# senikm/trpx

Hardware: AMD Instinct MI355X
Metric: frames/s (Terse encode + Prolix decode round trip, 512x512 uint16 stack, bit-exact vs CPU ref) (higher is better)
Workload: dtype u16

## Files before the change

### include/trpx_hip.h

```cpp
#ifndef TRPX_HIP_H
#define TRPX_HIP_H

#include <stddef.h>
#include <stdint.h>

#ifdef __cplusplus
extern "C" {
#endif

#define TRPX_ABI_VERSION 3

typedef enum trpx_status {
    TRPX_OK = 0,
    TRPX_ERR_INVALID_ARG = 1,
    TRPX_ERR_UNSUPPORTED = 2,
    TRPX_ERR_CAPACITY = 3,
    TRPX_ERR_HIP = 4,
    TRPX_ERR_CORRUPT = 5,
    TRPX_ERR_NO_DEVICE = 6,
    TRPX_ERR_TIMEOUT = 7
} trpx_status;

typedef enum trpx_dtype {
    TRPX_U8 = 0, TRPX_I8 = 1, TRPX_U16 = 2, TRPX_I16 = 3, TRPX_U32 = 4, TRPX_I32 = 5,
    TRPX_F32 = 6, TRPX_F64 = 7,
    TRPX_U64 = 8, TRPX_I64 = 9
} trpx_dtype;

enum { TRPX_STATUS_WORDS = 8 };

int         trpx_abi_version(void);
const char* trpx_last_error_string(void);
size_t      trpx_dtype_size(int dtype);
int         trpx_dtype_is_signed(int dtype);
int         trpx_device_count(void);

size_t trpx_worst_case_bytes(int dtype, size_t n_values, unsigned block);

size_t trpx_encode_workspace_bytes(int dtype, size_t n_values, size_t n_frames, unsigned block);
size_t trpx_decode_workspace_bytes(int dtype, size_t n_values, size_t n_frames, unsigned block);
unsigned trpx_decode_parts_per_frame(int dtype, size_t n_values, size_t n_frames, unsigned block);

int trpx_encode(int dtype, const void* pixels, size_t n_values, size_t n_frames, unsigned block,
                uint8_t* out, size_t out_capacity, uint64_t* frame_offsets, uint32_t* status,
                void* workspace, size_t workspace_bytes, void* stream);

int trpx_decode(int stream_signed, int out_dtype, const uint8_t* terse, size_t terse_bytes,
                const uint64_t* frame_offsets, size_t n_values, size_t n_frames, unsigned block,
                void* pixels_out, uint32_t* status, void* workspace, size_t workspace_bytes,
                void* stream);

int trpx_decode_convert(int stream_signed, int out_dtype, const uint8_t* terse, size_t terse_bytes,
                        const uint64_t* frame_offsets, size_t n_values, size_t n_frames, unsigned block,
                        void* pixels_out, uint32_t* status, void* workspace, size_t workspace_bytes,
                        void* stream);

size_t trpx_index_bytes(int dtype, size_t n_values, size_t n_frames, unsigned block);
int trpx_encode_indexed(int dtype, const void* pixels, size_t n_values, size_t n_frames, unsigned block,
                        uint8_t* out, size_t out_capacity, uint64_t* frame_offsets, uint32_t* status,
                        void* index, void* workspace, size_t workspace_bytes, void* stream);
int trpx_build_index(int dtype, const uint8_t* terse, size_t terse_bytes, const uint64_t* frame_offsets,
                     size_t n_values, size_t n_frames, unsigned block, void* index, uint32_t* status,
                     void* stream);
int trpx_decode_indexed(int stream_signed, int out_dtype, const uint8_t* terse, size_t terse_bytes,
                        const uint64_t* frame_offsets, const void* index, size_t n_values, size_t n_frames,
                        unsigned block, void* pixels_out, uint32_t* status, void* stream);

int trpx_encode_host(int dtype, const void* pixels, size_t n_values, size_t n_frames,
                     unsigned block, uint8_t* out, size_t out_capacity, size_t* total_bytes,
                     uint64_t* frame_offsets, uint32_t* prolix_bits, int device);
int trpx_decode_host(int stream_signed, int out_dtype, const uint8_t* terse, size_t terse_bytes,
                     const uint64_t* frame_offsets, size_t n_values, size_t n_frames,
                     unsigned block, void* pixels_out, int device);

int trpx_frame_offsets_host(const uint8_t* terse, size_t terse_bytes, size_t n_values, size_t n_frames,
                            unsigned block, unsigned max_bits, uint64_t* frame_offsets, int device);

size_t trpx_locate_workspace_bytes(size_t terse_bytes, size_t n_values, size_t n_frames, unsigned block);
int trpx_locate_frames(const uint8_t* terse, size_t terse_bytes, size_t n_values, size_t n_frames, unsigned block,
                       unsigned max_bits, uint64_t* frame_offsets, uint32_t* status, void* workspace, size_t workspace_bytes,
                       void* stream);
int trpx_set_locate_path(int path);

size_t trpx_decode_sum_workspace_bytes(int dtype, size_t terse_bytes, size_t n_values, size_t n_frames,
                                       unsigned block, unsigned group);
int trpx_decode_sum(int dtype, int out_dtype, const uint8_t* terse, size_t terse_bytes,
                    const uint64_t* frame_offsets, const void* index, size_t n_values, size_t n_frames,
                    unsigned block, unsigned group, void* sums_out, uint32_t* status,
                    void* workspace, size_t workspace_bytes, void* stream);
int trpx_decode_sum_host(int dtype, int out_dtype, const uint8_t* terse, size_t terse_bytes,
                         const uint64_t* frame_offsets, size_t n_values, size_t n_frames, unsigned block,
                         unsigned group, void* sums_out, int device);

size_t trpx_decode_roi_workspace_bytes(int dtype, size_t terse_bytes, size_t n_values, size_t n_frames, unsigned block);
int trpx_decode_roi(int dtype, const uint8_t* terse, size_t terse_bytes, const uint64_t* frame_offsets, const void* index,
                    size_t n_values, size_t n_frames, unsigned block, size_t width, const uint32_t* boxes, size_t n_boxes,
                    unsigned box_h, unsigned box_w, void* pixels_out, uint32_t* status, void* workspace,
                    size_t workspace_bytes, void* stream);
int trpx_decode_roi_host(int dtype, const uint8_t* terse, size_t terse_bytes, const uint64_t* frame_offsets, size_t n_values,
                         size_t n_frames, unsigned block, size_t width, const uint32_t* boxes, size_t n_boxes,
                         unsigned box_h, unsigned box_w, void* pixels_out, int device);

int trpx_synth_fill(int dtype, uint64_t seed, uint64_t frame0, size_t n_frames, size_t n_values,
                    void* pixels_dev, void* stream);

int trpx_workspace_invalidate(const void* workspace, size_t workspace_bytes);

int trpx_bench_stream(int mode, const void* src, void* dst, size_t bytes, void* stream);

int trpx_set_encode_path(int path);

int trpx_set_decode_path(int path);

int trpx_encode_checked(int dtype, const void* pixels, size_t n_values, size_t n_frames, unsigned block, uint8_t* out,
                        size_t out_capacity, uint64_t* frame_offsets, uint32_t* status, void* index, void* workspace,
                        size_t workspace_bytes, void* stream, uint32_t* host_status);

int trpx_profile_enable(int on);
int trpx_profile_read(float* stage_ms, int capacity);

typedef struct trpx_header {
    unsigned prolix_bits;
    int      is_signed;
    unsigned block;
    uint64_t memory_size;
    uint64_t number_of_values;
    uint64_t number_of_frames;
    unsigned n_dims;
    uint64_t dims[8];
} trpx_header;

size_t trpx_header_format(const trpx_header* h, char* buf, size_t buf_cap);
int trpx_header_parse(const char* data, size_t len, trpx_header* h, size_t* payload_offset);

size_t trpx_header_format_indexed(const trpx_header* h, const uint64_t* frame_sizes, size_t n_sizes, char* buf, size_t buf_cap);
size_t trpx_header_frame_sizes(const char* data, size_t len, uint64_t* frame_sizes, size_t capacity);

size_t trpx_group_count(size_t n_values, unsigned block);
int trpx_index_group_states(const void* index, size_t n_values, size_t n_frames, unsigned block, uint64_t* group_states, void* stream);
int trpx_index_from_group_states(int dtype, const uint8_t* terse, size_t terse_bytes, const uint64_t* frame_offsets,
                                 const uint64_t* group_states, size_t n_values, size_t n_frames, unsigned block, void* index,
                                 uint32_t* status, void* stream);
int trpx_group_states_host(const uint8_t* terse, size_t terse_bytes, const uint64_t* frame_offsets, size_t n_values,
                           size_t n_frames, unsigned block, unsigned max_bits, uint64_t* group_states, int device);
int trpx_decode_host_grouped(int stream_signed, int out_dtype, const uint8_t* terse, size_t terse_bytes, const uint64_t* frame_offsets,
                             const uint64_t* group_states, size_t n_values, size_t n_frames, unsigned block, void* pixels_out,
                             int device);
size_t trpx_header_format_grouped(const trpx_header* h, const uint64_t* frame_sizes, size_t n_sizes, const uint64_t* group_states,
                                  size_t n_states, char* buf, size_t buf_cap);
size_t trpx_header_group_states(const char* data, size_t len, uint64_t* group_states, size_t capacity);

typedef struct trpx_stack trpx_stack;
int trpx_stack_open(trpx_stack** handle, int stream_signed, const uint8_t* terse, size_t terse_bytes, const uint64_t* frame_offsets,
                    const uint64_t* group_states , size_t n_values, size_t n_frames, unsigned block,
                    unsigned max_bits, int device);
int trpx_stack_read(trpx_stack* stack, size_t frame, int out_dtype, void* pixels_out);
void trpx_stack_close(trpx_stack* stack);
void trpx_host_release(void);

size_t trpx_gather_workspace_bytes(size_t n_slot, int world);
int trpx_gather_frame_offsets(void* comm, const uint64_t* local_offsets, size_t n_local, size_t n_slot,
                              const uint32_t* encode_status, uint64_t* global_offsets, uint32_t* prolix_bits,
                              uint64_t* rank_base, void* workspace, size_t workspace_bytes, void* stream);
int trpx_gather_pack(const uint64_t* local_offsets, size_t n_local, size_t n_slot, const uint32_t* encode_status, uint64_t* message,
                     void* stream);
int trpx_gather_scan(const uint64_t* all_messages, int world, size_t n_slot, uint64_t* global_offsets, uint32_t* prolix_bits,
                     uint64_t* rank_base, void* stream);
size_t trpx_encode_sharded_workspace_bytes(int dtype, size_t n_values, size_t n_local, size_t n_slot, unsigned block, int world);
int trpx_encode_sharded(void* comm, int dtype, const void* pixels, size_t n_values, size_t n_local, size_t n_slot, unsigned block,
                        uint8_t* out, size_t out_capacity, uint64_t* local_offsets, uint32_t* status, uint64_t* global_offsets,
                        uint32_t* prolix_bits, uint64_t* rank_base, void* workspace, size_t workspace_bytes, void* stream,
                        void* gather_stream);
size_t trpx_decode_sharded_workspace_bytes(int dtype, size_t n_values, size_t n_local, unsigned block);
int trpx_decode_sharded(int stream_signed, int out_dtype, const uint8_t* local_terse, size_t local_bytes, const uint64_t* global_offsets,
                        size_t first_frame, size_t n_values, size_t n_local, unsigned block, void* pixels_out, uint32_t* status,
                        void* workspace, size_t workspace_bytes, void* stream);
int trpx_comm_unique_id(void* id128);
int trpx_comm_init(void** comm, int world, int rank, const void* id128);
int trpx_comm_destroy(void* comm);
int trpx_comm_info(void* comm, int* world, int* rank);
const char* trpx_shard_last_error(void);

#ifdef __cplusplus
}
#endif
#endif
```

### trpx_amd/_lib.py

```python
from __future__ import annotations

import ctypes as C
import os

_HERE = os.path.dirname(os.path.abspath(__file__))
LIB_PATH = os.environ.get("TRPX_LIB") or os.path.join(_HERE, "libtrpx_hip.so")

OK, ERR_INVALID_ARG, ERR_UNSUPPORTED, ERR_CAPACITY, ERR_HIP, ERR_CORRUPT, ERR_NO_DEVICE, ERR_TIMEOUT = range(8)
U8, I8, U16, I16, U32, I32, F32, F64, U64, I64 = range(10)
STATUS_WORDS = 8
ABI_VERSION = 3


class TrpxError(RuntimeError):
    def __init__(self, code: int, text: str):
        super().__init__(f"trpx error {code}: {text}")
        self.code = code


class trpx_header(C.Structure):
    _fields_ = [("prolix_bits", C.c_uint), ("is_signed", C.c_int), ("block", C.c_uint),
                ("memory_size", C.c_uint64), ("number_of_values", C.c_uint64),
                ("number_of_frames", C.c_uint64), ("n_dims", C.c_uint), ("dims", C.c_uint64 * 8)]


_P, _SZ, _U, _I, _U64 = C.c_void_p, C.c_size_t, C.c_uint, C.c_int, C.c_uint64
SYMBOLS = {
    "trpx_abi_version": (_I, []),
    "trpx_last_error_string": (C.c_char_p, []),
    "trpx_dtype_size": (_SZ, [_I]),
    "trpx_dtype_is_signed": (_I, [_I]),
    "trpx_device_count": (_I, []),
    "trpx_worst_case_bytes": (_SZ, [_I, _SZ, _U]),
    "trpx_encode_workspace_bytes": (_SZ, [_I, _SZ, _SZ, _U]),
    "trpx_decode_workspace_bytes": (_SZ, [_I, _SZ, _SZ, _U]),
    "trpx_decode_parts_per_frame": (_U, [_I, _SZ, _SZ, _U]),
    "trpx_encode": (_I, [_I, _P, _SZ, _SZ, _U, _P, _SZ, _P, _P, _P, _SZ, _P]),
    "trpx_decode": (_I, [_I, _I, _P, _SZ, _P, _SZ, _SZ, _U, _P, _P, _P, _SZ, _P]),
    "trpx_index_bytes": (_SZ, [_I, _SZ, _SZ, _U]),
    "trpx_encode_indexed": (_I, [_I, _P, _SZ, _SZ, _U, _P, _SZ, _P, _P, _P, _P, _SZ, _P]),
    "trpx_encode_checked": (_I, [_I, _P, _SZ, _SZ, _U, _P, _SZ, _P, _P, _P, _P, _SZ, _P, _P]),
    "trpx_build_index": (_I, [_I, _P, _SZ, _P, _SZ, _SZ, _U, _P, _P, _P]),
    "trpx_decode_indexed": (_I, [_I, _I, _P, _SZ, _P, _P, _SZ, _SZ, _U, _P, _P, _P]),
    "trpx_decode_convert": (_I, [_I, _I, _P, _SZ, _P, _SZ, _SZ, _U, _P, _P, _P, _SZ, _P]),
    "trpx_encode_host": (_I, [_I, _P, _SZ, _SZ, _U, _P, _SZ, C.POINTER(_SZ), _P, C.POINTER(_U), _I]),
    "trpx_decode_host": (_I, [_I, _I, _P, _SZ, _P, _SZ, _SZ, _U, _P, _I]),
    "trpx_frame_offsets_host": (_I, [_P, _SZ, _SZ, _SZ, _U, _U, _P, _I]),
    "trpx_locate_workspace_bytes": (_SZ, [_SZ, _SZ, _SZ, _U]),
    "trpx_locate_frames": (_I, [_P, _SZ, _SZ, _SZ, _U, _U, _P, _P, _P, _SZ, _P]),
    "trpx_decode_sum_workspace_bytes": (_SZ, [_I, _SZ, _SZ, _SZ, _U, _U]),
    "trpx_decode_sum": (_I, [_I, _I, _P, _SZ, _P, _P, _SZ, _SZ, _U, _U, _P, _P, _P, _SZ, _P]),
    "trpx_decode_sum_host": (_I, [_I, _I, _P, _SZ, _P, _SZ, _SZ, _U, _U, _P, _I]),
    "trpx_decode_roi_workspace_bytes": (_SZ, [_I, _SZ, _SZ, _SZ, _U]),
    "trpx_decode_roi": (_I, [_I, _P, _SZ, _P, _P, _SZ, _SZ, _U, _SZ, _P, _SZ, _U, _U, _P, _P, _P, _SZ, _P]),
    "trpx_decode_roi_host": (_I, [_I, _P, _SZ, _P, _SZ, _SZ, _U, _SZ, _P, _SZ, _U, _U, _P, _I]),
    "trpx_gather_workspace_bytes": (_SZ, [_SZ, _I]),
    "trpx_gather_frame_offsets": (_I, [_P, _P, _SZ, _SZ, _P, _P, _P, _P, _P, _SZ, _P]),
    "trpx_encode_sharded_workspace_bytes": (_SZ, [_I, _SZ, _SZ, _SZ, _U, _I]),
    "trpx_encode_sharded": (_I, [_P, _I, _P, _SZ, _SZ, _SZ, _U, _P, _SZ, _P, _P, _P, _P, _P, _P, _SZ, _P, _P]),
    "trpx_decode_sharded_workspace_bytes": (_SZ, [_I, _SZ, _SZ, _U]),
    "trpx_decode_sharded": (_I, [_I, _I, _P, _SZ, _P, _SZ, _SZ, _SZ, _U, _P, _P, _P, _SZ, _P]),
    "trpx_gather_pack": (_I, [_P, _SZ, _SZ, _P, _P, _P]),
    "trpx_gather_scan": (_I, [_P, _I, _SZ, _P, _P, _P, _P]),
    "trpx_comm_unique_id": (_I, [_P]),
    "trpx_comm_init": (_I, [C.POINTER(_P), _I, _I, _P]),
    "trpx_comm_destroy": (_I, [_P]),
    "trpx_comm_info": (_I, [_P, C.POINTER(C.c_int), C.POINTER(C.c_int)]),
    "trpx_shard_last_error": (C.c_char_p, []),
    "trpx_stack_open": (_I, [C.POINTER(_P), _I, _P, _SZ, _P, _P, _SZ, _SZ, _U, _U, _I]),
    "trpx_group_count": (_SZ, [_SZ, _U]),
    "trpx_index_group_states": (_I, [_P, _SZ, _SZ, _U, _P, _P]),
    "trpx_index_from_group_states": (_I, [_I, _P, _SZ, _P, _P, _SZ, _SZ, _U, _P, _P, _P]),
    "trpx_group_states_host": (_I, [_P, _SZ, _P, _SZ, _SZ, _U, _U, _P, _I]),
    "trpx_decode_host_grouped": (_I, [_I, _I, _P, _SZ, _P, _P, _SZ, _SZ, _U, _P, _I]),
    "trpx_header_format_grouped": (_SZ, [C.POINTER(trpx_header), C.c_void_p, _SZ, C.c_void_p, _SZ, C.c_char_p, _SZ]),
    "trpx_header_group_states": (_SZ, [C.c_char_p, _SZ, C.c_void_p, _SZ]),
    "trpx_stack_read": (_I, [_P, _SZ, _I, _P]),
    "trpx_stack_close": (None, [_P]),
    "trpx_host_release": (None, []),
    "trpx_set_encode_path": (_I, [_I]),
    "trpx_set_decode_path": (_I, [_I]),
    "trpx_set_locate_path": (_I, [_I]),
    "trpx_profile_enable": (_I, [_I]),
    "trpx_profile_read": (_I, [C.POINTER(C.c_float), _I]),
    "trpx_bench_stream": (_I, [_I, _P, _P, _SZ, _P]),
    "trpx_workspace_invalidate": (_I, [_P, _SZ]),
    "trpx_synth_fill": (_I, [_I, _U64, _U64, _SZ, _SZ, _P, _P]),
    "trpx_header_format": (_SZ, [C.POINTER(trpx_header), C.c_char_p, _SZ]),
    "trpx_header_parse": (_I, [C.c_char_p, _SZ, C.POINTER(trpx_header), C.POINTER(_SZ)]),
    "trpx_header_format_indexed": (_SZ, [C.POINTER(trpx_header), C.c_void_p, _SZ, C.c_char_p, _SZ]),
    "trpx_header_frame_sizes": (_SZ, [C.c_char_p, _SZ, C.c_void_p, _SZ]),
}

_lib = None


def lib() -> C.CDLL:
    global _lib
    if _lib is None:
        if not os.path.exists(LIB_PATH):
            raise ImportError(f"{LIB_PATH} is missing: the HIP extension has not been built "
                              "(run __graft_entry__.build()); trpx_amd has no CPU fallback")
        L = C.CDLL(LIB_PATH)
        for name, (res, args) in SYMBOLS.items():
            fn = getattr(L, name)
            fn.restype = res
            fn.argtypes = args
        if L.trpx_abi_version() != ABI_VERSION:
            raise ImportError(f"libtrpx_hip.so ABI version {L.trpx_abi_version()} != {ABI_VERSION} (include/trpx_hip.h: TRPX_ABI_VERSION)")
        _lib = L
    return _lib


def check(rc: int) -> None:
    if rc != OK:
        raise TrpxError(rc, lib().trpx_last_error_string().decode(errors="replace"))
```

### trpx_amd/codec.py

```python
from __future__ import annotations

from dataclasses import dataclass

import numpy as np
import torch

from . import _lib
from ._lib import check, lib

_TORCH2DT = {torch.uint8: _lib.U8, torch.int8: _lib.I8, torch.uint16: _lib.U16, torch.int16: _lib.I16,
             torch.uint32: _lib.U32, torch.int32: _lib.I32, torch.uint64: _lib.U64, torch.int64: _lib.I64}
_NP2TORCH = {np.dtype(np.uint8): torch.uint8, np.dtype(np.int8): torch.int8, np.dtype(np.uint16): torch.uint16,
             np.dtype(np.int16): torch.int16, np.dtype(np.uint32): torch.uint32, np.dtype(np.int32): torch.int32,
             np.dtype(np.uint64): torch.uint64, np.dtype(np.int64): torch.int64}
BLOCK = 12


def dtype_code(dt) -> int:
    if isinstance(dt, torch.dtype):
        return _TORCH2DT[dt]
    return _TORCH2DT[_NP2TORCH[np.dtype(dt)]]


def torch_dtype(dt) -> torch.dtype:
    return dt if isinstance(dt, torch.dtype) else _NP2TORCH[np.dtype(dt)]


def _stream_ptr(t: torch.Tensor) -> int:
    return torch.cuda.current_stream(t.device).cuda_stream


def worst_case_bytes(dtype, n_values: int, block: int = BLOCK) -> int:
    return lib().trpx_worst_case_bytes(dtype_code(dtype), n_values, block)


@dataclass
class Encoded:
    data: torch.Tensor
    frame_offsets: torch.Tensor
    status: torch.Tensor
    n_values: int
    n_frames: int
    dtype: torch.dtype
    index: torch.Tensor | None = None
    _retry: tuple | None = None

    def total_bytes(self) -> int:
        return int(self.frame_offsets[-1].item())

    def prolix_bits(self) -> int:
        return int(self.status[1].item())

    def check(self) -> None:
        code = int(self.status[0].item())
        if code == _lib.ERR_TIMEOUT and self._retry is not None:
            px, ws, block = self._retry
            with torch.cuda.device(px.device):
                check(lib().trpx_encode_checked(dtype_code(px.dtype), px.data_ptr(), self.n_values, self.n_frames, block,
                                                self.data.data_ptr(), self.data.numel(), self.frame_offsets.data_ptr(),
                                                self.status.data_ptr(), self.index.data_ptr() if self.index is not None else None,
                                                ws.data_ptr(), ws.numel(), _stream_ptr(px), None))
            code = int(self.status[0].item())
        if code:
            raise _lib.TrpxError(code, "device status after encode")

    def stack(self) -> torch.Tensor:
        return self.data[: self.total_bytes()]


class Workspace:

    def __init__(self, device):
        self.device = torch.device(device)
        self.buf = None

    def get(self, nbytes: int) -> torch.Tensor:
        if self.buf is None or self.buf.numel() < nbytes:
            self.release()
            self.buf = torch.empty(max(nbytes, 256), dtype=torch.uint8, device=self.device)
        return self.buf

    def release(self) -> None:
        if self.buf is not None:
            try:
                lib().trpx_workspace_invalidate(self.buf.data_ptr(), self.buf.numel())
            except Exception:
                pass
            self.buf = None

    def __del__(self):
        self.release()


def index_bytes(dtype, n_values: int, n_frames: int, block: int = BLOCK) -> int:
    return lib().trpx_index_bytes(dtype_code(dtype), n_values, n_frames, block)


def encode(pixels: torch.Tensor, out: torch.Tensor | None = None, workspace: Workspace | None = None,
           frame_offsets: torch.Tensor | None = None, status: torch.Tensor | None = None,
           block: int = BLOCK, index: torch.Tensor | bool | None = None) -> Encoded:
    if not pixels.is_cuda:
        raise ValueError("pixels must live on the GPU (use trpx_amd.Terse for host data)")
    px = pixels.contiguous()
    n_frames = px.shape[0]
    n_values = px[0].numel()
    code = dtype_code(px.dtype)
    dev = px.device
    if out is None:
        cap = (n_frames * worst_case_bytes(px.dtype, n_values, block) + 15) // 16 * 16
        out = torch.empty(cap, dtype=torch.uint8, device=dev)
    if frame_offsets is None:
        frame_offsets = torch.empty(n_frames + 1, dtype=torch.int64, device=dev)
    if status is None:
        status = torch.empty(_lib.STATUS_WORDS, dtype=torch.int32, device=dev)
    ws_bytes = lib().trpx_encode_workspace_bytes(code, n_values, n_frames, block)
    ws = workspace.get(ws_bytes) if workspace is not None else torch.empty(max(ws_bytes, 256), dtype=torch.uint8, device=dev)
    if index is True:
        index = torch.empty(index_bytes(px.dtype, n_values, n_frames, block), dtype=torch.uint8, device=dev)
    with torch.cuda.device(dev):
        check(lib().trpx_encode_indexed(code, px.data_ptr(), n_values, n_frames, block, out.data_ptr(), out.numel(),
                                        frame_offsets.data_ptr(), status.data_ptr(),
                                        index.data_ptr() if index is not None else None, ws.data_ptr(), ws.numel(),
                                        _stream_ptr(px)))
        if workspace is None:
            check(lib().trpx_workspace_invalidate(ws.data_ptr(), ws.numel()))
    return Encoded(out, frame_offsets, status, n_values, n_frames, px.dtype, index if index is not None else None, (px, ws, block))


def decode(terse: torch.Tensor, frame_offsets: torch.Tensor | None, n_values: int, n_frames: int, dtype,
           out: torch.Tensor | None = None, workspace: Workspace | None = None,
           status: torch.Tensor | None = None, stream_signed: bool | None = None,
           block: int = BLOCK, index: torch.Tensor | None = None):
    tdt = torch_dtype(dtype)
    code = dtype_code(tdt)
    dev = terse.device
    if stream_signed is None:
        stream_signed = bool(lib().trpx_dtype_is_signed(code))
    if out is None:
        out = torch.empty((n_frames, n_values), dtype=tdt, device=dev)
    if status is None:
        status = torch.empty(_lib.STATUS_WORDS, dtype=torch.int32, device=dev)
    if index is not None:
        with torch.cuda.device(dev):
            check(lib().trpx_decode_indexed(int(stream_signed), code, terse.data_ptr(), terse.numel(),
                                            frame_offsets.data_ptr(), index.data_ptr(), n_values, n_frames, block,
                                            out.data_ptr(), status.data_ptr(), _stream_ptr(terse)))
        return out, status
    ws_bytes = lib().trpx_decode_workspace_bytes(code, n_values, n_frames, block)
    ws = (workspace or Workspace(dev)).get(ws_bytes)
    with torch.cuda.device(dev):
        check(lib().trpx_decode(int(stream_signed), code, terse.data_ptr(), terse.numel(),
                                frame_offsets.data_ptr() if frame_offsets is not None else None,
                                n_values, n_frames, block, out.data_ptr(), status.data_ptr(), ws.data_ptr(),
                                ws.numel(), _stream_ptr(terse)))
    return out, status


def locate_workspace_bytes(terse_bytes: int, n_values: int, n_frames: int, block: int = BLOCK) -> int:
    return lib().trpx_locate_workspace_bytes(terse_bytes, n_values, n_frames, block)


def _max_bits(dtype) -> int:
    return 8 * lib().trpx_dtype_size(dtype_code(torch_dtype(dtype)))


def locate_frames(terse: torch.Tensor, n_values: int, n_frames: int, dtype, block: int = BLOCK,
                  workspace: Workspace | None = None, status: torch.Tensor | None = None,
                  out: torch.Tensor | None = None):
    dev = terse.device
    if out is None:
        out = torch.empty(n_frames + 1, dtype=torch.int64, device=dev)
    if status is None:
        status = torch.empty(_lib.STATUS_WORDS, dtype=torch.int32, device=dev)
    ws = (workspace or Workspace(dev)).get(locate_workspace_bytes(terse.numel(), n_values, n_frames, block))
    with torch.cuda.device(dev):
        check(lib().trpx_locate_frames(terse.data_ptr(), terse.numel(), n_values, n_frames, block, _max_bits(dtype),
                                       out.data_ptr(), status.data_ptr(), ws.data_ptr(), ws.numel(), _stream_ptr(terse)))
    return out, status


def build_index(terse: torch.Tensor, frame_offsets: torch.Tensor, n_values: int, n_frames: int, dtype,
                block: int = BLOCK) -> torch.Tensor:
    code = dtype_code(torch_dtype(dtype))
    dev = terse.device
    index = torch.empty(index_bytes(dtype, n_values, n_frames, block), dtype=torch.uint8, device=dev)
    status = torch.empty(_lib.STATUS_WORDS, dtype=torch.int32, device=dev)
    with torch.cuda.device(dev):
        check(lib().trpx_build_index(code, terse.data_ptr(), terse.numel(), frame_offsets.data_ptr(), n_values,
                                     n_frames, block, index.data_ptr(), status.data_ptr(), _stream_ptr(terse)))
    return index


def synth(dtype, frame0: int, n_frames: int, n_values: int, device="cuda", seed: int = 20240807) -> torch.Tensor:
    tdt = torch_dtype(dtype)
    out = torch.empty((n_frames, n_values), dtype=tdt, device=device)
    with torch.cuda.device(out.device):
        check(lib().trpx_synth_fill(dtype_code(tdt), seed, frame0, n_frames, n_values, out.data_ptr(),
                                    _stream_ptr(out)))
    return out


_SUM_OUT = {torch.int32: _lib.I32, torch.uint32: _lib.U32, torch.int64: _lib.I64, torch.uint64: _lib.U64,
            torch.float32: _lib.F32, torch.float64: _lib.F64}


def decode_sum_workspace_bytes(terse_bytes: int, n_values: int, n_frames: int, dtype, group: int, block: int = BLOCK) -> int:
    return lib().trpx_decode_sum_workspace_bytes(dtype_code(torch_dtype(dtype)), terse_bytes, n_values, n_frames, block, group)


def decode_sum(terse: torch.Tensor, frame_offsets: torch.Tensor | None, n_values: int, n_frames: int, dtype, group: int,
               out_dtype=torch.int32, index: torch.Tensor | None = None, out: torch.Tensor | None = None,
               workspace: Workspace | None = None, status: torch.Tensor | None = None, block: int = BLOCK):
    odt = torch_dtype(out_dtype)
    if odt not in _SUM_OUT:
        raise TypeError(f"decode_sum: out_dtype {odt} (int32, uint32, int64, uint64, float32, float64)")
    code = dtype_code(torch_dtype(dtype))
    dev = terse.device
    n_out = -(-n_frames // group) if group > 0 else 0
    if out is None:
        out = torch.empty((n_out, n_values), dtype=odt, device=dev)
    if status is None:
        status = torch.empty(_lib.STATUS_WORDS, dtype=torch.int32, device=dev)
    ws_bytes = lib().trpx_decode_sum_workspace_bytes(code, terse.numel(), n_values, n_frames, block, group)
    ws = (workspace or Workspace(dev)).get(ws_bytes)
    with torch.cuda.device(dev):
        check(lib().trpx_decode_sum(code, _SUM_OUT[odt], terse.data_ptr(), terse.numel(),
                                    frame_offsets.data_ptr() if frame_offsets is not None else None,
                                    index.data_ptr() if index is not None else None, n_values, n_frames, block, group,
                                    out.data_ptr(), status.data_ptr(), ws.data_ptr(), ws.numel(), _stream_ptr(terse)))
    return out, status


def decode_roi_workspace_bytes(terse_bytes: int, n_values: int, n_frames: int, dtype, block: int = BLOCK) -> int:
    return lib().trpx_decode_roi_workspace_bytes(dtype_code(torch_dtype(dtype)), terse_bytes, n_values, n_frames, block)


def decode_roi(terse: torch.Tensor, frame_offsets: torch.Tensor | None, n_values: int, n_frames: int, dtype, width: int,
               boxes: torch.Tensor, box_shape, index: torch.Tensor | None = None, out: torch.Tensor | None = None,
               workspace: Workspace | None = None, status: torch.Tensor | None = None, block: int = BLOCK):
    tdt = torch_dtype(dtype)
    code = dtype_code(tdt)
    dev = terse.device
    if boxes.dtype not in (torch.int32, torch.uint32) or boxes.dim() != 2 or boxes.shape[1] != 3 or not boxes.is_contiguous():
        raise TypeError("decode_roi: boxes must be a contiguous [n, 3] tensor of int32 / uint32")
    if boxes.device != dev:
        raise ValueError("decode_roi: boxes must live on the stack's device")
    box_h, box_w = (int(x) for x in box_shape)
    n_boxes = boxes.shape[0]
    if out is None:
        out = torch.empty((n_boxes, box_h, box_w), dtype=tdt, device=dev)
    elif out.dtype != tdt or out.numel() != n_boxes * box_h * box_w or not out.is_contiguous() or out.device != dev:
        raise ValueError(f"decode_roi: out must be a contiguous {tdt} tensor of {n_boxes} x {box_h} x {box_w} elements on {dev}")
    if status is None:
        status = torch.empty(_lib.STATUS_WORDS, dtype=torch.int32, device=dev)
    ws_ptr, ws_bytes = None, 0
    if index is None or frame_offsets is None:
        ws = (workspace or Workspace(dev)).get(lib().trpx_decode_roi_workspace_bytes(code, terse.numel(), n_values, n_frames, block))
        ws_ptr, ws_bytes = ws.data_ptr(), ws.numel()
    with torch.cuda.device(dev):
        check(lib().trpx_decode_roi(code, terse.data_ptr(), terse.numel(),
                                    frame_offsets.data_ptr() if frame_offsets is not None else None,
                                    index.data_ptr() if index is not None else None, n_values, n_frames, block, width,
                                    boxes.data_ptr(), n_boxes, box_h, box_w, out.data_ptr(), status.data_ptr(), ws_ptr, ws_bytes,
                                    _stream_ptr(terse)))
    return out, status
```

### trpx_amd/csrc/api.hip

```cpp
#include <hip/hip_runtime.h>
#include <stdarg.h>
#include <stdio.h>
#include <stdlib.h>
#include <string.h>
#include <algorithm>
#include <initializer_list>
#include <vector>

#include "../../include/trpx_hip.h"
#include "decode_roi.hpp"
#include "decode_sum.hpp"
#include "launchers.hpp"
#include "profile.hpp"

namespace trpx {
Profiler& profiler() {
    static thread_local Profiler p;
    return p;
}
}

namespace {

thread_local char g_err[512] = "";

int fail(int code, const char* fmt, ...) {
    va_list ap;
    va_start(ap, fmt);
    vsnprintf(g_err, sizeof g_err, fmt, ap);
    va_end(ap);
    return code;
}
#define HIP_TRY(expr)                                                                         \
    do {                                                                                      \
        hipError_t e_ = (expr);                                                               \
        if (e_ != hipSuccess) return fail(TRPX_ERR_HIP, "%s: %s", #expr, hipGetErrorString(e_)); \
    } while (0)

constexpr unsigned kMaxBlock = 4096;
constexpr unsigned kBlock = trpx::kBlock;

bool is64(int dtype) { return dtype == TRPX_U64 || dtype == TRPX_I64; }
size_t convert_elem_size(int out_dtype) { return out_dtype == TRPX_F32 ? 4 : out_dtype == TRPX_F64 ? 8 : trpx_dtype_size(out_dtype); }
bool tuned_type(int stream_signed, int out_dtype) {
    return trpx_dtype_size(out_dtype) && out_dtype <= TRPX_I32 && (stream_signed != 0) == (trpx_dtype_is_signed(out_dtype) != 0);
}
uint64_t worst_frame_bits(int dtype, size_t n_values, unsigned block) { return 8 * (uint64_t)trpx_worst_case_bytes(dtype, n_values, block); }
bool frame_bits_fit_32(int dtype, size_t n_values, unsigned block) { return worst_frame_bits(dtype, n_values, block) < 0xF0000000ull; }
bool fits_per_frame_decoder(int dtype, size_t n_values, unsigned block) { return worst_frame_bits(dtype, n_values, block) + (1u << 17) < (1ull << 26); }

bool geom_of(size_t n_values, unsigned block, trpx::FrameGeom* g) {
    if (n_values == 0 || block == 0 || block > kMaxBlock) return false;
    const uint64_t nb = (n_values + block - 1) / block;
    if (nb > 0xFFFFFFFFull) return false;
    g->n_values = n_values;
    g->n_blocks = (uint32_t)nb;
    g->n_tiles = (uint32_t)((nb + trpx::kTileBlocks - 1) / trpx::kTileBlocks);
    g->block = block;
    return true;
}

bool sizes_ok(const trpx::FrameGeom& g, size_t n_frames) {
    if (n_frames == 0 || n_frames > 0x7FFFFFFFull / g.n_tiles) return false;
    const unsigned __int128 bytes = (unsigned __int128)g.n_values * n_frames * 8;
    return bytes < ((unsigned __int128)1 << 62);
}
int bad_geom(const char* fn, unsigned block) {
    return fail(block != kBlock ? TRPX_ERR_UNSUPPORTED : TRPX_ERR_INVALID_ARG, "%s: unsupported sizes/block (block=%u)", fn, block);
}

struct PtrReq { const void* p; size_t align; bool required = true; };
enum : unsigned {
    kDtypeFirst = 1,
    kIndexOnly = 2,
    kSameSign = 4,
    kHasStream = 8,
};
int check_args(const char* fn, unsigned rules, int dtype, size_t elem, int stream_signed, size_t terse_bytes, size_t n_values,
               size_t n_frames, unsigned block, std::initializer_list<PtrReq> ptrs, trpx::FrameGeom* g) {
    if ((rules & kDtypeFirst) && !elem) return fail(TRPX_ERR_INVALID_ARG, "%s: unknown dtype %d", fn, dtype);
    if (rules & kIndexOnly ? block != kBlock : block == 0 || block > kMaxBlock)
        return fail(TRPX_ERR_UNSUPPORTED, rules & kIndexOnly ? "%s: block=%u (the decode index needs %u)" : "%s: block=%u (supported: 1..%u; 12 is the tuned default, Terse.hpp:264)",
                    fn, block, rules & kIndexOnly ? kBlock : kMaxBlock);
    if ((rules & kIndexOnly) && is64(dtype)) return fail(TRPX_ERR_UNSUPPORTED, "%s: no decode index for 64-bit containers (generic kernels)", fn);
    if ((rules & kSameSign) && (stream_signed != 0) != (trpx_dtype_is_signed(dtype) != 0))
        return fail(TRPX_ERR_UNSUPPORTED, "%s: stream signed=%d into dtype %d: only same-signedness decode is defined by the reference (Terse.hpp:356-357)",
                    fn, stream_signed, dtype);
    if (!elem) return fail(TRPX_ERR_INVALID_ARG, "%s: unknown dtype %d", fn, dtype);
    if (!geom_of(n_values, block, g) || !sizes_ok(*g, n_frames) || ((rules & kHasStream) && !terse_bytes))
        return fail(TRPX_ERR_INVALID_ARG, "%s: bad sizes n_values=%zu n_frames=%zu", fn, n_values, n_frames);
    for (const PtrReq& q : ptrs)
        if (q.required && !q.p) return fail(TRPX_ERR_INVALID_ARG, "%s: null pointer", fn);
    for (const PtrReq& q : ptrs)
        if ((uintptr_t)q.p % q.align) return fail(TRPX_ERR_INVALID_ARG, "%s: misaligned pointer (%p needs %zu B)", fn, q.p, q.align);
    return TRPX_OK;
}

struct EncWs { size_t frame_size, tile_off, tile_bits, fused, total; };
EncWs enc_ws(const trpx::FrameGeom& g, size_t n_frames) {
    EncWs w;
    const size_t tiles = n_frames * (size_t)g.n_tiles;
    w.frame_size = 0;
    w.tile_off = trpx::align_up(w.frame_size + 8 * n_frames, 16);
    w.tile_bits = trpx::align_up(w.tile_off + 8 * tiles, 16);
    w.fused = trpx::align_up(w.tile_bits + 4 * tiles, 256);
    w.total = w.fused + trpx::fused_workspace_bytes(g, n_frames);
    return w;
}

struct DecLayout { size_t tile_off, widths, seg, defer, parts, part_ws, total; };
DecLayout dec_layout(const trpx::FrameGeom& g, size_t n_frames, size_t pixel_bytes, size_t front, bool parts_route) {
    DecLayout l;
    l.tile_off = trpx::align_up(front, 16);
    l.widths = trpx::align_up(l.tile_off + 8 * n_frames * (size_t)g.n_tiles, 16);
    l.seg = trpx::align_up(l.widths + n_frames * (size_t)g.n_blocks, 256);
    l.defer = l.seg + trpx::seg_workspace_bytes(g, n_frames);
    l.parts = l.defer + trpx::defer_bytes(n_frames);
    size_t P = trpx::chain_parts_per_frame(g, n_frames, pixel_bytes), scratch = trpx::chain_workspace_bytes(g, n_frames, pixel_bytes);
    if (parts_route) {
        P = std::max<size_t>(P, trpx::parts_per_frame(g, n_frames));
        scratch = std::max(scratch, trpx::part_workspace_bytes(g, n_frames));
    }
    l.part_ws = l.parts + (P > 1 ? trpx::align_up(sizeof(trpx::PartDesc) * n_frames * P, 256) : 0);
    l.total = l.part_ws + scratch;
    return l;
}
DecLayout idx_layout(const trpx::FrameGeom& g, size_t n_frames, size_t pixel_bytes = 4) { return dec_layout(g, n_frames, pixel_bytes, 0, false); }
DecLayout dec_ws(const trpx::FrameGeom& g, size_t n_frames, size_t pixel_bytes) { return dec_layout(g, n_frames, pixel_bytes, 8 * (n_frames + 1), true); }

trpx::DecodeArgs decode_args(const uint8_t* terse, size_t terse_bytes, const uint64_t* frame_offsets, const trpx::FrameGeom& g,
                             size_t n_frames, void* pixels_out, uint32_t* status) {
    trpx::DecodeArgs a{};
    a.terse = terse;
    a.terse_bytes = terse_bytes;
    a.frame_offsets = frame_offsets;
    a.geom = g;
    a.n_frames = (uint32_t)n_frames;
    a.pixels_out = pixels_out;
    a.status = status;
    return a;
}
enum : unsigned { kSeg = 1, kDefer = 2, kParts = 4 };
void point_into(trpx::DecodeArgs& a, const void* block, const DecLayout& l, unsigned scratch = 0) {
    char* b = const_cast<char*>(static_cast<const char*>(block));
    a.tile_off = reinterpret_cast<uint64_t*>(b + l.tile_off);
    a.widths = reinterpret_cast<uint8_t*>(b + l.widths);
    if (scratch & kSeg) a.seg_ws = b + l.seg;
    if (scratch & kDefer) a.defer = reinterpret_cast<uint32_t*>(b + l.defer + trpx::kDeferFront);
    if (scratch & kParts) {
        a.parts = reinterpret_cast<trpx::PartDesc*>(b + l.parts);
        a.part_ws = b + l.part_ws;
    }
}

int g_encode_path = [] {
    const char* e = getenv("TRPX_ENCODE_PATH");
    return e && strcmp(e, "twopass") == 0 ? 1 : 0;
}();
enum DecodeRoute {
    kRouteAuto = 0,
    kRouteBasic = 1,
    kRouteTiled = 2,
    kRouteFrames = 3,
    kRouteParts = 4,
};
constexpr int kSelectDense = 5;
DecodeRoute g_decode_path = [] {
    const char* e = getenv("TRPX_DECODE_PATH");
    if (!e) return kRouteAuto;
    if (strcmp(e, "dense") == 0) trpx::set_dense_route(true);
    return strcmp(e, "basic") == 0 ? kRouteBasic : (strcmp(e, "tiles") == 0 || strcmp(e, "seg") == 0) ? kRouteTiled
           : strcmp(e, "frames") == 0 ? kRouteFrames : strcmp(e, "parts") == 0 ? kRouteParts : kRouteAuto;
}();
bool large_frames_by_index() { return g_decode_path != kRouteTiled && g_decode_path != kRouteParts; }
[[maybe_unused]] const int g_single_part_env = [] {
    const char* e = getenv("TRPX_SINGLE_PART");
    unsigned f = 0, b = 0;
    if (e && sscanf(e, "%u,%u", &f, &b) == 2) trpx::set_single_part_rule(f, b);
    return 0;
}();

struct IdxScratch {
    struct Slot { int dev; hipStream_t st; void* p; size_t bytes; };
    std::vector<Slot> slots;
    ~IdxScratch() { for (auto& s : slots) if (s.p) (void)hipFree(s.p); }
};
void* indexed_scratch(size_t bytes, hipStream_t st) {
    static thread_local IdxScratch t;
    int dev = 0;
    if (hipGetDevice(&dev) != hipSuccess) return nullptr;
    hipStreamCaptureStatus cs = hipStreamCaptureStatusNone;
    if (hipStreamIsCapturing(st, &cs) != hipSuccess) { (void)hipGetLastError(); return nullptr; }
    if (cs != hipStreamCaptureStatusNone) return nullptr;
    for (auto& s : t.slots)
        if (s.dev == dev && s.st == st) {
            if (s.bytes >= bytes) return s.p;
            if (hipStreamSynchronize(st) != hipSuccess) return nullptr;
            (void)hipFree(s.p);
            s.p = nullptr; s.bytes = 0;
            if (hipMalloc(&s.p, bytes) != hipSuccess) { s.p = nullptr; (void)hipGetLastError(); return nullptr; }
            s.bytes = bytes;
            return s.p;
        }
    void* p = nullptr;
    if (hipMalloc(&p, bytes) != hipSuccess) { (void)hipGetLastError(); return nullptr; }
    t.slots.push_back({dev, st, p, bytes});
    return p;
}

int build_index_impl(int dtype, const uint8_t* terse, size_t terse_bytes, const uint64_t* frame_offsets, size_t n_values,
                     size_t n_frames, unsigned block, void* index, uint32_t* status, bool clear_status, void* stream) {
    trpx::FrameGeom g;
    if (const int rc = check_args("trpx_build_index", kIndexOnly | kHasStream, dtype, trpx_dtype_size(dtype), 0, terse_bytes, n_values, n_frames, block,
                                  {{terse, 4}, {frame_offsets, 8}, {index, 16}, {status, 8}}, &g))
        return rc;
    if (!frame_bits_fit_32(dtype, n_values, block)) return fail(TRPX_ERR_UNSUPPORTED, "trpx_build_index: frames of >= 2^32 bits");
    trpx::DecodeArgs a = decode_args(terse, terse_bytes, frame_offsets, g, n_frames, nullptr, status);
    const DecLayout il = idx_layout(g, n_frames, trpx_dtype_size(dtype));
    point_into(a, index, il, kSeg | kDefer);
    a.index_per_frame = fits_per_frame_decoder(dtype, n_values, block) && g_decode_path != kRouteTiled;
    a.parts_per_frame = trpx::chain_parts_per_frame(g, n_frames, trpx_dtype_size(dtype));
    a.chain = a.parts_per_frame > 1u && n_frames * (uint64_t)a.parts_per_frame < 0x7FFFFFFFull && large_frames_by_index();
    if (a.chain) point_into(a, index, il, kParts);
    else a.parts_per_frame = 1;
    HIP_TRY(trpx::launch_walk_only(a, (uint32_t)(8 * trpx_dtype_size(dtype)), clear_status, static_cast<hipStream_t>(stream)));
    return TRPX_OK;
}

int encode_impl(int dtype, const void* pixels, size_t n_values, size_t n_frames, unsigned block, uint8_t* out, size_t out_capacity,
                uint64_t* frame_offsets, uint32_t* status, void* index, void* workspace, size_t workspace_bytes, void* stream,
                bool two_pass) {
    trpx::FrameGeom g;
    if (const int rc = check_args("trpx_encode", kDtypeFirst, dtype, trpx_dtype_size(dtype), 0, 0, n_values, n_frames, block,
                                  {{pixels, trpx_dtype_size(dtype)}, {frame_offsets, 8}, {status, 8}, {workspace, 8},
                                   {out, 16, out_capacity != 0}}, &g))
        return rc;
    const EncWs w = enc_ws(g, n_frames);
    if (workspace_bytes < w.total)
        return fail(TRPX_ERR_CAPACITY, "trpx_encode: workspace %zu < %zu", workspace_bytes, w.total);

    trpx::EncodeArgs a;
    a.pixels = pixels;
    a.geom = g;
    a.n_frames = (uint32_t)n_frames;
    a.out = out;
    a.out_capacity = out_capacity;
    a.frame_offsets = frame_offsets;
    a.status = status;
    char* ws = static_cast<char*>(workspace);
    a.frame_size = reinterpret_cast<uint64_t*>(ws + w.frame_size);
    a.tile_off = reinterpret_cast<uint64_t*>(ws + w.tile_off);
    a.tile_bits = reinterpret_cast<uint32_t*>(ws + w.tile_bits);
    if ((uintptr_t)index % 16) return fail(TRPX_ERR_INVALID_ARG, "trpx_encode_indexed: index must be 16-byte aligned");
    const DecLayout il = idx_layout(g, n_frames, trpx_dtype_size(dtype));
    a.idx_group_off = index ? reinterpret_cast<uint64_t*>(static_cast<char*>(index) + il.tile_off) : nullptr;
    a.idx_widths = index ? reinterpret_cast<uint8_t*>(static_cast<char*>(index) + il.widths) : nullptr;
    if (block != kBlock || is64(dtype)) {
        if (index) return fail(TRPX_ERR_UNSUPPORTED, "trpx_encode_indexed: the decode index needs block=12 and pixels of <= 32 bits");
        trpx::fused_ws_forget(workspace, workspace_bytes);
        HIP_TRY(trpx::launch_encode_generic(dtype, a, static_cast<hipStream_t>(stream)));
        return TRPX_OK;
    }
    const bool vec_ok = (uint64_t)g.n_blocks * 396 < (1ull << 40);
    if (g_encode_path == 0 && !two_pass && vec_ok) {
        trpx::fused_ws_forget(workspace, workspace_bytes, ws + w.fused);
        HIP_TRY(trpx::launch_encode_fused(dtype, a, ws + w.fused, static_cast<hipStream_t>(stream)));
    } else {
        trpx::fused_ws_forget(workspace, workspace_bytes);
        HIP_TRY(trpx::launch_encode(dtype, a, static_cast<hipStream_t>(stream)));
        if (index && out)
            return build_index_impl(dtype, out, out_capacity, frame_offsets, n_values, n_frames, block, index, status, false, stream);
    }
    return TRPX_OK;
}

hipError_t copy_sync(hipStream_t hs, void* dst, const void* src, size_t n, hipMemcpyKind kind) {
    const hipError_t e = hipMemcpyAsync(dst, src, n, kind, hs);
    return e != hipSuccess ? e : hipStreamSynchronize(hs);
}
int read_status(hipStream_t hs, const uint32_t* d_status, uint32_t st[TRPX_STATUS_WORDS]) {
    HIP_TRY(copy_sync(hs, st, d_status, 4 * TRPX_STATUS_WORDS, hipMemcpyDeviceToHost));
    return TRPX_OK;
}
int status_result(const char* fn, const uint32_t* st) {
    return st[0] ? fail((int)st[0], "%s: device status %u (5: corrupt or truncated stream)", fn, st[0]) : TRPX_OK;
}

int encode_retrying(int dtype, const void* pixels, size_t n_values, size_t n_frames, unsigned block, uint8_t* out, size_t out_capacity,
                    uint64_t* frame_offsets, uint32_t* status, void* index, void* workspace, size_t workspace_bytes, void* stream,
                    uint32_t st[TRPX_STATUS_WORDS]) {
    for (int attempt = 0; attempt < 2; ++attempt) {
        int rc = encode_impl(dtype, pixels, n_values, n_frames, block, out, out_capacity, frame_offsets, status, index, workspace,
                             workspace_bytes, stream, attempt == 1);
        if (rc || (rc = read_status(static_cast<hipStream_t>(stream), status, st))) return rc;
        if (st[0] != TRPX_ERR_TIMEOUT) break;
    }
    return TRPX_OK;
}

}

extern "C" {

int trpx_abi_version(void) { return TRPX_ABI_VERSION; }
const char* trpx_last_error_string(void) { return g_err; }

size_t trpx_dtype_size(int dtype) {
    switch (dtype) {
    case TRPX_U8: case TRPX_I8: return 1;
    case TRPX_U16: case TRPX_I16: return 2;
    case TRPX_U32: case TRPX_I32: return 4;
    case TRPX_U64: case TRPX_I64: return 8;
    }
    return 0;
}
int trpx_dtype_is_signed(int dtype) { return dtype >= 0 && dtype <= TRPX_I32 ? (dtype & 1) : (dtype == TRPX_I64 ? 1 : 0); }

int trpx_device_count(void) {
    int n = 0;
    if (hipGetDeviceCount(&n) != hipSuccess) return 0;
    return n;
}

size_t trpx_worst_case_bytes(int dtype, size_t n_values, unsigned block) {
    const size_t es = trpx_dtype_size(dtype);
    if (!es || !block) return 0;
    const size_t nblocks = (n_values + block - 1) / block;
    return n_values * es + (12 * nblocks + 7) / 8 + 1;
}

size_t trpx_encode_workspace_bytes(int dtype, size_t n_values, size_t n_frames, unsigned block) {
    trpx::FrameGeom g;
    if (!trpx_dtype_size(dtype) || !geom_of(n_values, block, &g)) return 0;
    return enc_ws(g, n_frames).total;
}
size_t trpx_decode_workspace_bytes(int dtype, size_t n_values, size_t n_frames, unsigned block) {
    trpx::FrameGeom g;
    if (!trpx_dtype_size(dtype) || !geom_of(n_values, block, &g)) return 0;
    return dec_ws(g, n_frames, trpx_dtype_size(dtype)).total;
}
size_t trpx_index_bytes(int dtype, size_t n_values, size_t n_frames, unsigned block) {
    trpx::FrameGeom g;
    if (!trpx_dtype_size(dtype) || !geom_of(n_values, block, &g)) return 0;
    return idx_layout(g, n_frames, trpx_dtype_size(dtype)).total;
}

unsigned trpx_decode_parts_per_frame(int dtype, size_t n_values, size_t n_frames, unsigned block) {
    trpx::FrameGeom g;
    if (!trpx_dtype_size(dtype) || is64(dtype) || block != kBlock || !geom_of(n_values, block, &g)) return 1;
    return g_decode_path != kRouteParts && frame_bits_fit_32(dtype, n_values, block) ? trpx::chain_parts_per_frame(g, n_frames, trpx_dtype_size(dtype))
                                                                                   : trpx::parts_per_frame(g, n_frames);
}

int trpx_encode(int dtype, const void* pixels, size_t n_values, size_t n_frames, unsigned block, uint8_t* out,
                size_t out_capacity, uint64_t* frame_offsets, uint32_t* status, void* workspace,
                size_t workspace_bytes, void* stream) {
    return encode_impl(dtype, pixels, n_values, n_frames, block, out, out_capacity, frame_offsets, status, nullptr, workspace,
                       workspace_bytes, stream, false);
}

int trpx_encode_indexed(int dtype, const void* pixels, size_t n_values, size_t n_frames, unsigned block, uint8_t* out,
                        size_t out_capacity, uint64_t* frame_offsets, uint32_t* status, void* index,
                        void* workspace, size_t workspace_bytes, void* stream) {
    return encode_impl(dtype, pixels, n_values, n_frames, block, out, out_capacity, frame_offsets, status, index, workspace,
                       workspace_bytes, stream, false);
}

int trpx_encode_checked(int dtype, const void* pixels, size_t n_values, size_t n_frames, unsigned block, uint8_t* out,
                        size_t out_capacity, uint64_t* frame_offsets, uint32_t* status, void* index, void* workspace,
                        size_t workspace_bytes, void* stream, uint32_t* host_status) {
    uint32_t st[TRPX_STATUS_WORDS] = {0};
    if (const int rc = encode_retrying(dtype, pixels, n_values, n_frames, block, out, out_capacity, frame_offsets, status, index,
                                       workspace, workspace_bytes, stream, st))
        return rc;
    if (host_status) memcpy(host_status, st, sizeof st);
    return status_result("trpx_encode_checked", st);
}

int trpx_decode(int stream_signed, int out_dtype, const uint8_t* terse, size_t terse_bytes,
                const uint64_t* frame_offsets, size_t n_values, size_t n_frames, unsigned block, void* pixels_out,
                uint32_t* status, void* workspace, size_t workspace_bytes, void* stream) {
    trpx::FrameGeom g;
    const size_t es = trpx_dtype_size(out_dtype);
    if (!es) return fail(TRPX_ERR_INVALID_ARG, "trpx_decode: unknown dtype %d", out_dtype);
    if (is64(out_dtype))
        return trpx_decode_convert(stream_signed, out_dtype, terse, terse_bytes, frame_offsets, n_values, n_frames, block, pixels_out,
                                   status, workspace, workspace_bytes, stream);
    if (const int rc = check_args("trpx_decode", kDtypeFirst | kSameSign | kHasStream, out_dtype, es, stream_signed, terse_bytes, n_values, n_frames,
                                  block, {{terse, 4}, {pixels_out, es}, {status, 8}, {workspace, 8}, {frame_offsets, 8, false}}, &g))
        return rc;
    const DecLayout w = dec_ws(g, n_frames, es);
    if (workspace_bytes < w.total)
        return fail(TRPX_ERR_CAPACITY, "trpx_decode: workspace %zu < %zu", workspace_bytes, w.total);

    hipStream_t hs = static_cast<hipStream_t>(stream);
    trpx::fused_ws_forget(workspace, workspace_bytes);
    trpx::DecodeArgs a = decode_args(terse, terse_bytes, frame_offsets, g, n_frames, pixels_out, status);
    char* ws = static_cast<char*>(workspace);
    a.walk_offsets = reinterpret_cast<uint64_t*>(ws);
#ifdef TRPX_DIAGNOSTICS
    static const bool no_defer = getenv("TRPX_NO_DEFER") != nullptr;
#else
    constexpr bool no_defer = false;
#endif
    point_into(a, ws, w, no_defer ? kSeg : kSeg | kDefer);
    const bool basic = g_decode_path == kRouteBasic, force_tiles = g_decode_path == kRouteTiled;
    const bool bits32 = frame_bits_fit_32(out_dtype, n_values, block);
    const uint32_t max_w = 8u * (uint32_t)es;
    const bool located = !frame_offsets && !basic && bits32 && block == kBlock && trpx::locate_parallel(g, terse_bytes, n_frames, max_w) &&
                         w.total - w.tile_off >= trpx::locate_workspace_bytes(g, terse_bytes, n_frames);
    if (located) {
        HIP_TRY(trpx::launch_locate(terse, terse_bytes, g, (uint32_t)n_frames, max_w, a.walk_offsets, status, ws + w.tile_off, hs));
        a.frame_offsets = frame_offsets = a.walk_offsets;
    }
    const bool fast_ok = frame_offsets && !basic && bits32 && block == kBlock;
    const bool frame26 = fits_per_frame_decoder(out_dtype, n_values, block);
    a.chain = large_frames_by_index() && bits32;
    a.parts_per_frame = a.chain ? trpx::chain_parts_per_frame(g, n_frames, es) : trpx::parts_per_frame(g, n_frames);
    const bool parts_ok = a.parts_per_frame > 1u && n_frames * (uint64_t)a.parts_per_frame < 0x7FFFFFFFull && a.defer;
    if (parts_ok) point_into(a, ws, w, kParts);
    else a.parts_per_frame = 1;
    if (fast_ok && (parts_ok || (frame26 && trpx::parts_per_frame(g, n_frames) == 1u)) && !force_tiles)
        HIP_TRY(trpx::launch_decode_frames(out_dtype, a, hs));
    else if (fast_ok)
        HIP_TRY(trpx::launch_decode_fast(out_dtype, a, false, hs));
    else
        HIP_TRY(trpx::launch_decode(out_dtype, a, frame_offsets != nullptr, hs));
    if (located)
        HIP_TRY(trpx::launch_locate_status(a.walk_offsets, (uint32_t)n_frames, status, hs));
    return TRPX_OK;
}

int trpx_build_index(int dtype, const uint8_t* terse, size_t terse_bytes, const uint64_t* frame_offsets,
                     size_t n_values, size_t n_frames, unsigned block, void* index, uint32_t* status, void* stream) {
    return build_index_impl(dtype, terse, terse_bytes, frame_offsets, n_values, n_frames, block, index, status, true, stream);
}

int trpx_decode_indexed(int stream_signed, int out_dtype, const uint8_t* terse, size_t terse_bytes,
                        const uint64_t* frame_offsets, const void* index, size_t n_values, size_t n_frames,
                        unsigned block, void* pixels_out, uint32_t* status, void* stream) {
    trpx::FrameGeom g;
    const size_t es = trpx_dtype_size(out_dtype);
    if (const int rc = check_args("trpx_decode_indexed", kDtypeFirst | kIndexOnly | kSameSign | kHasStream, out_dtype, es, stream_signed, terse_bytes,
                                  n_values, n_frames, block, {{terse, 4}, {index, 16}, {frame_offsets, 8}, {pixels_out, es}, {status, 8}}, &g))
        return rc;
    hipStream_t hs = static_cast<hipStream_t>(stream);
    trpx::DecodeArgs a = decode_args(terse, terse_bytes, frame_offsets, g, n_frames, pixels_out, status);
    point_into(a, index, idx_layout(g, n_frames, es));
    const bool per_frame = fits_per_frame_decoder(out_dtype, n_values, block) && g_decode_path != kRouteTiled &&
                           (g_decode_path == kRouteFrames || n_frames >= 1024);
    const bool misaligned = (g.n_values * es) % 128u != 0u || (uintptr_t)pixels_out % 128u != 0u;
    if (per_frame && misaligned && g_decode_path == kRouteAuto && trpx::parts_per_frame(g, n_frames) == 1u) {
        void* scratch = indexed_scratch(trpx::defer_bytes(n_frames), hs);
        if (scratch) {
            a.defer = reinterpret_cast<uint32_t*>(static_cast<char*>(scratch) + trpx::kDeferFront);
            a.seg_ws = scratch;
            a.index_given = true;
            HIP_TRY(trpx::launch_decode_frames(out_dtype, a, hs));
            return TRPX_OK;
        }
    }
    HIP_TRY(trpx::launch_decode_fast(out_dtype, a, true, hs, per_frame));
    return TRPX_OK;
}

size_t trpx_group_count(size_t n_values, unsigned block) {
    trpx::FrameGeom g;
    if (block != kBlock || !geom_of(n_values, block, &g)) return 0;
    return g.n_tiles;
}

int trpx_index_group_states(const void* index, size_t n_values, size_t n_frames, unsigned block, uint64_t* states, void* stream) {
    trpx::FrameGeom g;
    if (const int rc = check_args("trpx_index_group_states", kIndexOnly, TRPX_U8, 1, 0, 0, n_values, n_frames, block, {{index, 16}, {states, 8}}, &g))
        return rc;
    trpx::DecodeArgs a = decode_args(nullptr, 0, nullptr, g, n_frames, nullptr, nullptr);
    point_into(a, index, idx_layout(g, n_frames));
    HIP_TRY(trpx::launch_index_group_states(a, states, static_cast<hipStream_t>(stream)));
    return TRPX_OK;
}

int trpx_index_from_group_states(int dtype, const uint8_t* terse, size_t terse_bytes, const uint64_t* frame_offsets,
                                 const uint64_t* states, size_t n_values, size_t n_frames, unsigned block, void* index,
                                 uint32_t* status, void* stream) {
    trpx::FrameGeom g;
    if (const int rc = check_args("trpx_index_from_group_states", kIndexOnly | kHasStream, dtype, trpx_dtype_size(dtype), 0, terse_bytes, n_values,
                                  n_frames, block, {{terse, 4}, {frame_offsets, 8}, {states, 8}, {index, 16}, {status, 8}}, &g))
        return rc;
    if (worst_frame_bits(dtype, n_values, block) >= (1ull << 40))
        return fail(TRPX_ERR_UNSUPPORTED, "trpx_index_from_group_states: frames of >= 2^40 bits");
    trpx::DecodeArgs a = decode_args(terse, terse_bytes, frame_offsets, g, n_frames, nullptr, status);
    point_into(a, index, idx_layout(g, n_frames));
    HIP_TRY(trpx::launch_walk_groups(a, (uint32_t)(8 * trpx_dtype_size(dtype)), states, true, static_cast<hipStream_t>(stream)));
    return TRPX_OK;
}

int trpx_decode_convert(int stream_signed, int out_dtype, const uint8_t* terse, size_t terse_bytes,
                        const uint64_t* frame_offsets, size_t n_values, size_t n_frames, unsigned block, void* pixels_out,
                        uint32_t* status, void* workspace, size_t workspace_bytes, void* stream) {
    trpx::FrameGeom g;
    const size_t es = convert_elem_size(out_dtype);
    if (const int rc = check_args("trpx_decode_convert", kDtypeFirst | kHasStream, out_dtype, es, stream_signed, terse_bytes, n_values, n_frames, block,
                                  {{terse, 4}, {pixels_out, es}, {status, 8}, {workspace, 8}, {frame_offsets, 8, false}}, &g))
        return rc;
    const DecLayout w = dec_ws(g, n_frames, es);
    if (workspace_bytes < w.total) return fail(TRPX_ERR_CAPACITY, "trpx_decode_convert: workspace %zu < %zu", workspace_bytes, w.total);
    trpx::fused_ws_forget(workspace, workspace_bytes);
    trpx::DecodeArgs a = decode_args(terse, terse_bytes, frame_offsets, g, n_frames, pixels_out, status);
    a.walk_offsets = static_cast<uint64_t*>(workspace);
    point_into(a, workspace, w, kSeg);
    HIP_TRY(trpx::launch_decode_convert(out_dtype, a, stream_signed != 0, frame_offsets != nullptr, static_cast<hipStream_t>(stream)));
    return TRPX_OK;
}

int trpx_workspace_invalidate(const void* workspace, size_t workspace_bytes) {
    trpx::fused_ws_forget(workspace, workspace_bytes);
    return TRPX_OK;
}

int trpx_set_encode_path(int path) {
    if (path != 0 && path != 1) return fail(TRPX_ERR_INVALID_ARG, "trpx_set_encode_path: 0 = auto, 1 = two-pass");
    g_encode_path = path;
    return TRPX_OK;
}

int trpx_set_decode_path(int path) {
    if (path < kRouteAuto || path > kSelectDense) return fail(TRPX_ERR_INVALID_ARG, "trpx_set_decode_path: 0 = auto, 1 = basic, 2 = tiled, 3 = per-frame, 4 = parts route for large frames, 5 = auto with the dense walk for listed frames");
    trpx::set_dense_route(path == kSelectDense);
    g_decode_path = path == kSelectDense ? kRouteAuto : static_cast<DecodeRoute>(path);
    return TRPX_OK;
}

int trpx_set_locate_path(int path) {
    if (path != 0 && path != 1) return fail(TRPX_ERR_INVALID_ARG, "trpx_set_locate_path: 0 = auto, 1 = serial");
    trpx::g_locate_path = path;
    return TRPX_OK;
}

int trpx_profile_enable(int on) {
    trpx::profiler().enabled = on != 0;
    return TRPX_OK;
}
int trpx_profile_read(float* stage_ms, int capacity) {
    if (!stage_ms || capacity <= 0) return 0;
    return trpx::profiler().read(stage_ms, capacity);
}

int trpx_synth_fill(int dtype, uint64_t seed, uint64_t frame0, size_t n_frames, size_t n_values, void* pixels_dev,
                    void* stream) {
    if (dtype != TRPX_U16 && dtype != TRPX_I32)
        return fail(TRPX_ERR_UNSUPPORTED, "trpx_synth_fill: synth-v1 is defined for U16 and I32");
    if (!pixels_dev) return fail(TRPX_ERR_INVALID_ARG, "trpx_synth_fill: null pointer");
    HIP_TRY(trpx::launch_synth(dtype, seed, frame0, n_frames, n_values, pixels_dev, static_cast<hipStream_t>(stream)));
    return TRPX_OK;
}

size_t trpx_locate_workspace_bytes(size_t terse_bytes, size_t n_values, size_t n_frames, unsigned block) {
    trpx::FrameGeom g;
    if (!terse_bytes || !geom_of(n_values, block, &g) || !sizes_ok(g, n_frames)) return 0;
    return trpx::locate_workspace_bytes(g, terse_bytes, n_frames);
}

int trpx_locate_frames(const uint8_t* terse, size_t terse_bytes, size_t n_values, size_t n_frames, unsigned block, unsigned max_bits,
                       uint64_t* frame_offsets, uint32_t* status, void* workspace, size_t workspace_bytes, void* stream) {
    trpx::FrameGeom g;
    if (!terse || !terse_bytes || !frame_offsets || !status || !workspace || max_bits == 0 || max_bits > 64)
        return fail(TRPX_ERR_INVALID_ARG, "trpx_locate_frames: bad argument");
    if (!geom_of(n_values, block, &g)) return bad_geom("trpx_locate_frames", block);
    if (!sizes_ok(g, n_frames) || n_frames > terse_bytes)
        return fail(TRPX_ERR_INVALID_ARG, "trpx_locate_frames: bad sizes n_values=%zu n_frames=%zu", n_values, n_frames);
    if ((uintptr_t)terse % 4 || (uintptr_t)workspace % 8 || (uintptr_t)frame_offsets % 8 || (uintptr_t)status % 8)
        return fail(TRPX_ERR_INVALID_ARG, "trpx_locate_frames: misaligned pointer (terse needs 4 B, workspace 8 B)");
    const size_t need = trpx::locate_workspace_bytes(g, terse_bytes, n_frames);
    if (workspace_bytes < need) return fail(TRPX_ERR_CAPACITY, "trpx_locate_frames: workspace %zu < %zu", workspace_bytes, need);
    trpx::fused_ws_forget(workspace, workspace_bytes);
    HIP_TRY(trpx::launch_locate(terse, terse_bytes, g, (uint32_t)n_frames, max_bits, frame_offsets, status, workspace,
                                static_cast<hipStream_t>(stream)));
    return TRPX_OK;
}

}
namespace {
bool sum_out_ok(int out_dtype) {
    return out_dtype == TRPX_I32 || out_dtype == TRPX_U32 || out_dtype == TRPX_I64 || out_dtype == TRPX_U64 ||
           out_dtype == TRPX_F32 || out_dtype == TRPX_F64;
}
size_t sum_out_size(int out_dtype) { return out_dtype == TRPX_I32 || out_dtype == TRPX_U32 || out_dtype == TRPX_F32 ? 4 : 8; }
struct IndexWs { size_t offsets, region, total; };
IndexWs index_ws(int dtype, const trpx::FrameGeom& g, size_t terse_bytes, size_t n_frames, bool have_offsets, bool have_index) {
    IndexWs w;
    w.offsets = 0;
    w.region = have_offsets ? 0 : trpx::align_up(8 * (n_frames + 1), 256);
    const size_t idx = have_index ? 0 : idx_layout(g, n_frames, trpx_dtype_size(dtype)).total;
    const size_t loc = have_offsets ? 0 : trpx::locate_workspace_bytes(g, terse_bytes, n_frames);
    w.total = w.region + trpx::align_up(std::max(idx, loc), 256);
    return w;
}
int index_in_workspace(int dtype, const uint8_t* terse, size_t terse_bytes, const uint64_t** frame_offsets, const void** index,
                       size_t n_values, size_t n_frames, unsigned block, const trpx::FrameGeom& g, uint32_t* status, char* ws,
                       const IndexWs& w, void* stream, bool* clear) {
    *clear = true;
    if (!*frame_offsets) {
        uint64_t* offs = reinterpret_cast<uint64_t*>(ws + w.offsets);
        HIP_TRY(trpx::launch_locate(terse, terse_bytes, g, (uint32_t)n_frames, 8u * (uint32_t)trpx_dtype_size(dtype), offs, status,
                                    ws + w.region, static_cast<hipStream_t>(stream)));
        *frame_offsets = offs;
        *clear = false;
    }
    if (!*index) {
        const int rc = build_index_impl(dtype, terse, terse_bytes, *frame_offsets, n_values, n_frames, block, ws + w.region, status,
                                        *clear, stream);
        if (rc) return rc;
        *index = ws + w.region;
        *clear = false;
    }
    return TRPX_OK;
}
struct SumWs { IndexWs front; size_t partial, total; };
SumWs sum_ws(int dtype, const trpx::FrameGeom& g, size_t terse_bytes, size_t n_frames, size_t group, bool have_offsets, bool have_index) {
    SumWs w;
    w.front = index_ws(dtype, g, terse_bytes, n_frames, have_offsets, have_index);
    w.partial = w.front.total;
    w.total = w.partial + trpx::sum_plan(dtype, g, n_frames, group).partial_bytes;
    return w;
}
}

extern "C" {

size_t trpx_decode_sum_workspace_bytes(int dtype, size_t terse_bytes, size_t n_values, size_t n_frames, unsigned block,
                                       unsigned group) {
    trpx::FrameGeom g;
    if (dtype < TRPX_U8 || dtype > TRPX_I32 || block != kBlock || !group || !terse_bytes ||
        !geom_of(n_values, block, &g) || !sizes_ok(g, n_frames))
        return 0;
    return sum_ws(dtype, g, terse_bytes, n_frames, group, false, false).total;
}

int trpx_decode_sum(int dtype, int out_dtype, const uint8_t* terse, size_t terse_bytes, const uint64_t* frame_offsets,
                    const void* index, size_t n_values, size_t n_frames, unsigned block, unsigned group, void* sums_out,
                    uint32_t* status, void* workspace, size_t workspace_bytes, void* stream) {
    trpx::FrameGeom g;
    if (is64(dtype)) return fail(TRPX_ERR_UNSUPPORTED, "trpx_decode_sum: no decode index for 64-bit containers");
    if (dtype < TRPX_U8 || dtype > TRPX_I32) return fail(TRPX_ERR_INVALID_ARG, "trpx_decode_sum: unknown stream dtype %d", dtype);
    if (!sum_out_ok(out_dtype)) return fail(TRPX_ERR_INVALID_ARG, "trpx_decode_sum: out_dtype %d (I32, U32, I64, U64, F32, F64)", out_dtype);
    if (block != kBlock) return fail(TRPX_ERR_UNSUPPORTED, "trpx_decode_sum: block=%u (the decode index needs 12)", block);
    if (trpx_dtype_is_signed(dtype) && (out_dtype == TRPX_U32 || out_dtype == TRPX_U64))
        return fail(TRPX_ERR_UNSUPPORTED, "trpx_decode_sum: signed stream into an unsigned output (Terse.hpp:356-357)");
    if (group == 0) return fail(TRPX_ERR_INVALID_ARG, "trpx_decode_sum: group = 0");
    if (!geom_of(n_values, block, &g) || !sizes_ok(g, n_frames) || terse_bytes == 0 || n_frames > terse_bytes)
        return fail(TRPX_ERR_INVALID_ARG, "trpx_decode_sum: bad sizes n_values=%zu n_frames=%zu", n_values, n_frames);
    if (!terse || !sums_out || !status) return fail(TRPX_ERR_INVALID_ARG, "trpx_decode_sum: null pointer");
    if (index && !frame_offsets) return fail(TRPX_ERR_INVALID_ARG, "trpx_decode_sum: an index needs its frame offsets");
    if ((uintptr_t)terse % 4 || (uintptr_t)frame_offsets % 8 || (uintptr_t)index % 16 || (uintptr_t)status % 8 ||
        (uintptr_t)workspace % 8 || (uintptr_t)sums_out % sum_out_size(out_dtype))
        return fail(TRPX_ERR_INVALID_ARG, "trpx_decode_sum: misaligned pointer (terse 4 B, offsets / workspace 8 B, index 16 B, sums their type)");
    if (!frame_bits_fit_32(dtype, n_values, block)) return fail(TRPX_ERR_UNSUPPORTED, "trpx_decode_sum: frames of >= 2^32 bits");
    const SumWs w = sum_ws(dtype, g, terse_bytes, n_frames, group, frame_offsets != nullptr, index != nullptr);
    if (workspace_bytes < w.total) return fail(TRPX_ERR_CAPACITY, "trpx_decode_sum: workspace %zu < %zu", workspace_bytes, w.total);
    if (w.total && !workspace) return fail(TRPX_ERR_INVALID_ARG, "trpx_decode_sum: null workspace");
    const trpx::SumPlan p = trpx::sum_plan(dtype, g, n_frames, group);
    if (p.n_out * p.chunks * (uint64_t)p.tpf >= (1ull << 40)) return fail(TRPX_ERR_INVALID_ARG, "trpx_decode_sum: bad sizes");

    hipStream_t st = static_cast<hipStream_t>(stream);
    char* ws = static_cast<char*>(workspace);
    if (workspace) trpx::fused_ws_forget(workspace, workspace_bytes);
    bool clear = true;
    if (const int rc = index_in_workspace(dtype, terse, terse_bytes, &frame_offsets, &index, n_values, n_frames, block, g, status, ws,
                                          w.front, stream, &clear))
        return rc;
    const DecLayout il = idx_layout(g, n_frames, trpx_dtype_size(dtype));
    trpx::SumArgs a{};
    a.terse = terse;
    a.terse_bytes = terse_bytes;
    a.frame_offsets = frame_offsets;
    a.geom = g;
    a.n_frames = n_frames;
    a.group = group;
    a.n_out = p.n_out;
    a.tpf = p.tpf;
    a.chunks = p.chunks;
    a.fpc = p.fpc;
    a.tile_off = reinterpret_cast<const uint64_t*>(static_cast<const char*>(index) + il.tile_off);
    a.widths = reinterpret_cast<const uint8_t*>(static_cast<const char*>(index) + il.widths);
    a.out = sums_out;
    a.out_code = out_dtype;
    a.partial = p.chunks > 1 ? ws + w.partial : nullptr;
    a.status = status;
    HIP_TRY(trpx::launch_decode_sum(dtype, a, clear, st));
    return TRPX_OK;
}

}
namespace {
int roi_geometry(const char* fn, size_t n_values, size_t width, size_t n_boxes, unsigned box_h, unsigned box_w) {
    if (width == 0 || n_values % width) return fail(TRPX_ERR_INVALID_ARG, "%s: width %zu does not divide n_values %zu", fn, width, n_values);
    if (box_h == 0 || box_w == 0 || box_h > n_values / width || box_w > width)
        return fail(TRPX_ERR_INVALID_ARG, "%s: box %u x %u in frames of %zu x %zu", fn, box_h, box_w, n_values / width, width);
    if (n_boxes == 0) return fail(TRPX_ERR_INVALID_ARG, "%s: no boxes", fn);
    return TRPX_OK;
}
}
extern "C" {

size_t trpx_decode_roi_workspace_bytes(int dtype, size_t terse_bytes, size_t n_values, size_t n_frames, unsigned block) {
    trpx::FrameGeom g;
    if (dtype < TRPX_U8 || dtype > TRPX_I32 || block != kBlock || !terse_bytes || !geom_of(n_values, block, &g) || !sizes_ok(g, n_frames))
        return 0;
    return index_ws(dtype, g, terse_bytes, n_frames, false, false).total;
}

int trpx_decode_roi(int dtype, const uint8_t* terse, size_t terse_bytes, const uint64_t* frame_offsets, const void* index,
                    size_t n_values, size_t n_frames, unsigned block, size_t width, const uint32_t* boxes, size_t n_boxes,
                    unsigned box_h, unsigned box_w, void* pixels_out, uint32_t* status, void* workspace, size_t workspace_bytes,
                    void* stream) {
    trpx::FrameGeom g;
    const size_t es = trpx_dtype_size(dtype);
    if (const int rc = check_args("trpx_decode_roi", kDtypeFirst | kIndexOnly | kHasStream, dtype, es, 0, terse_bytes, n_values, n_frames, block,
                                  {{terse, 4}, {boxes, 4}, {pixels_out, es}, {status, 8}, {frame_offsets, 8, false}, {index, 16, false},
                                   {workspace, 8, false}}, &g))
        return rc;
    if (!frame_bits_fit_32(dtype, n_values, block)) return fail(TRPX_ERR_UNSUPPORTED, "trpx_decode_roi: frames of >= 2^32 bits");
    if (n_frames > terse_bytes) return fail(TRPX_ERR_INVALID_ARG, "trpx_decode_roi: bad sizes n_values=%zu n_frames=%zu", n_values, n_frames);
    if (const int rc = roi_geometry("trpx_decode_roi", n_values, width, n_boxes, box_h, box_w)) return rc;
    if (index && !frame_offsets) return fail(TRPX_ERR_INVALID_ARG, "trpx_decode_roi: an index needs its frame offsets");
    const uint32_t units = trpx::roi_units_per_box(g, (uint32_t)width, box_h, box_w);
    if ((unsigned __int128)n_boxes * units >= ((unsigned __int128)1 << 40) || (unsigned __int128)n_boxes * box_h * box_w * es >= ((unsigned __int128)1 << 62))
        return fail(TRPX_ERR_INVALID_ARG, "trpx_decode_roi: bad sizes n_boxes=%zu", n_boxes);
    const IndexWs w = index_ws(dtype, g, terse_bytes, n_frames, frame_offsets != nullptr, index != nullptr);
    if (workspace_bytes < w.total) return fail(TRPX_ERR_CAPACITY, "trpx_decode_roi: workspace %zu < %zu", workspace_bytes, w.total);
    if (w.total && !workspace) return fail(TRPX_ERR_INVALID_ARG, "trpx_decode_roi: null workspace");

    if (w.total) trpx::fused_ws_forget(workspace, workspace_bytes);
    bool clear = true;
    if (const int rc = index_in_workspace(dtype, terse, terse_bytes, &frame_offsets, &index, n_values, n_frames, block, g, status,
                                          static_cast<char*>(workspace), w, stream, &clear))
        return rc;
    const DecLayout il = idx_layout(g, n_frames, es);
    trpx::RoiArgs a{};
    a.terse = terse;
    a.terse_bytes = terse_bytes;
    a.frame_offsets = frame_offsets;
    a.geom = g;
    a.n_frames = n_frames;
    a.width = (uint32_t)width;
    a.height = (uint32_t)(n_values / width);
    a.boxes = boxes;
    a.n_boxes = n_boxes;
    a.box_h = box_h;
    a.box_w = box_w;
    a.units_per_box = units;
    a.tile_off = reinterpret_cast<const uint64_t*>(static_cast<const char*>(index) + il.tile_off);
    a.widths = reinterpret_cast<const uint8_t*>(static_cast<const char*>(index) + il.widths);
    a.out = pixels_out;
    a.status = status;
    HIP_TRY(trpx::launch_decode_roi(dtype, a, clear, static_cast<hipStream_t>(stream)));
    return TRPX_OK;
}

}
namespace {
struct Arena {
    enum { kPixels, kStream, kOffsets, kStatus, kWorkspace, kSlots };
    void* p[kSlots] = {};
    size_t cap[kSlots] = {};
    int device = -1;
    hipStream_t stream = nullptr;
    hipError_t on_device() {
        int dev = 0;
        const hipError_t e = hipGetDevice(&dev);
        if (e != hipSuccess) return e;
        if (dev != device) { release(); device = dev; }
        return hipSuccess;
    }
    hipError_t get(int slot, size_t n, void** out, bool encoder = false) {
        hipError_t e = on_device();
        if (e != hipSuccess) return e;
        if (slot == kWorkspace && !encoder && p[slot]) trpx::fused_ws_forget(p[slot], cap[slot]);
        if (cap[slot] < n) {
            if (p[slot] && slot == kWorkspace) trpx::fused_ws_forget(p[slot], cap[slot]);
            if (p[slot]) (void)hipFree(p[slot]);
            p[slot] = nullptr; cap[slot] = 0;
            const size_t want = n + n / 8 + 256;
            e = hipMalloc(&p[slot], want);
            if (e != hipSuccess) return e;
            cap[slot] = want;
        }
        *out = p[slot];
        return hipSuccess;
    }
    hipError_t get_stream(hipStream_t* out) {
        hipError_t e = on_device();
        if (e != hipSuccess) return e;
        if (!stream && (e = hipStreamCreateWithFlags(&stream, hipStreamNonBlocking)) != hipSuccess) return e;
        *out = stream;
        return hipSuccess;
    }
    void release() {
        if (p[kWorkspace]) trpx::fused_ws_forget(p[kWorkspace], cap[kWorkspace]);
        for (int i = 0; i < kSlots; ++i) { if (p[i]) (void)hipFree(p[i]); p[i] = nullptr; cap[i] = 0; }
        if (stream) (void)hipStreamDestroy(stream);
        stream = nullptr;
    }
    ~Arena() { release(); }
};
Arena& arena() {
    static thread_local Arena a;
    return a;
}

int enter(const char* fn, int device, hipStream_t* hs) {
    if (trpx_device_count() == 0) return fail(TRPX_ERR_NO_DEVICE, "%s: no HIP device", fn);
    if (device >= 0) HIP_TRY(hipSetDevice(device));
    HIP_TRY(arena().get_stream(hs));
    return TRPX_OK;
}
size_t padded_stream_bytes(size_t terse_bytes) { return trpx::align_up(terse_bytes, 4) + 8; }
hipError_t copy_stream_zero_tail(hipStream_t hs, void* d_terse, const uint8_t* terse, size_t terse_bytes) {
    const size_t whole = terse_bytes & ~size_t(3);
    const hipError_t e = hipMemsetAsync(static_cast<char*>(d_terse) + whole, 0, padded_stream_bytes(terse_bytes) - whole, hs);
    return e != hipSuccess ? e : copy_sync(hs, d_terse, terse, terse_bytes, hipMemcpyHostToDevice);
}
int upload_stream(hipStream_t hs, const uint8_t* terse, size_t terse_bytes, const uint8_t** d_terse) {
    void* p = nullptr;
    HIP_TRY(arena().get(Arena::kStream, padded_stream_bytes(terse_bytes), &p));
    HIP_TRY(copy_stream_zero_tail(hs, p, terse, terse_bytes));
    *d_terse = static_cast<const uint8_t*>(p);
    return TRPX_OK;
}
int upload_offsets(hipStream_t hs, const uint64_t* frame_offsets, size_t n_frames, size_t extra, uint64_t** d_offs) {
    void* p = nullptr;
    HIP_TRY(arena().get(Arena::kOffsets, 8 * (n_frames + 1) + extra, &p));
    if (frame_offsets) HIP_TRY(copy_sync(hs, p, frame_offsets, 8 * (n_frames + 1), hipMemcpyHostToDevice));
    *d_offs = static_cast<uint64_t*>(p);
    return TRPX_OK;
}
int status_slot(uint32_t** d_st) {
    void* p = nullptr;
    HIP_TRY(arena().get(Arena::kStatus, 4 * TRPX_STATUS_WORDS, &p));
    *d_st = static_cast<uint32_t*>(p);
    return TRPX_OK;
}

int decode_any(int stream_signed, int out_dtype, const uint8_t* d_terse, size_t terse_bytes, const uint64_t* d_offs, size_t n_values,
               size_t n_frames, unsigned block, void* d_out, uint32_t* d_st, void* d_ws, size_t ws_bytes, hipStream_t hs,
               uint32_t st[TRPX_STATUS_WORDS]) {
    for (bool convert = !tuned_type(stream_signed, out_dtype);; convert = true) {
        int rc = convert ? trpx_decode_convert(stream_signed, out_dtype, d_terse, terse_bytes, d_offs, n_values, n_frames, block, d_out, d_st, d_ws, ws_bytes, hs)
                         : trpx_decode(stream_signed, out_dtype, d_terse, terse_bytes, d_offs, n_values, n_frames, block, d_out, d_st, d_ws, ws_bytes, hs);
        if (rc || (rc = read_status(hs, d_st, st))) return rc;
        if (st[0] != TRPX_ERR_CORRUPT || convert) return TRPX_OK;
    }
}
int decode_walk_free(int stream_signed, int out_dtype, const uint8_t* d_terse, size_t terse_bytes, const uint64_t* d_offs,
                     const uint64_t* d_states, size_t n_values, size_t n_frames, unsigned block, void* d_index, void* d_out,
                     uint32_t* d_st, hipStream_t hs, bool stop_on_any, uint32_t st[TRPX_STATUS_WORDS], bool* decoded) {
    *decoded = false;
    int rc = trpx_index_from_group_states(out_dtype, d_terse, terse_bytes, d_offs, d_states, n_values, n_frames, block, d_index, d_st, hs);
    if (rc || (rc = read_status(hs, d_st, st))) return rc;
    if (st[0] == TRPX_ERR_CORRUPT || (stop_on_any && st[0])) return TRPX_OK;
    rc = trpx_decode_indexed(stream_signed, out_dtype, d_terse, terse_bytes, d_offs, d_index, n_values, n_frames, block, d_out, d_st, hs);
    if (rc || (rc = read_status(hs, d_st, st))) return rc;
    *decoded = true;
    return TRPX_OK;
}
}
extern "C" {

void trpx_host_release(void) { arena().release(); }

int trpx_encode_host(int dtype, const void* pixels, size_t n_values, size_t n_frames, unsigned block, uint8_t* out,
                     size_t out_capacity, size_t* total_bytes, uint64_t* frame_offsets, uint32_t* prolix_bits,
                     int device) {
    hipStream_t hs = nullptr;
    if (const int rc = enter("trpx_encode_host", device, &hs)) return rc;
    const size_t es = trpx_dtype_size(dtype);
    if (!es || !pixels || !out || !total_bytes) return fail(TRPX_ERR_INVALID_ARG, "trpx_encode_host: bad argument");
    trpx::FrameGeom g;
    if (!geom_of(n_values, block, &g)) return fail(block == 0 || block > kMaxBlock ? TRPX_ERR_UNSUPPORTED : TRPX_ERR_INVALID_ARG, "trpx_encode_host: unsupported sizes/block (block=%u)", block);
    if (!sizes_ok(g, n_frames)) return fail(TRPX_ERR_INVALID_ARG, "trpx_encode_host: bad sizes n_values=%zu n_frames=%zu", n_values, n_frames);
    const size_t in_bytes = n_values * n_frames * es;
    const size_t cap = trpx::align_up(n_frames * trpx_worst_case_bytes(dtype, n_values, block), 16);
    const size_t ws_bytes = enc_ws(g, n_frames).total;
    void *d_px = nullptr, *d_out = nullptr, *d_ws = nullptr;
    uint64_t* d_off = nullptr;
    uint32_t* d_st = nullptr;
    Arena& A = arena();
    HIP_TRY(A.get(Arena::kPixels, in_bytes, &d_px));
    HIP_TRY(A.get(Arena::kStream, cap, &d_out));
    HIP_TRY(A.get(Arena::kWorkspace, ws_bytes, &d_ws, true));
    int rc = upload_offsets(hs, nullptr, n_frames, 0, &d_off);
    if (rc || (rc = status_slot(&d_st))) return rc;
    HIP_TRY(copy_sync(hs, d_px, pixels, in_bytes, hipMemcpyHostToDevice));
    uint32_t st[TRPX_STATUS_WORDS];
    rc = encode_retrying(dtype, d_px, n_values, n_frames, block, static_cast<uint8_t*>(d_out), cap, d_off, d_st, nullptr, d_ws, ws_bytes, hs, st);
    if (rc || (rc = status_result("trpx_encode_host", st))) return rc;
    std::vector<uint64_t> offs(n_frames + 1);
    HIP_TRY(copy_sync(hs, offs.data(), d_off, 8 * (n_frames + 1), hipMemcpyDeviceToHost));
    const size_t total = (size_t)offs[n_frames];
    if (total > out_capacity) return fail(TRPX_ERR_CAPACITY, "trpx_encode_host: need %zu bytes, have %zu", total, out_capacity);
    HIP_TRY(copy_sync(hs, out, d_out, total, hipMemcpyDeviceToHost));
    *total_bytes = total;
    if (frame_offsets) memcpy(frame_offsets, offs.data(), 8 * (n_frames + 1));
    if (prolix_bits) *prolix_bits = st[1];
    return TRPX_OK;
}

int trpx_decode_host(int stream_signed, int out_dtype, const uint8_t* terse, size_t terse_bytes,
                     const uint64_t* frame_offsets, size_t n_values, size_t n_frames, unsigned block,
                     void* pixels_out, int device) {
    hipStream_t hs = nullptr;
    if (const int rc = enter("trpx_decode_host", device, &hs)) return rc;
    const size_t es = convert_elem_size(out_dtype);
    if (!es || !terse || !pixels_out || !terse_bytes) return fail(TRPX_ERR_INVALID_ARG, "trpx_decode_host: bad argument");
    trpx::FrameGeom g;
    if (!geom_of(n_values, block, &g)) return bad_geom("trpx_decode_host", block);
    if (!sizes_ok(g, n_frames)) return fail(TRPX_ERR_INVALID_ARG, "trpx_decode_host: bad sizes");
    const size_t out_bytes = n_values * n_frames * es;
    const size_t ws_bytes = trpx_decode_workspace_bytes(TRPX_U8, n_values, n_frames, block);
    const uint8_t* d_in = nullptr;
    uint64_t* d_off = nullptr;
    uint32_t* d_st = nullptr;
    void *d_out = nullptr, *d_ws = nullptr;
    int rc = upload_stream(hs, terse, terse_bytes, &d_in);
    if (rc || (rc = status_slot(&d_st)) || (frame_offsets && (rc = upload_offsets(hs, frame_offsets, n_frames, 0, &d_off)))) return rc;
    HIP_TRY(arena().get(Arena::kPixels, out_bytes, &d_out));
    HIP_TRY(arena().get(Arena::kWorkspace, ws_bytes, &d_ws));
    uint32_t st[TRPX_STATUS_WORDS];
    rc = decode_any(stream_signed, out_dtype, d_in, terse_bytes, d_off, n_values, n_frames, block, d_out, d_st, d_ws, ws_bytes, hs, st);
    if (rc || (rc = status_result("trpx_decode_host", st))) return rc;
    HIP_TRY(copy_sync(hs, pixels_out, d_out, out_bytes, hipMemcpyDeviceToHost));
    return TRPX_OK;
}

int trpx_frame_offsets_host(const uint8_t* terse, size_t terse_bytes, size_t n_values, size_t n_frames,
                            unsigned block, unsigned max_bits, uint64_t* frame_offsets, int device) {
    hipStream_t hs = nullptr;
    if (const int rc = enter("trpx_frame_offsets_host", device, &hs)) return rc;
    trpx::FrameGeom g;
    if (!terse || !terse_bytes || !frame_offsets || !n_frames || max_bits == 0 || max_bits > 64)
        return fail(TRPX_ERR_INVALID_ARG, "trpx_frame_offsets_host: bad argument");
    if (!geom_of(n_values, block, &g)) return bad_geom("trpx_frame_offsets_host", block);
    if (!sizes_ok(g, n_frames) || n_frames > terse_bytes)
        return fail(TRPX_ERR_INVALID_ARG, "trpx_frame_offsets_host: bad sizes n_values=%zu n_frames=%zu", n_values, n_frames);
    const size_t ws_bytes = trpx::locate_workspace_bytes(g, terse_bytes, n_frames);
    const uint8_t* d_in = nullptr;
    uint64_t* d_off = nullptr;
    uint32_t* d_st = nullptr;
    void* d_ws = nullptr;
    int rc = upload_stream(hs, terse, terse_bytes, &d_in);
    if (rc || (rc = upload_offsets(hs, nullptr, n_frames, 0, &d_off)) || (rc = status_slot(&d_st))) return rc;
    HIP_TRY(arena().get(Arena::kWorkspace, ws_bytes, &d_ws));
    uint32_t st[TRPX_STATUS_WORDS];
    rc = trpx_locate_frames(d_in, terse_bytes, n_values, n_frames, block, max_bits, d_off, d_st, d_ws, ws_bytes, hs);
    if (rc || (rc = read_status(hs, d_st, st)) || (rc = status_result("trpx_frame_offsets_host", st))) return rc;
    HIP_TRY(copy_sync(hs, frame_offsets, d_off, 8 * (n_frames + 1), hipMemcpyDeviceToHost));
    return TRPX_OK;
}

int trpx_decode_sum_host(int dtype, int out_dtype, const uint8_t* terse, size_t terse_bytes, const uint64_t* frame_offsets,
                         size_t n_values, size_t n_frames, unsigned block, unsigned group, void* sums_out, int device) {
    hipStream_t hs = nullptr;
    if (const int rc = enter("trpx_decode_sum_host", device, &hs)) return rc;
    trpx::FrameGeom g;
    if (!terse || !sums_out || !terse_bytes || !sum_out_ok(out_dtype) || !group)
        return fail(TRPX_ERR_INVALID_ARG, "trpx_decode_sum_host: bad argument");
    if (block != kBlock || is64(dtype)) return fail(TRPX_ERR_UNSUPPORTED, "trpx_decode_sum_host: block=%u dtype=%d", block, dtype);
    if (!geom_of(n_values, block, &g) || !sizes_ok(g, n_frames)) return fail(TRPX_ERR_INVALID_ARG, "trpx_decode_sum_host: bad sizes");
    const size_t ws_bytes = trpx_decode_sum_workspace_bytes(dtype, terse_bytes, n_values, n_frames, block, group);
    if (!ws_bytes) return fail(TRPX_ERR_INVALID_ARG, "trpx_decode_sum_host: bad dtype/sizes");
    const size_t out_bytes = (n_frames + group - 1) / group * n_values * sum_out_size(out_dtype);
    const uint8_t* d_in = nullptr;
    uint64_t* d_off = nullptr;
    uint32_t* d_st = nullptr;
    void *d_out = nullptr, *d_ws = nullptr;
    int rc = upload_stream(hs, terse, terse_bytes, &d_in);
    if (rc || (rc = status_slot(&d_st)) || (frame_offsets && (rc = upload_offsets(hs, frame_offsets, n_frames, 0, &d_off)))) return rc;
    HIP_TRY(arena().get(Arena::kPixels, out_bytes, &d_out));
    HIP_TRY(arena().get(Arena::kWorkspace, ws_bytes, &d_ws));
    uint32_t st[TRPX_STATUS_WORDS];
    rc = trpx_decode_sum(dtype, out_dtype, d_in, terse_bytes, d_off, nullptr, n_values, n_frames, block, group, d_out, d_st, d_ws, ws_bytes, hs);
    if (rc || (rc = read_status(hs, d_st, st)) || (rc = status_result("trpx_decode_sum_host", st))) return rc;
    HIP_TRY(copy_sync(hs, sums_out, d_out, out_bytes, hipMemcpyDeviceToHost));
    return TRPX_OK;
}

int trpx_decode_roi_host(int dtype, const uint8_t* terse, size_t terse_bytes, const uint64_t* frame_offsets, size_t n_values,
                         size_t n_frames, unsigned block, size_t width, const uint32_t* boxes, size_t n_boxes, unsigned box_h,
                         unsigned box_w, void* pixels_out, int device) {
    trpx::FrameGeom g;
    if (!terse || !boxes || !pixels_out || !terse_bytes) return fail(TRPX_ERR_INVALID_ARG, "trpx_decode_roi_host: bad argument");
    if (block != kBlock || is64(dtype)) return fail(TRPX_ERR_UNSUPPORTED, "trpx_decode_roi_host: block=%u dtype=%d", block, dtype);
    if (!geom_of(n_values, block, &g) || !sizes_ok(g, n_frames)) return fail(TRPX_ERR_INVALID_ARG, "trpx_decode_roi_host: bad sizes");
    if (const int rc = roi_geometry("trpx_decode_roi_host", n_values, width, n_boxes, box_h, box_w)) return rc;
    const size_t ws_bytes = trpx_decode_roi_workspace_bytes(dtype, terse_bytes, n_values, n_frames, block);
    if (!ws_bytes) return fail(TRPX_ERR_INVALID_ARG, "trpx_decode_roi_host: bad dtype/sizes");
    if ((unsigned __int128)n_boxes * box_h * box_w * trpx_dtype_size(dtype) >= ((unsigned __int128)1 << 62) || n_boxes >= ((size_t)1 << 40))
        return fail(TRPX_ERR_INVALID_ARG, "trpx_decode_roi_host: bad sizes n_boxes=%zu", n_boxes);
    for (size_t i = 0; i < n_boxes; ++i)
        if (boxes[3 * i] >= n_frames || (uint64_t)boxes[3 * i + 1] + box_h > n_values / width || (uint64_t)boxes[3 * i + 2] + box_w > width)
            return fail(TRPX_ERR_INVALID_ARG, "trpx_decode_roi_host: box %zu (frame %u, y0 %u, x0 %u) leaves the stack", i, boxes[3 * i],
                        boxes[3 * i + 1], boxes[3 * i + 2]);
    hipStream_t hs = nullptr;
    if (const int rc = enter("trpx_decode_roi_host", device, &hs)) return rc;
    const size_t out_bytes = n_boxes * box_h * box_w * trpx_dtype_size(dtype);
    const uint8_t* d_in = nullptr;
    uint64_t* d_off = nullptr;
    uint32_t* d_st = nullptr;
    void *d_out = nullptr, *d_ws = nullptr;
    int rc = upload_stream(hs, terse, terse_bytes, &d_in);
    if (rc || (rc = status_slot(&d_st)) || (rc = upload_offsets(hs, frame_offsets, n_frames, 12 * n_boxes, &d_off))) return rc;
    uint32_t* d_boxes = reinterpret_cast<uint32_t*>(d_off + (n_frames + 1));
    HIP_TRY(copy_sync(hs, d_boxes, boxes, 12 * n_boxes, hipMemcpyHostToDevice));
    HIP_TRY(arena().get(Arena::kPixels, out_bytes, &d_out));
    HIP_TRY(arena().get(Arena::kWorkspace, ws_bytes, &d_ws));
    uint32_t st[TRPX_STATUS_WORDS];
    rc = trpx_decode_roi(dtype, d_in, terse_bytes, frame_offsets ? d_off : nullptr, nullptr, n_values, n_frames, block, width, d_boxes,
                         n_boxes, box_h, box_w, d_out, d_st, d_ws, ws_bytes, hs);
    if (rc || (rc = read_status(hs, d_st, st)) || (rc = status_result("trpx_decode_roi_host", st))) return rc;
    HIP_TRY(copy_sync(hs, pixels_out, d_out, out_bytes, hipMemcpyDeviceToHost));
    return TRPX_OK;
}

int trpx_group_states_host(const uint8_t* terse, size_t terse_bytes, const uint64_t* frame_offsets, size_t n_values,
                           size_t n_frames, unsigned block, unsigned max_bits, uint64_t* group_states, int device) {
    hipStream_t hs = nullptr;
    if (const int rc = enter("trpx_group_states_host", device, &hs)) return rc;
    trpx::FrameGeom g;
    if (!terse || !terse_bytes || !frame_offsets || !group_states || max_bits == 0 || max_bits > 32)
        return fail(TRPX_ERR_INVALID_ARG, "trpx_group_states_host: bad argument");
    if (block != kBlock) return fail(TRPX_ERR_UNSUPPORTED, "trpx_group_states_host: block=%u", block);
    if (!geom_of(n_values, block, &g) || !sizes_ok(g, n_frames) || n_frames > terse_bytes)
        return fail(TRPX_ERR_INVALID_ARG, "trpx_group_states_host: bad sizes");
    const int dtype = max_bits <= 8 ? TRPX_U8 : max_bits <= 16 ? TRPX_U16 : TRPX_U32;
    const size_t ib = trpx_index_bytes(dtype, n_values, n_frames, block), ng = n_frames * (size_t)g.n_tiles;
    const uint8_t* d_in = nullptr;
    uint64_t* d_off = nullptr;
    uint32_t* d_st = nullptr;
    void* d_idx = nullptr;
    int rc = upload_stream(hs, terse, terse_bytes, &d_in);
    if (rc || (rc = upload_offsets(hs, frame_offsets, n_frames, 8 * ng, &d_off)) || (rc = status_slot(&d_st))) return rc;
    HIP_TRY(arena().get(Arena::kWorkspace, ib, &d_idx));
    uint64_t* d_states = d_off + (n_frames + 1);
    uint32_t st[TRPX_STATUS_WORDS];
    rc = trpx_build_index(dtype, d_in, terse_bytes, d_off, n_values, n_frames, block, d_idx, d_st, hs);
    if (rc || (rc = trpx_index_group_states(d_idx, n_values, n_frames, block, d_states, hs)) || (rc = read_status(hs, d_st, st)) ||
        (rc = status_result("trpx_group_states_host", st)))
        return rc;
    HIP_TRY(copy_sync(hs, group_states, d_states, 8 * ng, hipMemcpyDeviceToHost));
    return TRPX_OK;
}

int trpx_decode_host_grouped(int stream_signed, int out_dtype, const uint8_t* terse, size_t terse_bytes, const uint64_t* frame_offsets,
                             const uint64_t* group_states, size_t n_values, size_t n_frames, unsigned block, void* pixels_out,
                             int device) {
    trpx::FrameGeom g;
    const bool tuned = group_states && frame_offsets && tuned_type(stream_signed, out_dtype) && block == kBlock &&
                       geom_of(n_values, block, &g) && sizes_ok(g, n_frames);
    if (!tuned) return trpx_decode_host(stream_signed, out_dtype, terse, terse_bytes, frame_offsets, n_values, n_frames, block, pixels_out, device);
    hipStream_t hs = nullptr;
    if (const int rc = enter("trpx_decode_host_grouped", device, &hs)) return rc;
    if (!terse || !terse_bytes || !pixels_out) return fail(TRPX_ERR_INVALID_ARG, "trpx_decode_host_grouped: bad argument");
    const size_t out_bytes = n_values * n_frames * trpx_dtype_size(out_dtype), ng = n_frames * (size_t)g.n_tiles;
    const size_t ib = trpx_index_bytes(out_dtype, n_values, n_frames, block);
    const uint8_t* d_in = nullptr;
    uint64_t* d_off = nullptr;
    uint32_t* d_st = nullptr;
    void *d_out = nullptr, *d_idx = nullptr;
    int rc = upload_stream(hs, terse, terse_bytes, &d_in);
    if (rc || (rc = upload_offsets(hs, frame_offsets, n_frames, 8 * ng, &d_off)) || (rc = status_slot(&d_st))) return rc;
    HIP_TRY(arena().get(Arena::kPixels, out_bytes, &d_out));
    HIP_TRY(arena().get(Arena::kWorkspace, ib, &d_idx));
    uint64_t* d_states = d_off + (n_frames + 1);
    HIP_TRY(copy_sync(hs, d_states, group_states, 8 * ng, hipMemcpyHostToDevice));
    uint32_t st[TRPX_STATUS_WORDS];
    bool decoded = false;
    rc = decode_walk_free(stream_signed, out_dtype, d_in, terse_bytes, d_off, d_states, n_values, n_frames, block, d_idx, d_out, d_st, hs,
                          false, st, &decoded);
    if (rc) return rc;
    if (!decoded)
        return trpx_decode_host(stream_signed, out_dtype, terse, terse_bytes, frame_offsets, n_values, n_frames, block, pixels_out, device);
    if ((rc = status_result("trpx_decode_host_grouped", st))) return rc;
    HIP_TRY(copy_sync(hs, pixels_out, d_out, out_bytes, hipMemcpyDeviceToHost));
    return TRPX_OK;
}

struct trpx_stack {
    int device = 0;
    int stream_signed = 0;
    size_t n_values = 0, n_frames = 0, terse_bytes = 0;
    unsigned block = kBlock;
    void* d_terse = nullptr;
    void* d_offs = nullptr;
    void* d_status = nullptr;
    void* d_ws = nullptr;
    size_t ws_bytes = 0;
    void* d_states = nullptr;
    void* d_index = nullptr;
    size_t groups = 0;
    void* d_window = nullptr;
    size_t window_cap = 0, win_first = 0, win_count = 0, window_frames = 0;
    int win_dtype = -1;
    std::vector<uint64_t> offs;
};

static void stack_free(trpx_stack* s) {
    if (!s) return;
    for (void* q : {s->d_terse, s->d_offs, s->d_status, s->d_ws, s->d_window, s->d_states, s->d_index}) if (q) (void)hipFree(q);
    delete s;
}

int trpx_stack_open(trpx_stack** handle, int stream_signed, const uint8_t* terse, size_t terse_bytes, const uint64_t* frame_offsets,
                    const uint64_t* group_states, size_t n_values, size_t n_frames, unsigned block, unsigned max_bits, int device) {
    if (!handle) return fail(TRPX_ERR_INVALID_ARG, "trpx_stack_open: null handle");
    *handle = nullptr;
    hipStream_t hs = nullptr;
    if (const int rc = enter("trpx_stack_open", device, &hs)) return rc;
    trpx::FrameGeom g;
    if (!terse || !terse_bytes || !geom_of(n_values, block, &g) || !sizes_ok(g, n_frames) || n_frames > terse_bytes)
        return fail(TRPX_ERR_INVALID_ARG, "trpx_stack_open: bad argument / sizes");
    std::vector<uint64_t> offs(n_frames + 1);
    if (frame_offsets) {
        memcpy(offs.data(), frame_offsets, 8 * (n_frames + 1));
        if (offs[0] != 0 || offs[n_frames] > terse_bytes) return fail(TRPX_ERR_CORRUPT, "trpx_stack_open: frame offsets do not fit the stack");
        for (size_t f = 0; f < n_frames; ++f)
            if (offs[f + 1] <= offs[f]) return fail(TRPX_ERR_CORRUPT, "trpx_stack_open: frame offsets are not increasing");
    } else if (max_bits > 64) {
        return fail(TRPX_ERR_INVALID_ARG, "trpx_stack_open: max_bits=%u", max_bits);
    }
    trpx_stack* s = new trpx_stack;
    auto bail = [&](hipError_t e, const char* what) { stack_free(s); return fail(TRPX_ERR_HIP, "trpx_stack_open: %s: %s", what, hipGetErrorString(e)); };
    hipError_t e;
    if ((e = hipGetDevice(&s->device)) != hipSuccess) return bail(e, "hipGetDevice");
    s->stream_signed = stream_signed != 0;
    s->n_values = n_values; s->n_frames = n_frames; s->terse_bytes = terse_bytes; s->block = block;
    s->offs.swap(offs);
    const size_t frame_bytes = n_values * 8;
    s->window_frames = std::max<size_t>(1, std::min<size_t>(n_frames, (size_t(64) << 20) / frame_bytes));
    s->ws_bytes = trpx_decode_workspace_bytes(TRPX_U8, n_values, s->window_frames, block);
    if ((e = hipMalloc(&s->d_terse, padded_stream_bytes(terse_bytes))) != hipSuccess) return bail(e, "hipMalloc(stack)");
    if ((e = hipMalloc(&s->d_offs, 8 * (n_frames + 1))) != hipSuccess) return bail(e, "hipMalloc(offsets)");
    if ((e = hipMalloc(&s->d_status, 4 * TRPX_STATUS_WORDS)) != hipSuccess) return bail(e, "hipMalloc(status)");
    if ((e = hipMalloc(&s->d_ws, s->ws_bytes ? s->ws_bytes : 256)) != hipSuccess) return bail(e, "hipMalloc(workspace)");
    if ((e = copy_stream_zero_tail(hs, s->d_terse, terse, terse_bytes)) != hipSuccess) return bail(e, "upload of the stack");
    if (frame_offsets) {
        if ((e = copy_sync(hs, s->d_offs, s->offs.data(), 8 * (n_frames + 1), hipMemcpyHostToDevice)) != hipSuccess) return bail(e, "hipMemcpy(offsets)");
    } else {
        const size_t lb = trpx::locate_workspace_bytes(g, terse_bytes, n_frames);
        void* d_lws = nullptr;
        if ((e = arena().get(Arena::kWorkspace, lb, &d_lws)) != hipSuccess) return bail(e, "locate workspace");
        uint32_t st[TRPX_STATUS_WORDS];
        int rc = trpx_locate_frames(static_cast<const uint8_t*>(s->d_terse), terse_bytes, n_values, n_frames, block,
                                    max_bits ? max_bits : 32, static_cast<uint64_t*>(s->d_offs),
                                    static_cast<uint32_t*>(s->d_status), d_lws, lb, hs);
        if (rc || (rc = read_status(hs, static_cast<uint32_t*>(s->d_status), st)) || (rc = status_result("trpx_stack_open", st))) { stack_free(s); return rc; }
        if ((e = copy_sync(hs, s->offs.data(), s->d_offs, 8 * (n_frames + 1), hipMemcpyDeviceToHost)) != hipSuccess) return bail(e, "hipMemcpy(offsets)");
    }
    if (group_states && block == kBlock) {
        s->groups = g.n_tiles;
        if ((e = hipMalloc(&s->d_states, 8 * n_frames * s->groups)) != hipSuccess) return bail(e, "hipMalloc(states)");
        if ((e = copy_sync(hs, s->d_states, group_states, 8 * n_frames * s->groups, hipMemcpyHostToDevice)) != hipSuccess) return bail(e, "hipMemcpy(states)");
        if ((e = hipMalloc(&s->d_index, trpx_index_bytes(TRPX_U8, n_values, s->window_frames, block))) != hipSuccess) return bail(e, "hipMalloc(index)");
    }
    *handle = s;
    return TRPX_OK;
}

int trpx_stack_read(trpx_stack* s, size_t frame, int out_dtype, void* pixels_out) {
    if (!s || !pixels_out || frame >= s->n_frames) return fail(TRPX_ERR_INVALID_ARG, "trpx_stack_read: bad argument");
    const size_t es = convert_elem_size(out_dtype);
    if (!es) return fail(TRPX_ERR_INVALID_ARG, "trpx_stack_read: unknown dtype %d", out_dtype);
    HIP_TRY(hipSetDevice(s->device));
    hipStream_t hs = nullptr;
    HIP_TRY(arena().get_stream(&hs));
    if (out_dtype != s->win_dtype || frame < s->win_first || frame >= s->win_first + s->win_count) {
        const size_t count = std::min(s->window_frames, s->n_frames - frame);
        const size_t need = count * s->n_values * es;
        if (s->window_cap < need) {
            if (s->d_window) (void)hipFree(s->d_window);
            s->d_window = nullptr; s->window_cap = 0;
            HIP_TRY(hipMalloc(&s->d_window, need));
            s->window_cap = need;
        }
        s->win_count = 0;
        const uint64_t first_byte = s->offs[frame] & ~uint64_t(3);
        const uint8_t* base = static_cast<const uint8_t*>(s->d_terse) + first_byte;
        uint64_t* d_offs = static_cast<uint64_t*>(s->d_offs);
        uint32_t* d_st = static_cast<uint32_t*>(s->d_status);
        std::vector<uint64_t> rel(count + 1);
        for (size_t i = 0; i <= count; ++i) rel[i] = s->offs[frame + i] - first_byte;
        HIP_TRY(copy_sync(hs, d_offs, rel.data(), 8 * (count + 1), hipMemcpyHostToDevice));
        const size_t bytes = (size_t)rel[count];
        uint32_t st[TRPX_STATUS_WORDS];
        bool done = false;
        if (s->d_states && tuned_type(s->stream_signed, out_dtype)) {
            if (const int rc = decode_walk_free(s->stream_signed, out_dtype, base, bytes, d_offs, static_cast<const uint64_t*>(s->d_states) + frame * s->groups,
                                                s->n_values, count, s->block, s->d_index, s->d_window, d_st, hs, true, st, &done))
                return rc;
            done = done && st[0] == 0;
        }
        if (!done)
            if (const int rc = decode_any(s->stream_signed, out_dtype, base, bytes, d_offs, s->n_values, count, s->block, s->d_window, d_st,
                                          s->d_ws, s->ws_bytes, hs, st))
                return rc;
        if (const int rc = status_result("trpx_stack_read", st)) return rc;
        s->win_first = frame; s->win_count = count; s->win_dtype = out_dtype;
    }
    const size_t fb = s->n_values * es;
    HIP_TRY(copy_sync(hs, pixels_out, static_cast<const char*>(s->d_window) + (frame - s->win_first) * fb, fb, hipMemcpyDeviceToHost));
    return TRPX_OK;
}

void trpx_stack_close(trpx_stack* s) {
    if (s) { (void)hipSetDevice(s->device); stack_free(s); }
}

}
```

### trpx_amd/csrc/codec_common.hpp

```cpp
#pragma once
#include <hip/hip_runtime.h>
#include <stdint.h>
#include "trpx_hip.h"

namespace trpx {

constexpr int kBlock = 12;
constexpr int kWave = 64;
constexpr int kThreads = 256;
constexpr int kTileBlocks = kThreads;
constexpr int kTileValues = kTileBlocks * kBlock;

struct FrameGeom {
    uint64_t n_values;
    uint32_t n_blocks;
    uint32_t n_tiles;
    uint32_t block;
};

template <typename T> struct PixelTraits;
template <> struct PixelTraits<uint8_t>  { using U = uint8_t;  static constexpr int bits = 8;  static constexpr bool is_signed = false; static constexpr int dtype = TRPX_U8; };
template <> struct PixelTraits<int8_t>   { using U = uint8_t;  static constexpr int bits = 8;  static constexpr bool is_signed = true;  static constexpr int dtype = TRPX_I8; };
template <> struct PixelTraits<uint16_t> { using U = uint16_t; static constexpr int bits = 16; static constexpr bool is_signed = false; static constexpr int dtype = TRPX_U16; };
template <> struct PixelTraits<int16_t>  { using U = uint16_t; static constexpr int bits = 16; static constexpr bool is_signed = true;  static constexpr int dtype = TRPX_I16; };
template <> struct PixelTraits<uint32_t> { using U = uint32_t; static constexpr int bits = 32; static constexpr bool is_signed = false; static constexpr int dtype = TRPX_U32; };
template <> struct PixelTraits<int32_t>  { using U = uint32_t; static constexpr int bits = 32; static constexpr bool is_signed = true;  static constexpr int dtype = TRPX_I32; };
template <> struct PixelTraits<uint64_t> { using U = uint64_t; static constexpr int bits = 64; static constexpr bool is_signed = false; static constexpr int dtype = TRPX_U64; };
template <> struct PixelTraits<int64_t>  { using U = uint64_t; static constexpr int bits = 64; static constexpr bool is_signed = true;  static constexpr int dtype = TRPX_I64; };

template <class F> inline hipError_t for_pixel_type(int dtype, F&& f) {
    switch (dtype) {
    case TRPX_U8:  return f.template operator()<uint8_t>();
    case TRPX_I8:  return f.template operator()<int8_t>();
    case TRPX_U16: return f.template operator()<uint16_t>();
    case TRPX_I16: return f.template operator()<int16_t>();
    case TRPX_U32: return f.template operator()<uint32_t>();
    case TRPX_I32: return f.template operator()<int32_t>();
    }
    return hipErrorInvalidValue;
}

template <typename T> constexpr int max_block_bits() { return 12 + kBlock * PixelTraits<T>::bits; }

__device__ __forceinline__ uint32_t header_len(uint32_t w, uint32_t w_prev) {
    return w == w_prev ? 1u : (w < 7u ? 4u : (w < 10u ? 6u : 12u));
}
__device__ __forceinline__ uint32_t header_val(uint32_t w, uint32_t w_prev) {
    if (w == w_prev) return 1u;
    if (w < 7u) return w << 1;
    if (w < 10u) return (7u + ((w - 7u) << 3)) << 1;
    return (31u + ((w - 10u) << 5)) << 1;
}
struct ExplicitHeader { uint32_t w, len; };
__device__ __forceinline__ ExplicitHeader parse_explicit_header(uint32_t bits) {
    uint32_t w = (bits >> 1) & 7u, len = 4;
    if (w == 7u) {
        w += (bits >> 4) & 3u; len = 6;
        if (w == 10u) { w += (bits >> 6) & 63u; len = 12; }
    }
    return {w, len};
}
__device__ __forceinline__ ExplicitHeader parse_explicit_header_select(uint32_t bits, uint32_t ext_mask = 63u) {
    const uint32_t w3 = (bits >> 1) & 7u, wa = 7u + ((bits >> 4) & 3u), wb = 10u + ((bits >> 6) & ext_mask);
    return {w3 != 7u ? w3 : (wa != 10u ? wa : wb), w3 != 7u ? 4u : (wa != 10u ? 6u : 12u)};
}

template <typename T>
__device__ __forceinline__ uint32_t width_from_or(uint32_t m) {
    uint32_t bl = 32u - (uint32_t)__builtin_clz(m | 0u) ;
    bl = m ? bl : 0u;
    if (PixelTraits<T>::is_signed) {
        uint32_t w = m ? bl + 1u : 0u;
        return w > (uint32_t)PixelTraits<T>::bits ? (uint32_t)PixelTraits<T>::bits : w;
    }
    return bl;
}

template <typename T>
__device__ __forceinline__ uint32_t width_from_or64(uint64_t m) {
    const uint32_t bl = m ? 64u - (uint32_t)__builtin_clzll(m) : 0u;
    if (PixelTraits<T>::is_signed) {
        const uint32_t w = m ? bl + 1u : 0u;
        return w > (uint32_t)PixelTraits<T>::bits ? (uint32_t)PixelTraits<T>::bits : w;
    }
    return bl;
}
template <typename T>
__device__ __forceinline__ uint64_t magnitude64(T v) {
    if (PixelTraits<T>::is_signed) {
        const int64_t s = (int64_t)v;
        return s < 0 ? (uint64_t)0 - (uint64_t)s : (uint64_t)s;
    }
    return (uint64_t)(typename PixelTraits<T>::U)v;
}

template <typename T>
__device__ __forceinline__ uint32_t magnitude(T v) {
    if (PixelTraits<T>::is_signed) {
        int32_t s = (int32_t)v;
        return s < 0 ? 0u - (uint32_t)s : (uint32_t)s;
    }
    return (uint32_t)(typename PixelTraits<T>::U)v;
}

__device__ __forceinline__ uint32_t wave_inclusive_scan(uint32_t v) {
    v += (uint32_t)__builtin_amdgcn_update_dpp(0, (int)v, 0x111, 0xf, 0xf, false);
    v += (uint32_t)__builtin_amdgcn_update_dpp(0, (int)v, 0x112, 0xf, 0xf, false);
    v += (uint32_t)__builtin_amdgcn_update_dpp(0, (int)v, 0x114, 0xf, 0xf, false);
    v += (uint32_t)__builtin_amdgcn_update_dpp(0, (int)v, 0x118, 0xf, 0xf, false);
    v += (uint32_t)__builtin_amdgcn_update_dpp(0, (int)v, 0x142, 0xa, 0xf, false);
    v += (uint32_t)__builtin_amdgcn_update_dpp(0, (int)v, 0x143, 0xc, 0xf, false);
    return v;
}

__device__ __forceinline__ uint32_t wave_max(uint32_t v) {
    auto step = [](uint32_t x, uint32_t y) { return x > y ? x : y; };
    v = step(v, (uint32_t)__builtin_amdgcn_update_dpp(0, (int)v, 0x111, 0xf, 0xf, false));
    v = step(v, (uint32_t)__builtin_amdgcn_update_dpp(0, (int)v, 0x112, 0xf, 0xf, false));
    v = step(v, (uint32_t)__builtin_amdgcn_update_dpp(0, (int)v, 0x114, 0xf, 0xf, false));
    v = step(v, (uint32_t)__builtin_amdgcn_update_dpp(0, (int)v, 0x118, 0xf, 0xf, false));
    v = step(v, (uint32_t)__builtin_amdgcn_update_dpp(0, (int)v, 0x142, 0xa, 0xf, false));
    v = step(v, (uint32_t)__builtin_amdgcn_update_dpp(0, (int)v, 0x143, 0xc, 0xf, false));
    return (uint32_t)__builtin_amdgcn_readlane((int)v, 63);
}

__device__ __forceinline__ int lane_id() { return (int)(threadIdx.x & 63u); }
__device__ __forceinline__ int wave_id() { return __builtin_amdgcn_readfirstlane((int)(threadIdx.x >> 6)); }

__device__ __forceinline__ uint32_t block_exclusive_scan(uint32_t v, uint32_t* wave_tot, uint32_t* total) {
    uint32_t inc = wave_inclusive_scan(v);
    if (lane_id() == 63) wave_tot[wave_id()] = inc;
    __syncthreads();
    uint32_t t0 = wave_tot[0], t1 = wave_tot[1], t2 = wave_tot[2], t3 = wave_tot[3];
    int w = wave_id();
    uint32_t base = (w > 0 ? t0 : 0u) + (w > 1 ? t1 : 0u) + (w > 2 ? t2 : 0u);
    *total = t0 + t1 + t2 + t3;
    return base + inc - v;
}

template <int kUnused = 0>
__global__ __launch_bounds__(kThreads) void k_zero_words(uint64_t* __restrict__ p, uint64_t n, uint64_t* __restrict__ q,
                                                         uint64_t m) {
    for (uint64_t i = (uint64_t)blockIdx.x * kThreads + threadIdx.x; i < n; i += (uint64_t)gridDim.x * kThreads) p[i] = 0ull;
    if (blockIdx.x == 0 && threadIdx.x < m) q[threadIdx.x] = 0ull;
}
inline void zero_status(uint32_t* status, hipStream_t st) {
    hipLaunchKernelGGL(k_zero_words<0>, dim3(1), dim3(kThreads), 0, st, static_cast<uint64_t*>(nullptr), (uint64_t)0,
                       reinterpret_cast<uint64_t*>(status), (uint64_t)4);
}

__host__ __device__ inline uint64_t align_up(uint64_t x, uint64_t a) { return (x + a - 1) / a * a; }
constexpr uint32_t kDeferSlots = 64, kDeferSlotWords = 16;
constexpr size_t kDeferFront = 8u * kDeferSlots * kDeferSlotWords;
inline size_t defer_bytes(size_t n_frames) { return kDeferFront + align_up(4 * (n_frames + 2), 256); }

}
```

### trpx_amd/csrc/decode_frame.hip

```cpp
#include "codec_common.hpp"
#include "launchers.hpp"
#include "profile.hpp"
#include "unpack_common.hpp"

namespace trpx {

#ifndef TRPX_FRAME_WAVES
#define TRPX_FRAME_WAVES 4
#endif
constexpr int kFrameWaves = TRPX_FRAME_WAVES;
constexpr int kFrameThreads = kFrameWaves * kWave;

#ifndef TRPX_FRAME_CHUNK_DW
#define TRPX_FRAME_CHUNK_DW 2048
#endif
#ifndef TRPX_IDX_TOUCH
#define TRPX_IDX_TOUCH 1
#endif
template <typename T>
struct FrameCfg {
#ifdef TRPX_FRAME_GPW
    static constexpr int kGpw = TRPX_FRAME_GPW;
#else
    static constexpr int kGpw = 4;
#endif
    static constexpr int kStepGroups = (kFrameWaves - 1) * kGpw;
    static constexpr int kStepBlocks = kStepGroups * kWave;
    static constexpr int kChunkDw = TRPX_FRAME_CHUNK_DW;
#ifdef TRPX_DEC_DIRECT_STORES
    static constexpr bool kOutStaged = sizeof(T) == 4;
#else
    static constexpr bool kOutStaged = true;
#endif
    static constexpr int kRawDw = 4 * RawQuads<T>::n;
    static constexpr int kOutDw = kWave * kBlock * (int)sizeof(T) / 4;
    static_assert(kChunkDw % (kWave * 4) == 0, "window = whole 1 KB pieces");
};

__device__ __forceinline__ void lds_dma16(const uint32_t* src_uniform, uint32_t lane_byte_offset, uint32_t lds_base) {
    uint32_t keep;
    asm volatile("s_mov_b32 %0, m0\n\ts_mov_b32 m0, %3\n\ts_nop 0\n\tglobal_load_lds_dwordx4 %1, %2\n\ts_mov_b32 m0, %0"
                 : "=&s"(keep) : "v"(lane_byte_offset), "s"(src_uniform), "s"(lds_base) : "memory");
}

template <typename T, int MODE, bool PARTS = false, bool LINES = false>
__device__ __forceinline__ void decode_frame_body(const uint8_t* __restrict__ terse, uint64_t terse_bytes,
                                                  const uint64_t* __restrict__ frame_offsets, const FrameGeom& g,
                                                  T* __restrict__ pixels_out, uint32_t* __restrict__ defer,
                                                  uint32_t* __restrict__ status, const uint64_t item,
                                                  const uint8_t* __restrict__ idx_widths, const uint64_t* __restrict__ idx_group_off,
                                                  const PartDesc* __restrict__ parts = nullptr) {
    using Cfg = FrameCfg<T>;
    constexpr bool IDX = MODE == 1;
    constexpr int kStepBlocks = Cfg::kStepBlocks, kChunkDw = Cfg::kChunkDw;
    constexpr uint32_t kMaxW = PixelTraits<T>::bits;
    __shared__ __attribute__((aligned(16))) uint32_t s_chunk[kChunkDw + 4];
    constexpr int kPosEntries = kStepBlocks + 64 + 68;
    __shared__ uint32_t s_pos[2][kPosEntries];
    uint32_t* const s_posx = &s_pos[0][0];
    constexpr uint32_t kPosBits = 26, kPosMask = (1u << kPosBits) - 1u;
    __shared__ __attribute__((aligned(16))) uint32_t s_out[kFrameWaves - 1][Cfg::kOutStaged ? Cfg::kOutDw + kStageCarryDw : 4];
    __shared__ uint32_t s_err;
#ifdef TRPX_DEC_LDS_PAD
    __shared__ uint32_t s_pad[TRPX_DEC_LDS_PAD / 4];
    if (terse_bytes == 1) s_pad[threadIdx.x] = 0;
#endif
    __shared__ uint32_t s_role[kFrameWaves];
    __shared__ uint64_t s_keep[3];

    const uint32_t lane = (uint32_t)lane_id();
    const int hw_wave = wave_id();
    uint64_t frame = item;
    uint32_t pb0 = 0, pb1 = g.n_blocks, ppos0 = 0, pw0 = 0, ppos1 = 0, pw1 = 0;
    if constexpr (PARTS && MODE == 1) {
        const uint32_t unit_blocks = (uint32_t)(uintptr_t)parts;
        const uint32_t upf = (g.n_blocks + unit_blocks - 1u) / unit_blocks;
        frame = item / upf;
        pb0 = (uint32_t)(item % upf) * unit_blocks;
        pb1 = pb0 + unit_blocks < g.n_blocks ? pb0 + unit_blocks : g.n_blocks;
        ppos0 = (uint32_t)idx_group_off[frame * g.n_tiles + pb0 / (uint32_t)kTileBlocks];
        pw0 = pb0 ? (uint32_t)idx_widths[frame * g.n_blocks + pb0 - 1u] : 0u;
        if (pb1 < g.n_blocks) {
            ppos1 = (uint32_t)idx_group_off[frame * g.n_tiles + pb1 / (uint32_t)kTileBlocks];
            pw1 = (uint32_t)idx_widths[frame * g.n_blocks + pb1 - 1u];
        }
    } else if constexpr (PARTS) {
        const PartDesc d = parts[item];
        frame = d.frame; pb0 = d.b0; pb1 = d.b1; ppos0 = d.pos0; pw0 = d.w0; ppos1 = d.pos1; pw1 = d.w1;
        if (pb1 <= pb0) return;
    }
    const uint64_t fo = frame_offsets[frame], fe = frame_offsets[frame + 1];
    if (threadIdx.x == 0) {
        s_err = (fe > fo && fe <= terse_bytes && (uint64_t)ppos0 < 8 * (fe - fo) && pb1 <= g.n_blocks) ? 0u : 1u;
        s_keep[0] = (uint64_t)(uintptr_t)status; s_keep[1] = (uint64_t)(uintptr_t)defer; s_keep[2] = item;
    }
    uint32_t hw_slot = 0;
    {
        uint32_t hwid;
        asm volatile("s_getreg_b32 %0, hwreg(HW_REG_HW_ID)" : "=s"(hwid));
        if (lane == 0) s_role[hw_wave] = ((hwid >> 4) & 3u) == (hwid & 3u) ? 1u : 0u;
        hw_slot = hwid & 7u;
    }
    __syncthreads();
    int walker_wave = 0;
#pragma unroll
    for (int i = kFrameWaves - 1; i >= 0; --i) walker_wave = s_role[i] ? i : walker_wave;
    walker_wave = __builtin_amdgcn_readfirstlane(walker_wave);
    const int wave = (hw_wave - walker_wave + kFrameWaves) % kFrameWaves;
    if (s_err) {
        if (threadIdx.x == 0) atomicMax(&status[0], 5u);
        return;
    }
    const uint32_t* __restrict__ s32 = reinterpret_cast<const uint32_t*>(terse);
    const uint64_t n_dw = (terse_bytes + 3) / 4;
    const bool base16 = ((uintptr_t)terse & 15) == 0;
    const uint64_t frame_abit = 8 * fo + ppos0;
    const uint32_t limit = (uint32_t)(8 * (fe - fo) - ppos0);
    const uint64_t frame_dw = frame_abit >> 5;
    const uint32_t frame_sh = (uint32_t)(frame_abit & 31);
    const uint32_t n_blocks = pb1 - pb0;
    const bool at_end = pb1 == g.n_blocks;
    const uint32_t nb_last = at_end ? (uint32_t)(g.n_values - (uint64_t)(g.n_blocks - 1) * kBlock) : (uint32_t)kBlock;
    const uint32_t sb0 = defer ? (uint32_t)((kFrameWaves - 1) * kWave) : (uint32_t)kStepBlocks;
    const uint32_t n_steps = n_blocks <= sb0 ? 1u : 1u + (n_blocks - sb0 + kStepBlocks - 1) / kStepBlocks;
    auto step_begin = [&](uint32_t t) -> uint32_t { return t == 0u ? 0u : sb0 + (t - 1u) * kStepBlocks; };
    T* __restrict__ fout = pixels_out + frame * g.n_values + (uint64_t)pb0 * kBlock;
    const uint32_t out_c = LINES ? (uint32_t)((uintptr_t)fout & 127u) : 0u;

#ifdef TRPX_DEC_NO_STORE
    uint32_t diag_acc = 0;
#endif
    int32_t c_lo = 0, c_hi = 0;
    uint32_t b = 0, w_prev = pw0, pos = 0;
#ifndef TRPX_DEC_WALK_PRIO
#define TRPX_DEC_WALK_PRIO 3
#endif
#ifndef TRPX_DEFER_NUM
#define TRPX_DEFER_NUM 2
#define TRPX_DEFER_DEN 9
#endif
    if (wave == 0) __builtin_amdgcn_s_setprio(TRPX_DEC_WALK_PRIO);
    constexpr int kIdxChunks = IDX ? kStepBlocks / kWave : 1;
    constexpr int kIdxQuads = IDX ? kStepBlocks / (4 * kWave) : 1;
    static_assert(!IDX || kStepBlocks % (4 * kWave) == 0, "the width prefetch covers a super-step in whole quads of 64 lanes (TRPX_FRAME_GPW: a multiple of 4 per three extraction waves)");
    __shared__ __attribute__((aligned(4))) uint8_t s_wnext[IDX ? kStepBlocks : 4];
    [[maybe_unused]] auto idx_load = [&](uint32_t ss, uint32_t (&dst)[kIdxQuads]) {
        const uint8_t* __restrict__ wfl = idx_widths + frame * g.n_blocks + pb0;
        const uint32_t bb = step_begin(ss), be = step_begin(ss + 1u) < n_blocks ? step_begin(ss + 1u) : n_blocks;
#pragma unroll
        for (int j = 0; j < kIdxQuads; ++j) {
            const uint32_t bi = bb + 4u * ((uint32_t)j * kWave + lane);
            uint32_t v = 0u;
            if (bi + 4u <= be) __builtin_memcpy(&v, wfl + bi, 4);
            else {
#pragma unroll
                for (uint32_t k = 0; k < 4u; ++k) v |= bi + k < be ? (uint32_t)wfl[bi + k] << (8u * k) : 0u;
            }
            dst[j] = v;
        }
    };
    [[maybe_unused]] auto idx_park = [&](const uint32_t (&src)[kIdxQuads]) {
#pragma unroll
        for (int j = 0; j < kIdxQuads; ++j) reinterpret_cast<uint32_t*>(s_wnext)[j * kWave + lane] = src[j];
    };
    if constexpr (IDX) {
        if (wave == 0) {
            uint32_t w0[kIdxQuads];
            idx_load(0u, w0);
            idx_park(w0);
        }
    }

#ifdef TRPX_DEC_STAMPS
    uint64_t st_work = 0, st_wait = 0, st_t0 = __builtin_readcyclecounter(), st_start = st_t0;
#endif
    [[maybe_unused]] uint32_t idx_touch = 0;
    for (uint32_t s = 0; s <= n_steps; ++s) {
        if (wave == 0) {
            if (IDX && s < n_steps) {
#if TRPX_IDX_TOUCH
                asm volatile("s_waitcnt vmcnt(0)" : "+v"(idx_touch) : : "memory");
#endif
                const uint32_t beg_b = step_begin(s);
                const uint32_t end_nom = step_begin(s + 1u) < n_blocks ? step_begin(s + 1u) : n_blocks;
                uint32_t* const ent = s_posx + (s & 1u) * kPosEntries;
                uint32_t wq[kIdxChunks], wn[kIdxQuads];
#pragma unroll
                for (int i = 0; i < kIdxChunks; ++i) wq[i] = s_wnext[i * kWave + lane];
                if (s + 1u < n_steps) idx_load(s + 1u, wn);
                bool bad = false;
                [[maybe_unused]] const uint32_t pos_begin = pos;
#pragma unroll
                for (int i = 0; i < kIdxChunks; ++i) {
                    const uint32_t b0 = beg_b + (uint32_t)i * kWave;
                    if (b0 >= end_nom) continue;
                    const uint32_t bi = b0 + lane, wi = wq[i];
                    uint32_t wp = (uint32_t)__shfl_up((int)wi, 1, 64);
                    if (lane == 0) wp = w_prev;
                    const uint32_t hl = wi == wp ? 1u : (wi < 7u ? 4u : (wi < 10u ? 6u : 12u));
                    const uint32_t nv = bi + 1u == n_blocks ? nb_last : (uint32_t)kBlock;
                    const uint32_t len = bi < end_nom ? hl + nv * wi : 0u;
                    const uint32_t incl = wave_inclusive_scan(len);
                    const uint32_t p = pos + incl - len;
                    bad = bad || wi > kMaxW;
                    if (bi < end_nom) {
                        ent[bi - beg_b] = (frame_sh + p) | (wp << kPosBits);
                        if (((pb0 + bi) & (uint32_t)(kTileBlocks - 1)) == 0u && idx_group_off &&
                            idx_group_off[frame * g.n_tiles + (pb0 + bi) / (uint32_t)kTileBlocks] != (uint64_t)ppos0 + p) bad = true;
                    }
                    pos += (uint32_t)__builtin_amdgcn_readlane((int)incl, 63);
                    const uint32_t lastl = end_nom - b0 < (uint32_t)kWave ? end_nom - b0 - 1u : (uint32_t)kWave - 1u;
                    w_prev = (uint32_t)__builtin_amdgcn_readlane((int)wi, (int)lastl);
                    if (pos > limit) bad = true;
                }
                b = end_nom;
                if (!__ballot(bad) && b == n_blocks)
                    bad = at_end ? !(pos <= limit && 1 + ((uint64_t)ppos0 + pos) / 8 == fe - fo) : !(ppos0 + pos == ppos1 && w_prev == pw1);
                if (__ballot(bad) && lane == 0) s_err = 1u;
                if (lane == 0) ent[b - beg_b] = (frame_sh + (pos <= limit ? pos : limit)) | (w_prev << kPosBits);
#if TRPX_IDX_TOUCH
                {
                    const uint64_t a0 = (4u * frame_dw + ((frame_sh + pos_begin) >> 3)) & ~127ull;
                    const uint64_t a1 = 4u * frame_dw + ((frame_sh + (pos <= limit ? pos : limit)) >> 3);
                    for (uint64_t my = a0 + 128u * lane; my <= a1 && my + 4u <= terse_bytes; my += 128u * kWave)
                        asm volatile("global_load_dword %0, %1, off" : "=v"(idx_touch) : "v"(terse + my) : "memory");
                }
#endif
                if (s + 1u < n_steps) idx_park(wn);
            } else if (s < n_steps) {
                const uint32_t buf = s & 1u;
                const uint32_t beg_b = step_begin(s);
                const uint32_t end_nom = step_begin(s + 1u) < n_blocks ? step_begin(s + 1u) : n_blocks;
                const int32_t fast_lim = (int32_t)end_nom < (int32_t)n_blocks - 64 ? (int32_t)end_nom : (int32_t)n_blocks - 64;
                uint32_t* const ent = s_posx + buf * kPosEntries;
                bool bad = false;
                if (s > 0u && lane <= b - beg_b)
                    ent[lane] = s_posx[(buf ^ 1u) * kPosEntries + (beg_b - step_begin(s - 1u)) + lane];
                while (true) {
                    {
                        const uint32_t base8 = 8u * (uint32_t)(uintptr_t)&s_chunk[0];
                        uint32_t pw = frame_sh + pos - 32u * (uint32_t)c_lo + base8;
                        uint32_t stride = 1u + kBlock * w_prev;
                        const uint32_t pw_end = 32u * (uint32_t)(c_hi - c_lo - 1) + base8;
                        uint32_t pw_max = pw_end - 63u * stride;
                        uint32_t v_ls = __umul24(lane, stride);
                        const uint32_t e_base = 32u * (uint32_t)c_lo - base8;
                        uint32_t s_e = e_base + (w_prev << kPosBits);
                        const uint32_t v_entl = (uint32_t)(uintptr_t)ent - 4u * beg_b + 4u * lane;
                        uint32_t s_bad = 0, t_first, t_h, t_t, t_p, t_a, t_bits;
                        asm volatile(
                            "s_cmp_lt_i32 %[b], %[lim]\n\t"
                            "s_cbranch_scc0 9f\n\t"
                            "s_cmp_lt_i32 %[pw], %[pwmax]\n\t"
                            "s_cbranch_scc0 9f\n"
                            "1:\n\t"
                            "v_add_u32 %[p], %[pw], %[ls]\n\t"
                            "v_lshrrev_b32 %[a], 3, %[p]\n\t"
                            "v_and_b32 %[a], 0x1ffffffc, %[a]\n\t"
                            "ds_read2_b32 v[62:63], %[a] offset1:1\n\t"
                            "v_add_u32 %[bits], %[se], %[p]\n\t"
                            "v_lshl_add_u32 %[a], %[b], 2, %[entl]\n\t"
                            "ds_write_b32 %[a], %[bits]\n\t"
                            "s_waitcnt lgkmcnt(1)\n\t"
                            "v_alignbit_b32 %[bits], v63, v62, %[p]\n\t"
                            "v_and_b32 %[a], 1, %[bits]\n\t"
                            "v_cmp_eq_u32 vcc, 0, %[a]\n\t"
                            "s_cbranch_vccz 5f\n\t"
                            "s_ff1_i32_b64 %[first], vcc\n\t"
                            "v_readlane_b32 %[h], %[bits], %[first]\n\t"
                            "s_bfe_u32 %[w], %[h], 0x30001\n\t"
                            "s_cmp_lg_u32 %[w], 7\n\t"
                            "s_cbranch_scc0 6f\n\t"
                            "s_addc_u32 %[b], %[b], %[first]\n\t"
                            "s_mul_i32 %[t], %[first], %[stride]\n\t"
                            "s_mul_i32 %[stride], %[w], 12\n\t"
                            "s_add_i32 %[pw], %[pw], %[t]\n\t"
                            "s_add_i32 %[stride], %[stride], 1\n\t"
                            "s_add_i32 %[pw], %[pw], %[stride]\n\t"
                            "s_add_i32 %[pw], %[pw], 3\n"
                            "3:\n\t"
                            "v_mul_u32_u24 %[ls], %[stride], %[lane]\n\t"
                            "s_lshl_b32 %[t], %[w], 26\n\t"
                            "s_add_i32 %[se], %[ebase], %[t]\n\t"
                            "s_mul_i32 %[t], %[stride], 63\n\t"
                            "s_sub_i32 %[pwmax], %[pwend], %[t]\n"
                            "4:\n\t"
                            "s_cmp_lt_i32 %[b], %[lim]\n\t"
                            "s_cbranch_scc0 9f\n\t"
                            "s_cmp_lt_i32 %[pw], %[pwmax]\n\t"
                            "s_cbranch_scc1 1b\n\t"
                            "s_branch 9f\n"
                            "5:\n\t"
                            "s_lshl_b32 %[t], %[stride], 6\n\t"
                            "s_add_i32 %[pw], %[pw], %[t]\n\t"
                            "s_add_i32 %[b], %[b], 64\n\t"
                            "s_branch 4b\n"
                            "6:\n\t"
                            "s_bfe_u32 %[t], %[h], 0x20004\n\t"
                            "s_add_i32 %[w], %[t], 7\n\t"
                            "s_mul_i32 %[t], %[first], %[stride]\n\t"
                            "s_add_i32 %[pw], %[pw], %[t]\n\t"
                            "s_add_i32 %[pw], %[pw], 6\n\t"
                            "s_cmp_lg_u32 %[w], 10\n\t"
                            "s_cbranch_scc1 7f\n\t"
                            "s_bfe_u32 %[t], %[h], 0x60006\n\t"
                            "s_add_i32 %[w], %[t], 10\n\t"
                            "s_add_i32 %[pw], %[pw], 6\n"
                            "7:\n\t"
                            "s_cmp_gt_u32 %[w], %[maxw]\n\t"
                            "s_cbranch_scc1 8f\n\t"
                            "s_add_i32 %[b], %[b], %[first]\n\t"
                            "s_add_i32 %[b], %[b], 1\n\t"
                            "s_mul_i32 %[stride], %[w], 12\n\t"
                            "s_add_i32 %[pw], %[pw], %[stride]\n\t"
                            "s_add_i32 %[stride], %[stride], 1\n\t"
                            "s_branch 3b\n"
                            "8:\n\t"
                            "s_mov_b32 %[bad], 1\n"
                            "9:\n"
                            : [pw] "+s"(pw), [b] "+s"(b), [w] "+s"(w_prev), [stride] "+s"(stride), [se] "+s"(s_e), [pwmax] "+s"(pw_max),
                              [ls] "+v"(v_ls), [bad] "+s"(s_bad), [first] "=&s"(t_first), [h] "=&s"(t_h), [t] "=&s"(t_t), [p] "=&v"(t_p),
                              [a] "=&v"(t_a), [bits] "=&v"(t_bits)
                            : [lim] "s"(fast_lim), [lane] "v"(lane), [entl] "v"(v_entl), [ebase] "s"(e_base), [pwend] "s"(pw_end),
                              [maxw] "n"(kMaxW)
                            : "vcc", "scc", "memory", "v62", "v63");
                        pos = pw - base8 + 32u * (uint32_t)c_lo - frame_sh;
                        bad = s_bad != 0u;
                    }
                    if (bad || b >= end_nom || b == n_blocks) break;
                    const uint32_t stride = 1u + kBlock * w_prev;
                    const uint32_t need_lo = (frame_sh + pos) >> 5;
                    const uint32_t need_hi = ((frame_sh + pos + 63u * stride) >> 5) + 2;
                    if ((int32_t)need_lo < c_lo || (int32_t)need_hi > c_hi) {
                        c_lo = (int32_t)(((frame_dw + need_lo) & ~3ull) - frame_dw);
                        c_hi = c_lo + kChunkDw;
                        const uint64_t d0 = (uint64_t)((int64_t)frame_dw + c_lo);
                        if (base16 && (d0 & 3) == 0 && d0 + kChunkDw <= n_dw) {
#pragma unroll
                            for (int it = 0; it < kChunkDw / (kWave * 4); ++it)
                                lds_dma16(s32 + d0 + it * kWave * 4, lane * 16u, (uint32_t)(uintptr_t)&s_chunk[it * kWave * 4]);
                            asm volatile("s_waitcnt vmcnt(0)" ::: "memory");
                        } else {
                            for (uint32_t i = lane * 4; i < (uint32_t)kChunkDw; i += kWave * 4) {
                                const uint64_t d = d0 + i;
                                uint4 x;
                                x.x = d < n_dw ? s32[d] : 0u; x.y = d + 1 < n_dw ? s32[d + 1] : 0u;
                                x.z = d + 2 < n_dw ? s32[d + 2] : 0u; x.w = d + 3 < n_dw ? s32[d + 3] : 0u;
                                *reinterpret_cast<uint4*>(&s_chunk[i]) = x;
                            }
                        }
                        if ((int32_t)b < fast_lim) continue;
                    }
                    const uint32_t lpos = pos + lane * stride;
                    const uint32_t fbit = frame_sh + lpos - 32u * (uint32_t)c_lo;
                    const uint32_t bits = __builtin_amdgcn_alignbit(s_chunk[(fbit >> 5) + 1], s_chunk[fbit >> 5], fbit);
                    const uint32_t left = n_blocks - b;
                    const uint64_t valid = left >= 64u ? ~0ull : ((1ull << left) - 1ull);
                    const uint64_t same = __ballot((bits & 1u) != 0u) & valid;
                    const uint64_t stop = ~same;
                    const uint32_t first = stop ? (uint32_t)__builtin_ctzll(stop) : 64u;
                    uint32_t e_w = w_prev, new_pos, new_b;
                    if (first < left && first < 64u) {
                        const auto [w, hl] = parse_explicit_header((uint32_t)__builtin_amdgcn_readlane((int)bits, first));
                        if (w > kMaxW) { bad = true; break; }
                        e_w = w;
                        const uint32_t nbv = b + first + 1 == n_blocks ? nb_last : (uint32_t)kBlock;
                        new_pos = pos + first * stride + hl + nbv * w;
                        new_b = b + first + 1;
                    } else {
                        const uint32_t cnt = left < 64u ? left : 64u;
                        new_pos = pos + cnt * stride;
                        if (b + cnt == n_blocks) new_pos = pos + (cnt - 1) * stride + 1u + nb_last * w_prev;
                        new_b = b + cnt;
                    }
                    if (lane < new_b - b) ent[b - beg_b + lane] = frame_sh + lpos + (w_prev << kPosBits);
                    pos = new_pos;
                    w_prev = e_w;
                    b = new_b;
                    if (pos > limit + 64u * 400u) { bad = true; break; }
                    if (b == n_blocks) break;
                }
                if (!bad && b == n_blocks)
                    bad = at_end ? !(pos <= limit && 1 + ((uint64_t)ppos0 + pos) / 8 == fe - fo) : !(ppos0 + pos == ppos1 && w_prev == pw1);
                if (bad && lane == 0) s_err = 1u;
                if (lane == 0) ent[b - beg_b] = (frame_sh + pos) | (w_prev << kPosBits);
                if (defer && !bad && (s <= 1u || s == 3u || s == 11u) && end_nom == step_begin(s + 1u) && end_nom < n_blocks) {
                    const uint32_t per = (end_nom - beg_b) / kWave;
                    uint32_t changes = 0;
#pragma unroll
                    for (int i = 0; i < kStepBlocks / kWave; ++i) {
                        const uint32_t at = lane * per + i;
                        if ((uint32_t)i < per) changes += (ent[at] >> kPosBits) != (ent[at + 1] >> kPosBits) ? 1u : 0u;
                    }
                    const uint32_t inc = wave_inclusive_scan(changes);
                    const uint32_t chg = (uint32_t)__builtin_amdgcn_readlane((int)inc, 63);
                    const uint32_t blk = per * kWave;
                    uint64_t* const slots = reinterpret_cast<uint64_t*>(defer) - kDeferSlots * kDeferSlotWords;
                    if (s == 0u && lane == 0)
                        __hip_atomic_fetch_add(slots + (blockIdx.x % kDeferSlots) * kDeferSlotWords, ((uint64_t)chg << 32) | blk, __ATOMIC_RELAXED,
                                               __HIP_MEMORY_SCOPE_AGENT);
                    uint64_t d_chg = chg, d_blk = blk;
                    if (chg * 100u > 14u * blk && chg * 100u < 30u * blk) {
                        const uint32_t enough = (gridDim.x < 64u ? gridDim.x : 64u) * blk;
                        uint32_t c = 0, n = 0;
                        for (int poll = 0; poll < 24; ++poll) {
                            const uint64_t v = __hip_atomic_load(slots + lane * kDeferSlotWords, __ATOMIC_RELAXED, __HIP_MEMORY_SCOPE_AGENT);
                            c = (uint32_t)(v >> 32); n = (uint32_t)v;
                            c = (uint32_t)__builtin_amdgcn_readlane((int)wave_inclusive_scan(c), 63);
                            n = (uint32_t)__builtin_amdgcn_readlane((int)wave_inclusive_scan(n), 63);
                            if (s != 0u || n >= enough) break;
                            __builtin_amdgcn_s_sleep(16);
                        }
                        if (s == 0u) { d_chg += c; d_blk += n; }
                        else if (n) { d_chg = c; d_blk = n; }
                    }
                    if (d_chg * (uint64_t)TRPX_DEFER_DEN > (uint64_t)TRPX_DEFER_NUM * d_blk && lane == 0) s_err = 3u;
#ifdef TRPX_DEFER_STATS
                    if (lane == 0) {
                        if (d_chg * (uint64_t)TRPX_DEFER_DEN > (uint64_t)TRPX_DEFER_NUM * d_blk) atomicAdd(status + (s == 0u ? 2 : s == 3u ? 3 : 4), 1u);
                        if (d_blk != blk) atomicAdd(status + 5, 1u);
                        if (s == 0u) atomicAdd(status + 6, chg * 1000u / blk);
                    }
#endif
                }
            }
        } else if (s >= 1) {
#ifndef TRPX_DEC_PRIO_FLAT
            if (((hw_slot + s) & 1u) != 0u) __builtin_amdgcn_s_setprio(1); else __builtin_amdgcn_s_setprio(0);
#endif
            const uint32_t pbuf = (s - 1) & 1u;
            constexpr int kRawDw = Cfg::kRawDw;
            const uint32_t* __restrict__ fbase = s32 + frame_dw;
            const uint32_t step0 = step_begin(s - 1u);
            const uint32_t step1 = step_begin(s) < n_blocks ? step_begin(s) : n_blocks;
            const uint32_t* const ent = s_posx + pbuf * kPosEntries;
#ifdef TRPX_DEC_WALK_ONLY
            const uint32_t gpw = 0;
#else
            const uint32_t gpw = (step_begin(s) - step0) / (uint32_t)((kFrameWaves - 1) * kWave);
#endif
            [[maybe_unused]] const uint32_t n_whole = nb_last == (uint32_t)kBlock || step1 < n_blocks ? step1 : step1 - 1u;
            [[maybe_unused]] bool carry_live = false;
#pragma unroll 1
            for (uint32_t gq = 0; gq < gpw; ++gq) {
                const uint32_t g0 = step0 + ((uint32_t)(wave - 1) * gpw + gq) * kWave;
                if (g0 >= step1) break;
                const uint32_t blk = g0 + lane;
                uint32_t w = 0, q = frame_sh + limit;
                if (blk < step1) {
                    const uint32_t pw = ent[blk - step0 + 1u];
                    w = pw >> kPosBits;
                    q = (pw & kPosMask) - (blk + 1u == n_blocks ? nb_last : (uint32_t)kBlock) * w;
                }
                if constexpr (MODE == 2) {
                    if (blk < step1) {
                        const_cast<uint8_t*>(idx_widths)[frame * g.n_blocks + pb0 + blk] = (uint8_t)w;
                        if (((pb0 + blk) & (uint32_t)(kTileBlocks - 1)) == 0u)
                            const_cast<uint64_t*>(idx_group_off)[frame * g.n_tiles + (pb0 + blk) / (uint32_t)kTileBlocks] =
                                (uint64_t)ppos0 + ((ent[blk - step0] & kPosMask) - frame_sh);
                    }
                    continue;
                }
                const uint32_t dq = q >> 5, sq = q & 31u;
                const uint32_t last_dw = (uint32_t)__builtin_amdgcn_readlane((int)dq, 63) + (uint32_t)kRawDw;
                uint32_t raw[kRawDw];
                if (frame_dw + last_dw <= n_dw) {
#pragma unroll
                    for (int i = 0; i < kRawDw / 4; ++i) {
                        typedef uint32_t u4 __attribute__((ext_vector_type(4)));
                        u4 x4;
                        __builtin_memcpy(&x4, fbase + dq + 4 * i, 16);
                        raw[4 * i] = x4.x; raw[4 * i + 1] = x4.y; raw[4 * i + 2] = x4.z; raw[4 * i + 3] = x4.w;
                    }
                } else {
#pragma unroll
                    for (int i = 0; i < kRawDw; ++i) {
                        const uint64_t d = frame_dw + dq + i;
                        raw[i] = d < n_dw ? s32[d] : 0u;
                    }
                }
#ifdef TRPX_DEC_NO_EXTRACT
                if (q == 0xFFFFFFFFu) fout[0] = (T)(w + raw[0]);
                continue;
#endif
                const bool full = blk < step1 && (blk + 1 < n_blocks || nb_last == (uint32_t)kBlock);
                T* __restrict__ dst = fout + (uint64_t)blk * kBlock;
                uint64_t todo = __ballot(full);
                if (Cfg::kOutStaged && todo == ~0ull) {
                    uint32_t* const stage = s_out[wave - 1] + kStageCarryDw;
                    uint32_t* const row = stage + lane * (kBlock * (uint32_t)sizeof(T) / 4u);
                    [[maybe_unused]] const bool cont = LINES && gq + 1u < gpw && g0 + 2u * (uint32_t)kWave <= n_whole;
                    while (todo) {
                        const int l0 = __builtin_ctzll(todo);
                        const uint32_t w0 = (uint32_t)__builtin_amdgcn_readlane((int)w, l0);
                        uint32_t wd = w0;
                        asm volatile("" : "+s"(wd));
                        const uint64_t mine = __ballot(w == w0);
                        uint32_t ss = sq;
                        asm volatile("" : "+v"(ss));
                        uint32_t o[PackedDwords<T>::n];
                        UnpackRegsDispatch<T, 0, PixelTraits<T>::bits>::run(raw, ss, wd, o);
                        stage_packed_masked<T>(row, o, mine);
                        todo &= ~mine;
                    }
                    __builtin_amdgcn_fence(__ATOMIC_RELEASE, "wavefront");
                    __builtin_amdgcn_wave_barrier();
                    __builtin_amdgcn_fence(__ATOMIC_ACQUIRE, "wavefront");
                    if constexpr (!LINES) store_group<T, false>(stage, fout + (uint64_t)g0 * kBlock);
                    else {
                        store_group_lines<T>(stage, fout + (uint64_t)g0 * kBlock, out_c, carry_live, cont);
                        carry_live = cont;
                    }
                    __builtin_amdgcn_wave_barrier();
                } else if constexpr (sizeof(T) == 4) {
                    while (todo) {
                        const int l0 = __builtin_ctzll(todo);
                        const uint32_t w0 = (uint32_t)__builtin_amdgcn_readlane((int)w, l0);
                        uint32_t wd = w0;
                        asm volatile("" : "+s"(wd));
                        const bool mine = full && w == w0;
                        uint32_t ss = sq;
                        asm volatile("" : "+v"(ss));
                        if (mine) UnpackStoreDispatch<T, 0, PixelTraits<T>::bits>::run(raw, ss, wd, dst);
                        todo &= ~__ballot(mine);
                    }
                } else {
                    uint32_t o[PackedDwords<T>::n];
                    while (todo) {
                        const int l0 = __builtin_ctzll(todo);
                        const uint32_t w0 = (uint32_t)__builtin_amdgcn_readlane((int)w, l0);
                        uint32_t wd = w0;
                        asm volatile("" : "+s"(wd));
                        const bool mine = full && w == w0;
                        uint32_t ss = sq;
                        asm volatile("" : "+v"(ss));
                        if (mine) UnpackRegsDispatch<T, 0, PixelTraits<T>::bits>::run(raw, ss, wd, o);
                        todo &= ~__ballot(mine);
                    }
#ifdef TRPX_DEC_NO_STORE
                    if (full) diag_acc ^= o[0];
#else
                    if (full) store_packed<T>(dst, o);
#endif
                }
                if (blk + 1 == n_blocks && blk < step1 && !full) {
                    const uint32_t mask = w >= 32u ? 0xFFFFFFFFu : ((1u << w) - 1u);
                    uint32_t p = q;
                    for (uint32_t k = 0; k < nb_last; ++k) {
                        uint32_t f = 0;
                        if (w) {
                            const uint64_t d = frame_dw + (p >> 5);
                            const uint64_t two = (uint64_t)(d < n_dw ? s32[d] : 0u) | ((uint64_t)(d + 1 < n_dw ? s32[d + 1] : 0u) << 32);
                            f = (uint32_t)(two >> (p & 31u)) & mask;
                            if (PixelTraits<T>::is_signed) f = (uint32_t)((int32_t)(f << (32u - w)) >> (32u - w));
                        }
                        dst[k] = (T)f;
                        p += w;
                    }
                }
            }
        }
#ifdef TRPX_DEC_STAMPS
        { const uint64_t t1 = __builtin_readcyclecounter(); st_work += t1 - st_t0; st_t0 = t1; }
#endif
        __syncthreads();
#ifdef TRPX_DEC_STAMPS
        { const uint64_t t1 = __builtin_readcyclecounter(); st_wait += t1 - st_t0; st_t0 = t1; }
#endif
        if (s_err) break;
    }
#ifdef TRPX_DEC_STAMPS
    if (lane == 0) {
        uint32_t hwid;
        asm volatile("s_getreg_b32 %0, hwreg(HW_REG_HW_ID)" : "=s"(hwid));
        uint32_t* dbg = reinterpret_cast<uint32_t*>(fout) + 8 * wave;
        dbg[0] = (uint32_t)st_work; dbg[1] = (uint32_t)st_wait; dbg[2] = hwid; dbg[3] = (uint32_t)(st_t0 - st_start);
        dbg[4] = (uint32_t)(st_start & 0xFFFFFFFFu);
        uint32_t xcc;
        asm volatile("s_getreg_b32 %0, hwreg(HW_REG_XCC_ID)" : "=s"(xcc));
        dbg[5] = xcc;
        dbg[6] = dbg[7] = 0;
    }
#endif
#ifdef TRPX_DEC_NO_STORE
    if (diag_acc == 0x12345678u) fout[threadIdx.x] = (T)diag_acc;
#endif
    if (threadIdx.x == 0 && s_err != 0u) {
        asm volatile("" ::: "memory");
        uint32_t* const status_l = reinterpret_cast<uint32_t*>((uintptr_t)s_keep[0]);
        uint32_t* const defer_l = reinterpret_cast<uint32_t*>((uintptr_t)s_keep[1]);
        if (s_err == 1u) atomicMax(&status_l[0], 5u);
        if (s_err >= 2u) {
            defer_l[1u + atomicAdd(&defer_l[0], 1u)] = (uint32_t)s_keep[2] | (s_err == 3u ? 0x80000000u : 0u);
            if (s_err == 3u) atomicAdd(reinterpret_cast<unsigned long long*>(defer_l) - 2, 1ull);
        }
    }
}

template <typename T, bool LINES>
__global__ __launch_bounds__(kFrameThreads, sizeof(T) == 4 ? 6 : 8) void k_decode_frames(const uint8_t* __restrict__ terse, uint64_t terse_bytes,
                                                               const uint64_t* __restrict__ frame_offsets, FrameGeom g,
                                                               T* __restrict__ pixels_out, uint32_t* __restrict__ defer,
                                                               uint32_t* __restrict__ status) {
    decode_frame_body<T, 0, false, LINES>(terse, terse_bytes, frame_offsets, g, pixels_out, defer, status, blockIdx.x, nullptr, nullptr);
}

template <typename T>
__global__ __launch_bounds__(kFrameThreads, sizeof(T) == 4 ? 6 : 8) void k_decode_parts(const uint8_t* __restrict__ terse, uint64_t terse_bytes,
                                                               const uint64_t* __restrict__ frame_offsets, FrameGeom g,
                                                               T* __restrict__ pixels_out, uint32_t* __restrict__ status,
                                                               const PartDesc* __restrict__ parts, const uint32_t* __restrict__ frame_mode) {
    if (status[0] != 0u) return;
    if (frame_mode && frame_mode[parts[blockIdx.x].frame] != 0u) return;
    decode_frame_body<T, 0, true, true>(terse, terse_bytes, frame_offsets, g, pixels_out, nullptr, status, blockIdx.x, nullptr, nullptr, parts);
}

template <typename T>
__global__ __launch_bounds__(kFrameThreads, sizeof(T) == 4 ? 6 : 8) void k_decode_frames_indexed(const uint8_t* __restrict__ terse, uint64_t terse_bytes,
                                                               const uint64_t* __restrict__ frame_offsets, FrameGeom g,
                                                               const uint8_t* __restrict__ widths, const uint64_t* __restrict__ group_off,
                                                               const uint32_t* __restrict__ list, T* __restrict__ pixels_out,
                                                               uint32_t* __restrict__ status) {
    uint64_t frame = blockIdx.x;
    if (list) {
        if (blockIdx.x >= list[0] || status[0] != 0u) return;
        frame = list[1u + blockIdx.x] & 0x7FFFFFFFu;
    }
#ifdef TRPX_IDX_LINES
    decode_frame_body<T, 1, false, true>(terse, terse_bytes, frame_offsets, g, pixels_out, nullptr, status, frame, widths, group_off);
#else
    decode_frame_body<T, 1>(terse, terse_bytes, frame_offsets, g, pixels_out, nullptr, status, frame, widths, group_off);
#endif
}

template <typename T>
__global__ __launch_bounds__(kFrameThreads, sizeof(T) == 4 ? 6 : 8) void k_decode_units_indexed(const uint8_t* __restrict__ terse, uint64_t terse_bytes,
                                                               const uint64_t* __restrict__ frame_offsets, FrameGeom g,
                                                               const uint8_t* __restrict__ widths, const uint64_t* __restrict__ group_off,
                                                               uint32_t unit_blocks, T* __restrict__ pixels_out, uint32_t* __restrict__ status,
                                                               const uint32_t* __restrict__ frame_mode) {
    if (status[0] != 0u) return;
    if (frame_mode && frame_mode[blockIdx.x / ((g.n_blocks + unit_blocks - 1u) / unit_blocks)] == 0u) return;
    decode_frame_body<T, 1, true>(terse, terse_bytes, frame_offsets, g, pixels_out, nullptr, status, blockIdx.x, widths, group_off,
                                  reinterpret_cast<const PartDesc*>((uintptr_t)unit_blocks));
}
template <typename T>
static uint32_t units_choose(const DecodeArgs& a, uint64_t* cost_out);
template <typename T>
static hipError_t launch_decode_units_indexed_t(const DecodeArgs& a, hipStream_t st, const uint32_t* frame_mode) {
    const uint32_t unit_blocks = units_choose<T>(a, nullptr);
    const uint32_t upf = (a.geom.n_blocks + unit_blocks - 1u) / unit_blocks;
    hipLaunchKernelGGL((k_decode_units_indexed<T>), dim3(a.n_frames * upf), dim3(kFrameThreads), 0, st, a.terse, (uint64_t)a.terse_bytes,
                       a.frame_offsets, a.geom, static_cast<const uint8_t*>(a.widths), static_cast<const uint64_t*>(a.tile_off), unit_blocks,
                       static_cast<T*>(a.pixels_out), a.status, frame_mode);
    return hipGetLastError();
}
constexpr uint64_t units_resident(size_t pixel_bytes) { return (uint64_t)(pixel_bytes == 4 ? 6 : 8) * 256u; }
template <typename T>
static uint32_t units_choose(const DecodeArgs& a, uint64_t* cost_out) {
    constexpr uint32_t step = FrameCfg<T>::kStepBlocks;
    static_assert(step % kTileBlocks == 0, "units start on index groups");
    const uint64_t resident = units_resident(sizeof(T)) * 15u / 16u;
    uint32_t unit_blocks = 8u * step;
    uint64_t best = ~0ull;
    for (uint32_t k = 8; k <= 32; ++k) {
        const uint64_t u = (uint64_t)k * step, units = (uint64_t)a.n_frames * ((a.geom.n_blocks + u - 1) / u);
        const uint64_t cost = ((units + resident - 1) / resident) * (u + step);
        if (cost < best) { best = cost; unit_blocks = (uint32_t)u; }
    }
    if (cost_out) *cost_out = best;
    return unit_blocks;
}
hipError_t launch_decode_units_indexed(int dtype, const DecodeArgs& a, hipStream_t st, const uint32_t* frame_mode) {
    return for_pixel_type(dtype, [&]<class T>() { return launch_decode_units_indexed_t<T>(a, st, frame_mode); });
}

template <typename T>
__global__ __launch_bounds__(kFrameThreads, sizeof(T) == 4 ? 6 : 8) void k_index_frames(const uint8_t* __restrict__ terse, uint64_t terse_bytes,
                                                               const uint64_t* __restrict__ frame_offsets, FrameGeom g,
                                                               uint8_t* __restrict__ widths, uint64_t* __restrict__ group_off,
                                                               uint32_t* __restrict__ defer, uint32_t* __restrict__ status) {
    decode_frame_body<T, 2>(terse, terse_bytes, frame_offsets, g, static_cast<T*>(nullptr), defer, status, blockIdx.x, widths, group_off);
}

hipError_t launch_index_frames(uint32_t max_w, const DecodeArgs& a, bool clear_status, hipStream_t st) {
    hipLaunchKernelGGL(k_zero_words<0>, dim3(1), dim3(kThreads), 0, st, reinterpret_cast<uint64_t*>(a.defer) - kDeferSlots * kDeferSlotWords,
                       (uint64_t)(kDeferSlots * kDeferSlotWords + 1), reinterpret_cast<uint64_t*>(a.status), (uint64_t)(clear_status ? 4 : 0));
    if (max_w <= 8u)
        hipLaunchKernelGGL((k_index_frames<uint8_t>), dim3(a.n_frames), dim3(kFrameThreads), 0, st, a.terse, (uint64_t)a.terse_bytes,
                           a.frame_offsets, a.geom, a.widths, a.tile_off, a.defer, a.status);
    else if (max_w <= 16u)
        hipLaunchKernelGGL((k_index_frames<uint16_t>), dim3(a.n_frames), dim3(kFrameThreads), 0, st, a.terse, (uint64_t)a.terse_bytes,
                           a.frame_offsets, a.geom, a.widths, a.tile_off, a.defer, a.status);
    else
        hipLaunchKernelGGL((k_index_frames<uint32_t>), dim3(a.n_frames), dim3(kFrameThreads), 0, st, a.terse, (uint64_t)a.terse_bytes,
                           a.frame_offsets, a.geom, a.widths, a.tile_off, a.defer, a.status);
    return launch_seg_listed(a, max_w, st);
}

template <typename T>
static hipError_t launch_decode_frames_indexed_t(const DecodeArgs& a, const uint32_t* list, hipStream_t st) {
#ifdef TRPX_IDX_AS_UNITS
    if (!list) return launch_decode_units_indexed_t<T>(a, st, nullptr);
#endif
    if (!list && a.geom.n_blocks > 8u * FrameCfg<T>::kStepBlocks) {
        uint64_t cost_units = 0;
        units_choose<T>(a, &cost_units);
        const uint64_t resident = units_resident(sizeof(T));
        const uint64_t cost_whole = ((a.n_frames + resident - 1) / resident) * ((uint64_t)a.geom.n_blocks + FrameCfg<T>::kStepBlocks);
        if (10u * cost_units < 9u * cost_whole) return launch_decode_units_indexed_t<T>(a, st, nullptr);
    }
    hipLaunchKernelGGL((k_decode_frames_indexed<T>), dim3(a.n_frames), dim3(kFrameThreads), 0, st, a.terse, (uint64_t)a.terse_bytes,
                       a.frame_offsets, a.geom, static_cast<const uint8_t*>(a.widths), static_cast<const uint64_t*>(a.tile_off), list,
                       static_cast<T*>(a.pixels_out), a.status);
    return hipGetLastError();
}

hipError_t launch_decode_frames_indexed(int dtype, const DecodeArgs& a, const uint32_t* list, hipStream_t st) {
    return for_pixel_type(dtype, [&]<class T>() { return launch_decode_frames_indexed_t<T>(a, list, st); });
}

template <typename T>
static hipError_t launch_decode_frames_t(const DecodeArgs& a, hipStream_t st) {
    uint32_t* defer = a.defer && a.seg_ws ? a.defer : nullptr;
    const bool chain = a.chain && a.parts && a.parts_per_frame > 1u;
    if (chain) {
        if (!defer) return hipErrorInvalidValue;
        const hipError_t e = launch_chain_zero(a, (uint32_t)PixelTraits<T>::bits, true, st);
        if (e != hipSuccess) return e;
    } else
        hipLaunchKernelGGL(k_zero_words<0>, dim3(1), dim3(kThreads), 0, st,
                           defer ? reinterpret_cast<uint64_t*>(defer) - kDeferSlots * kDeferSlotWords : static_cast<uint64_t*>(nullptr),
                           (uint64_t)(defer ? kDeferSlots * kDeferSlotWords + 1 : 0),
                           reinterpret_cast<uint64_t*>(a.status), (uint64_t)4);
    Profiler& prof = profiler();
    prof.begin();
    prof.mark(st);
    if (chain) {
        if (!defer) return hipErrorInvalidValue;
        constexpr int dt = PixelTraits<T>::dtype;
        constexpr bool narrow = sizeof(T) < 4;
        const uint32_t* frame_mode = nullptr;
        hipError_t e = launch_build_index_chain(a, (uint32_t)PixelTraits<T>::bits, narrow, &frame_mode, st);
        if (e != hipSuccess) return e;
        prof.mark(st);
        e = launch_seg_listed(a, (uint32_t)PixelTraits<T>::bits, st);
        if (e != hipSuccess) return e;
#ifdef TRPX_CHAIN_EXTRACT_TILES
        const bool tiles = TRPX_CHAIN_EXTRACT_TILES != 0;
#else
        const bool tiles = sizeof(T) == 4 || a.geom.n_blocks < (1u << 18);
#endif
        e = tiles ? launch_unpack_tiles(dt, a, st, narrow ? frame_mode : nullptr) : launch_decode_units_indexed(dt, a, st, narrow ? frame_mode : nullptr);
        if (e != hipSuccess) return e;
        if constexpr (narrow)
            hipLaunchKernelGGL((k_decode_parts<T>), dim3(a.n_frames * a.parts_per_frame), dim3(kFrameThreads), 0, st, a.terse, (uint64_t)a.terse_bytes,
                               a.frame_offsets, a.geom, static_cast<T*>(a.pixels_out), a.status, static_cast<const PartDesc*>(a.parts), frame_mode);
        prof.mark(st);
        return hipGetLastError();
    } else if (a.parts && a.parts_per_frame > 1u) {
        if (!defer) return hipErrorInvalidValue;
        const hipError_t e = launch_build_parts(a, (uint32_t)PixelTraits<T>::bits, st);
        if (e != hipSuccess) return e;
        hipLaunchKernelGGL((k_decode_parts<T>), dim3(a.n_frames * a.parts_per_frame), dim3(kFrameThreads), 0, st, a.terse, (uint64_t)a.terse_bytes,
                           a.frame_offsets, a.geom, static_cast<T*>(a.pixels_out), a.status, static_cast<const PartDesc*>(a.parts),
                           static_cast<const uint32_t*>(nullptr));
    } else if ((a.geom.n_values * sizeof(T)) % 128u == 0u && (uintptr_t)a.pixels_out % 128u == 0u)
        hipLaunchKernelGGL((k_decode_frames<T, false>), dim3(a.n_frames), dim3(kFrameThreads), 0, st, a.terse, (uint64_t)a.terse_bytes,
                           a.frame_offsets, a.geom, static_cast<T*>(a.pixels_out), defer, a.status);
    else
        hipLaunchKernelGGL((k_decode_frames<T, true>), dim3(a.n_frames), dim3(kFrameThreads), 0, st, a.terse, (uint64_t)a.terse_bytes,
                           a.frame_offsets, a.geom, static_cast<T*>(a.pixels_out), defer, a.status);
    prof.mark(st);
    if (defer) {
        const hipError_t e = launch_decode_deferred(PixelTraits<T>::dtype, a, st);
        prof.mark(st);
        if (e != hipSuccess) return e;
    }
    return hipGetLastError();
}

hipError_t launch_decode_frames(int dtype, const DecodeArgs& a, hipStream_t st) {
    return for_pixel_type(dtype, [&]<class T>() { return launch_decode_frames_t<T>(a, st); });
}

}
```

### trpx_amd/csrc/launchers.hpp

```cpp
#pragma once
#include <hip/hip_runtime.h>
#include <stdint.h>
#include <stddef.h>
#include "codec_common.hpp"

namespace trpx {

struct EncodeArgs {
    const void* pixels;
    FrameGeom   geom;
    uint32_t    n_frames;
    uint8_t*    out;
    size_t      out_capacity;
    uint64_t*   frame_offsets;
    uint32_t*   status;
    uint64_t*   frame_size;
    uint64_t*   tile_off;
    uint32_t*   tile_bits;
    uint8_t*    idx_widths;
    uint64_t*   idx_group_off;
};

struct PartDesc {
    uint32_t frame, b0, b1, pos0, w0, pos1, w1, pad;
};
constexpr uint32_t kPartBlocks = 16384;
constexpr uint32_t kPartMaxBlocks = 32768;
constexpr uint32_t kManyFrames = 768;
constexpr uint32_t kManyBlocks = 1u << 20;
uint32_t single_part_blocks(size_t n_frames);
void set_single_part_rule(uint32_t many_frames, uint32_t many_blocks);

struct DecodeArgs {
    const uint8_t*  terse;
    size_t          terse_bytes;
    const uint64_t* frame_offsets;
    FrameGeom       geom;
    uint32_t        n_frames;
    void*           pixels_out;
    uint32_t*       status;
    uint64_t*       tile_off;
    uint8_t*        widths;
    uint64_t*       walk_offsets;
    uint32_t*       defer;
    void*           seg_ws;
    bool            index_per_frame = false;
    PartDesc*       parts = nullptr;
    uint32_t        parts_per_frame = 1;
    void*           part_ws = nullptr;
    bool            index_given = false;
    bool            chain = false;
};
uint32_t parts_per_frame(const FrameGeom& g, size_t n_frames);
size_t part_workspace_bytes(const FrameGeom& g, size_t n_frames);
hipError_t launch_build_parts(const DecodeArgs& a, uint32_t max_w, hipStream_t st);
uint32_t chain_parts_per_frame(const FrameGeom& g, size_t n_frames, size_t pixel_bytes);
size_t chain_workspace_bytes(const FrameGeom& g, size_t n_frames, size_t pixel_bytes);
hipError_t launch_build_index_chain(const DecodeArgs& a, uint32_t max_w, bool narrow, const uint32_t** frame_mode, hipStream_t st);
hipError_t launch_chain_zero(const DecodeArgs& a, uint32_t max_w, bool clear_status, hipStream_t st);
hipError_t launch_unpack_tiles(int dtype, const DecodeArgs& a, hipStream_t st, const uint32_t* frame_mode = nullptr);

hipError_t launch_encode(int dtype, const EncodeArgs& a, hipStream_t st);
hipError_t launch_encode_generic(int dtype, const EncodeArgs& a, hipStream_t st);
size_t fused_workspace_bytes(const FrameGeom& g, size_t n_frames);
hipError_t launch_encode_fused(int dtype, const EncodeArgs& a, void* ws, hipStream_t st);
void fused_ws_forget(const void* lo, size_t bytes, const void* keep = nullptr);
hipError_t launch_decode(int dtype, const DecodeArgs& a, bool have_offsets, hipStream_t st);
hipError_t launch_decode_convert(int dtype, const DecodeArgs& a, int stream_signed, bool have_offsets, hipStream_t st);
hipError_t launch_decode_fast(int dtype, const DecodeArgs& a, bool have_index, hipStream_t st, bool per_frame = false);
hipError_t launch_decode_frames(int dtype, const DecodeArgs& a, hipStream_t st);
hipError_t launch_decode_frames_indexed(int dtype, const DecodeArgs& a, const uint32_t* list, hipStream_t st);
hipError_t launch_decode_units_indexed(int dtype, const DecodeArgs& a, hipStream_t st, const uint32_t* frame_mode = nullptr);
hipError_t launch_index_frames(uint32_t max_w, const DecodeArgs& a, bool clear_status, hipStream_t st);
hipError_t launch_seg_listed(const DecodeArgs& a, uint32_t max_w, hipStream_t st);
hipError_t launch_seg_groups(const DecodeArgs& a, uint32_t max_w, const uint64_t* states, hipStream_t st);
hipError_t launch_walk_only(const DecodeArgs& a, uint32_t max_w, bool clear_status, hipStream_t st);
hipError_t launch_walk_serial(const DecodeArgs& a, uint32_t max_w, hipStream_t st);
extern int g_locate_path;
size_t locate_workspace_bytes(const FrameGeom& g, uint64_t terse_bytes, uint64_t n_frames);
hipError_t launch_locate(const uint8_t* terse, uint64_t terse_bytes, const FrameGeom& g, uint32_t n_frames, uint32_t max_w,
                         uint64_t* offsets, uint32_t* status, void* workspace, hipStream_t st, bool clear_status = true);
bool locate_parallel(const FrameGeom& g, uint64_t terse_bytes, uint64_t n_frames, uint32_t max_w);
hipError_t launch_locate_status(const uint64_t* offsets, uint32_t n_frames, uint32_t* status, hipStream_t st);
hipError_t launch_index_group_states(const DecodeArgs& a, uint64_t* states, hipStream_t st);
hipError_t launch_walk_groups(const DecodeArgs& a, uint32_t max_w, const uint64_t* states, bool clear_status, hipStream_t st);
size_t seg_workspace_bytes(const FrameGeom& g, size_t n_frames);
size_t dense_workspace_bytes(const FrameGeom& g, size_t n_frames);
hipError_t launch_dense_listed(const DecodeArgs& a, uint32_t max_w, void* dense_ws, const uint32_t* list, hipStream_t st);
void set_dense_route(bool on);
hipError_t launch_seg_walk(const DecodeArgs& a, uint32_t max_w, hipStream_t st);
bool seg_single_wave(const FrameGeom& g, size_t n_frames);
hipError_t launch_decode_deferred(int dtype, const DecodeArgs& a, hipStream_t st);
hipError_t launch_synth(int dtype, uint64_t seed, uint64_t frame0, size_t n_frames, size_t n_values,
                        void* out, hipStream_t st);

}
```

Before: 3.761 million.

## Collapse per-frame decode to one launch via last-block ticket and host feedback

Adds a ticket scheme to the per-frame decode kernel: the last finishing block resets the defer and status words itself, so the separate zeroing launch can be skipped on reused workspaces. A host-mapped feedback word tells the next call whether any frames were deferred, so the deferred-decode launches can also be skipped when the previous call on the same workspace had none. This cuts kernel launches per decode call to one in steady state. In exchange it adds host-side workspace tracking under a mutex, graph-capture detection, and a speculative keep path that counts would-be deferrals instead of deferring.

```diff
diff --git a/include/trpx_hip.h b/include/trpx_hip.h
--- a/include/trpx_hip.h
+++ b/include/trpx_hip.h
@@ -106,6 +106,8 @@
 
 int trpx_workspace_invalidate(const void* workspace, size_t workspace_bytes);
 
+int trpx_last_decode_launches(void);
+
 int trpx_bench_stream(int mode, const void* src, void* dst, size_t bytes, void* stream);
 
 int trpx_set_encode_path(int path);
diff --git a/trpx_amd/_lib.py b/trpx_amd/_lib.py
--- a/trpx_amd/_lib.py
+++ b/trpx_amd/_lib.py
@@ -85,6 +85,7 @@
     "trpx_profile_read": (_I, [C.POINTER(C.c_float), _I]),
     "trpx_bench_stream": (_I, [_I, _P, _P, _SZ, _P]),
     "trpx_workspace_invalidate": (_I, [_P, _SZ]),
+    "trpx_last_decode_launches": (_I, []),
     "trpx_synth_fill": (_I, [_I, _U64, _U64, _SZ, _SZ, _P, _P]),
     "trpx_header_format": (_SZ, [C.POINTER(trpx_header), C.c_char_p, _SZ]),
     "trpx_header_parse": (_I, [C.c_char_p, _SZ, C.POINTER(trpx_header), C.POINTER(_SZ)]),
diff --git a/trpx_amd/codec.py b/trpx_amd/codec.py
--- a/trpx_amd/codec.py
+++ b/trpx_amd/codec.py
@@ -147,12 +147,14 @@
                                             out.data_ptr(), status.data_ptr(), _stream_ptr(terse)))
         return out, status
     ws_bytes = lib().trpx_decode_workspace_bytes(code, n_values, n_frames, block)
-    ws = (workspace or Workspace(dev)).get(ws_bytes)
+    ws = workspace.get(ws_bytes) if workspace is not None else torch.empty(max(ws_bytes, 256), dtype=torch.uint8, device=dev)
     with torch.cuda.device(dev):
         check(lib().trpx_decode(int(stream_signed), code, terse.data_ptr(), terse.numel(),
                                 frame_offsets.data_ptr() if frame_offsets is not None else None,
                                 n_values, n_frames, block, out.data_ptr(), status.data_ptr(), ws.data_ptr(),
                                 ws.numel(), _stream_ptr(terse)))
+        if workspace is None:
+            check(lib().trpx_workspace_invalidate(ws.data_ptr(), ws.numel()))
     return out, status
 
 
diff --git a/trpx_amd/csrc/api.hip b/trpx_amd/csrc/api.hip
--- a/trpx_amd/csrc/api.hip
+++ b/trpx_amd/csrc/api.hip
@@ -5,6 +5,7 @@
 #include <string.h>
 #include <algorithm>
 #include <initializer_list>
+#include <mutex>
 #include <vector>
 
 #include "../../include/trpx_hip.h"
@@ -180,6 +181,96 @@
     return 0;
 }();
 
+struct DecWs {
+    int device; const char* ptr; size_t bytes;
+    int dtype; size_t n_values, n_frames;
+    uint32_t first_seq, last_seq;
+    bool clean, captured;
+    int slot;
+};
+std::mutex g_dec_mu;
+std::vector<DecWs> g_dec;
+constexpr int kDecSlots = 64;
+uint64_t* g_dec_fb = nullptr;
+bool g_dec_slot_used[kDecSlots];
+uint32_t g_dec_seq = 0;
+thread_local int g_last_decode_launches = 0;
+
+void decode_ws_forget(const void* lo, size_t bytes) {
+    std::lock_guard<std::mutex> lk(g_dec_mu);
+    const char* a = static_cast<const char*>(lo);
+    for (size_t i = 0; i < g_dec.size();)
+        if (!lo || (g_dec[i].ptr < a + bytes && a < g_dec[i].ptr + g_dec[i].bytes)) {
+            if (g_dec[i].slot >= 0) g_dec_slot_used[g_dec[i].slot] = false;
+            g_dec[i] = g_dec.back(); g_dec.pop_back();
+        } else ++i;
+}
+void forget_workspace(const void* lo, size_t bytes, const void* keep_encoder = nullptr) {
+    trpx::fused_ws_forget(lo, bytes, keep_encoder);
+    decode_ws_forget(lo, bytes);
+}
+
+trpx::DecodeCtl one_launch_rule(const void* ws, size_t bytes, int dtype, size_t n_values, size_t n_frames, hipStream_t hs) {
+    trpx::DecodeCtl ctl;
+    ctl.launches = &g_last_decode_launches;
+    hipStreamCaptureStatus cap = hipStreamCaptureStatusNone;
+    if (hipStreamIsCapturing(hs, &cap) != hipSuccess) { (void)hipGetLastError(); cap = hipStreamCaptureStatusActive; }
+    const bool capturing = cap != hipStreamCaptureStatusNone;
+    int device = -1;
+    (void)hipGetDevice(&device);
+    const char* a = static_cast<const char*>(ws);
+    std::lock_guard<std::mutex> lk(g_dec_mu);
+    DecWs* e = nullptr;
+    bool tainted = false;
+    for (size_t i = 0; i < g_dec.size();) {
+        DecWs& d = g_dec[i];
+        if (!(d.ptr < a + bytes && a < d.ptr + d.bytes)) { ++i; continue; }
+        if (d.device == device && d.ptr == a && d.bytes == bytes) { e = &d; ++i; continue; }
+        tainted = tainted || d.captured;
+        if (d.slot >= 0) g_dec_slot_used[d.slot] = false;
+        const bool moved = e == &g_dec.back();
+        d = g_dec.back(); g_dec.pop_back();
+        if (moved) e = &d;
+    }
+    if (capturing || tainted || (e && e->captured)) {
+        if (e) { if (e->slot >= 0) g_dec_slot_used[e->slot] = false; e->slot = -1; e->captured = true; }
+        else g_dec.push_back(DecWs{device, a, bytes, dtype, n_values, n_frames, 0, 0, false, true, -1});
+        return ctl;
+    }
+    const uint32_t seq = ++g_dec_seq ? g_dec_seq : ++g_dec_seq;
+    const bool recognised = e && e->dtype == dtype && e->n_values == n_values && e->n_frames == n_frames;
+    if (!e) {
+        if (!g_dec_fb && hipHostMalloc(reinterpret_cast<void**>(&g_dec_fb), 64 * kDecSlots, hipHostMallocPortable | hipHostMallocMapped | hipHostMallocCoherent) != hipSuccess) {
+            (void)hipGetLastError();
+            g_dec_fb = nullptr;
+            return ctl;
+        }
+        int slot = 0;
+        while (slot < kDecSlots && g_dec_slot_used[slot]) ++slot;
+        if (slot == kDecSlots) return ctl;
+        g_dec_slot_used[slot] = true;
+        g_dec.push_back(DecWs{device, a, bytes, dtype, n_values, n_frames, seq, seq, false, false, slot});
+        e = &g_dec.back();
+    } else if (!recognised) {
+        e->dtype = dtype; e->n_values = n_values; e->n_frames = n_frames;
+        e->first_seq = seq; e->clean = false;
+    }
+    uint64_t* const word = g_dec_fb + 8 * e->slot;
+    void* dev_word = nullptr;
+    if (hipHostGetDevicePointer(&dev_word, word, 0) != hipSuccess) { (void)hipGetLastError(); return ctl; }
+    const uint64_t fb = __atomic_load_n(word, __ATOMIC_RELAXED);
+    const uint32_t fb_seq = (uint32_t)(fb >> 32), fb_count = (uint32_t)fb;
+    const bool fb_ours = recognised && fb != 0 && (int32_t)(fb_seq - e->first_seq) >= 0;
+    ctl.ticket = true;
+    ctl.keep = fb_ours && fb_count == 0u;
+    ctl.clear = !(recognised && (e->clean || (fb_ours && fb_seq == e->last_seq && fb_count == 0u)));
+    ctl.seq = seq;
+    ctl.feedback = static_cast<uint64_t*>(dev_word);
+    e->last_seq = seq;
+    e->clean = ctl.keep;
+    return ctl;
+}
+
 struct IdxScratch {
     struct Slot { int dev; hipStream_t st; void* p; size_t bytes; };
     std::vector<Slot> slots;
@@ -257,16 +348,16 @@
     a.idx_widths = index ? reinterpret_cast<uint8_t*>(static_cast<char*>(index) + il.widths) : nullptr;
     if (block != kBlock || is64(dtype)) {
         if (index) return fail(TRPX_ERR_UNSUPPORTED, "trpx_encode_indexed: the decode index needs block=12 and pixels of <= 32 bits");
-        trpx::fused_ws_forget(workspace, workspace_bytes);
+        forget_workspace(workspace, workspace_bytes);
         HIP_TRY(trpx::launch_encode_generic(dtype, a, static_cast<hipStream_t>(stream)));
         return TRPX_OK;
     }
     const bool vec_ok = (uint64_t)g.n_blocks * 396 < (1ull << 40);
     if (g_encode_path == 0 && !two_pass && vec_ok) {
-        trpx::fused_ws_forget(workspace, workspace_bytes, ws + w.fused);
+        forget_workspace(workspace, workspace_bytes, ws + w.fused);
         HIP_TRY(trpx::launch_encode_fused(dtype, a, ws + w.fused, static_cast<hipStream_t>(stream)));
     } else {
-        trpx::fused_ws_forget(workspace, workspace_bytes);
+        forget_workspace(workspace, workspace_bytes);
         HIP_TRY(trpx::launch_encode(dtype, a, static_cast<hipStream_t>(stream)));
         if (index && out)
             return build_index_impl(dtype, out, out_capacity, frame_offsets, n_values, n_frames, block, index, status, false, stream);
@@ -420,9 +511,17 @@
     const bool parts_ok = a.parts_per_frame > 1u && n_frames * (uint64_t)a.parts_per_frame < 0x7FFFFFFFull && a.defer;
     if (parts_ok) point_into(a, ws, w, kParts);
     else a.parts_per_frame = 1;
-    if (fast_ok && (parts_ok || (frame26 && trpx::parts_per_frame(g, n_frames) == 1u)) && !force_tiles)
-        HIP_TRY(trpx::launch_decode_frames(out_dtype, a, hs));
-    else if (fast_ok)
+    const bool per_frame = fast_ok && (parts_ok || (frame26 && trpx::parts_per_frame(g, n_frames) == 1u)) && !force_tiles;
+    g_last_decode_launches = 0;
+    if (per_frame && !parts_ok && !located && a.defer && trpx::decode_ticket_route(g, n_frames))
+        a.ctl = one_launch_rule(workspace, workspace_bytes, out_dtype, n_values, n_frames, hs);
+    else
+        decode_ws_forget(workspace, workspace_bytes);
+    if (per_frame) {
+        const hipError_t e = trpx::launch_decode_frames(out_dtype, a, hs);
+        if (e != hipSuccess) decode_ws_forget(workspace, workspace_bytes);
+        HIP_TRY(e);
+    } else if (fast_ok)
         HIP_TRY(trpx::launch_decode_fast(out_dtype, a, false, hs));
     else
         HIP_TRY(trpx::launch_decode(out_dtype, a, frame_offsets != nullptr, hs));
@@ -505,7 +604,7 @@
         return rc;
     const DecLayout w = dec_ws(g, n_frames, es);
     if (workspace_bytes < w.total) return fail(TRPX_ERR_CAPACITY, "trpx_decode_convert: workspace %zu < %zu", workspace_bytes, w.total);
-    trpx::fused_ws_forget(workspace, workspace_bytes);
+    forget_workspace(workspace, workspace_bytes);
     trpx::DecodeArgs a = decode_args(terse, terse_bytes, frame_offsets, g, n_frames, pixels_out, status);
     a.walk_offsets = static_cast<uint64_t*>(workspace);
     point_into(a, workspace, w, kSeg);
@@ -514,9 +613,11 @@
 }
 
 int trpx_workspace_invalidate(const void* workspace, size_t workspace_bytes) {
-    trpx::fused_ws_forget(workspace, workspace_bytes);
-    return TRPX_OK;
-}
+    forget_workspace(workspace, workspace_bytes);
+    return TRPX_OK;
+}
+
+int trpx_last_decode_launches(void) { return g_last_decode_launches; }
 
 int trpx_set_encode_path(int path) {
     if (path != 0 && path != 1) return fail(TRPX_ERR_INVALID_ARG, "trpx_set_encode_path: 0 = auto, 1 = two-pass");
@@ -573,7 +674,7 @@
         return fail(TRPX_ERR_INVALID_ARG, "trpx_locate_frames: misaligned pointer (terse needs 4 B, workspace 8 B)");
     const size_t need = trpx::locate_workspace_bytes(g, terse_bytes, n_frames);
     if (workspace_bytes < need) return fail(TRPX_ERR_CAPACITY, "trpx_locate_frames: workspace %zu < %zu", workspace_bytes, need);
-    trpx::fused_ws_forget(workspace, workspace_bytes);
+    forget_workspace(workspace, workspace_bytes);
     HIP_TRY(trpx::launch_locate(terse, terse_bytes, g, (uint32_t)n_frames, max_bits, frame_offsets, status, workspace,
                                 static_cast<hipStream_t>(stream)));
     return TRPX_OK;
@@ -664,7 +765,7 @@
 
     hipStream_t st = static_cast<hipStream_t>(stream);
     char* ws = static_cast<char*>(workspace);
-    if (workspace) trpx::fused_ws_forget(workspace, workspace_bytes);
+    if (workspace) forget_workspace(workspace, workspace_bytes);
     bool clear = true;
     if (const int rc = index_in_workspace(dtype, terse, terse_bytes, &frame_offsets, &index, n_values, n_frames, block, g, status, ws,
                                           w.front, stream, &clear))
@@ -731,7 +832,7 @@
     if (workspace_bytes < w.total) return fail(TRPX_ERR_CAPACITY, "trpx_decode_roi: workspace %zu < %zu", workspace_bytes, w.total);
     if (w.total && !workspace) return fail(TRPX_ERR_INVALID_ARG, "trpx_decode_roi: null workspace");
 
-    if (w.total) trpx::fused_ws_forget(workspace, workspace_bytes);
+    if (w.total) forget_workspace(workspace, workspace_bytes);
     bool clear = true;
     if (const int rc = index_in_workspace(dtype, terse, terse_bytes, &frame_offsets, &index, n_values, n_frames, block, g, status,
                                           static_cast<char*>(workspace), w, stream, &clear))
@@ -776,9 +877,9 @@
     hipError_t get(int slot, size_t n, void** out, bool encoder = false) {
         hipError_t e = on_device();
         if (e != hipSuccess) return e;
-        if (slot == kWorkspace && !encoder && p[slot]) trpx::fused_ws_forget(p[slot], cap[slot]);
+        if (slot == kWorkspace && !encoder && p[slot]) forget_workspace(p[slot], cap[slot]);
         if (cap[slot] < n) {
-            if (p[slot] && slot == kWorkspace) trpx::fused_ws_forget(p[slot], cap[slot]);
+            if (p[slot] && slot == kWorkspace) forget_workspace(p[slot], cap[slot]);
             if (p[slot]) (void)hipFree(p[slot]);
             p[slot] = nullptr; cap[slot] = 0;
             const size_t want = n + n / 8 + 256;
@@ -797,7 +898,7 @@
         return hipSuccess;
     }
     void release() {
-        if (p[kWorkspace]) trpx::fused_ws_forget(p[kWorkspace], cap[kWorkspace]);
+        if (p[kWorkspace]) forget_workspace(p[kWorkspace], cap[kWorkspace]);
         for (int i = 0; i < kSlots; ++i) { if (p[i]) (void)hipFree(p[i]); p[i] = nullptr; cap[i] = 0; }
         if (stream) (void)hipStreamDestroy(stream);
         stream = nullptr;
diff --git a/trpx_amd/csrc/codec_common.hpp b/trpx_amd/csrc/codec_common.hpp
--- a/trpx_amd/csrc/codec_common.hpp
+++ b/trpx_amd/csrc/codec_common.hpp
@@ -151,6 +151,7 @@
 
 __host__ __device__ inline uint64_t align_up(uint64_t x, uint64_t a) { return (x + a - 1) / a * a; }
 constexpr uint32_t kDeferSlots = 64, kDeferSlotWords = 16;
+constexpr uint32_t kDeferTicketWord = 8;
 constexpr size_t kDeferFront = 8u * kDeferSlots * kDeferSlotWords;
 inline size_t defer_bytes(size_t n_frames) { return kDeferFront + align_up(4 * (n_frames + 2), 256); }
 
diff --git a/trpx_amd/csrc/decode_frame.hip b/trpx_amd/csrc/decode_frame.hip
--- a/trpx_amd/csrc/decode_frame.hip
+++ b/trpx_amd/csrc/decode_frame.hip
@@ -10,6 +10,7 @@
 #endif
 constexpr int kFrameWaves = TRPX_FRAME_WAVES;
 constexpr int kFrameThreads = kFrameWaves * kWave;
+constexpr uint64_t kDecTicket = 1, kDecKeep = 2;
 
 #ifndef TRPX_FRAME_CHUNK_DW
 #define TRPX_FRAME_CHUNK_DW 2048
@@ -49,7 +50,8 @@
                                                   T* __restrict__ pixels_out, uint32_t* __restrict__ defer,
                                                   uint32_t* __restrict__ status, const uint64_t item,
                                                   const uint8_t* __restrict__ idx_widths, const uint64_t* __restrict__ idx_group_off,
-                                                  const PartDesc* __restrict__ parts = nullptr) {
+                                                  const PartDesc* __restrict__ parts = nullptr,
+                                                  const uint64_t ctl_bits = 0, uint64_t* __restrict__ feedback = nullptr) {
     using Cfg = FrameCfg<T>;
     constexpr bool IDX = MODE == 1;
     constexpr int kStepBlocks = Cfg::kStepBlocks, kChunkDw = Cfg::kChunkDw;
@@ -66,7 +68,8 @@
     if (terse_bytes == 1) s_pad[threadIdx.x] = 0;
 #endif
     __shared__ uint32_t s_role[kFrameWaves];
-    __shared__ uint64_t s_keep[3];
+    __shared__ uint64_t s_keep[5];
+    __shared__ uint32_t s_would;
 
     const uint32_t lane = (uint32_t)lane_id();
     const int hw_wave = wave_id();
@@ -93,6 +96,8 @@
     if (threadIdx.x == 0) {
         s_err = (fe > fo && fe <= terse_bytes && (uint64_t)ppos0 < 8 * (fe - fo) && pb1 <= g.n_blocks) ? 0u : 1u;
         s_keep[0] = (uint64_t)(uintptr_t)status; s_keep[1] = (uint64_t)(uintptr_t)defer; s_keep[2] = item;
+        s_keep[3] = ctl_bits; s_keep[4] = (uint64_t)(uintptr_t)feedback;
+        s_would = 0u;
     }
     uint32_t hw_slot = 0;
     {
@@ -107,8 +112,49 @@
     for (int i = kFrameWaves - 1; i >= 0; --i) walker_wave = s_role[i] ? i : walker_wave;
     walker_wave = __builtin_amdgcn_readfirstlane(walker_wave);
     const int wave = (hw_wave - walker_wave + kFrameWaves) % kFrameWaves;
+    auto depart = [&]() {
+        if (wave != 0) return;
+        asm volatile("s_waitcnt vmcnt(0)" ::: "memory");
+        uint32_t* const status_l = reinterpret_cast<uint32_t*>((uintptr_t)s_keep[0]);
+        uint32_t* const defer_l = reinterpret_cast<uint32_t*>((uintptr_t)s_keep[1]);
+        const uint64_t bits = s_keep[3];
+        const uint32_t err = s_err;
+        uint32_t seen = 0;
+        if (lane == 0 && err >= 2u) {
+            defer_l[1u + atomicAdd(&defer_l[0], 1u)] = (uint32_t)s_keep[2] | (err == 3u ? 0x80000000u : 0u);
+            if (err == 3u) seen = (uint32_t)atomicAdd(reinterpret_cast<unsigned long long*>(defer_l) - 2, 1ull);
+        }
+        if (!(bits & kDecTicket)) {
+            if (lane == 0 && err == 1u) atomicMax(&status_l[0], 5u);
+            return;
+        }
+        uint64_t* const slots = reinterpret_cast<uint64_t*>(defer_l) - kDeferSlots * kDeferSlotWords;
+        uint32_t* const ticket = reinterpret_cast<uint32_t*>(slots + kDeferTicketWord);
+        uint32_t* const err_w = reinterpret_cast<uint32_t*>(slots + kDeferSlotWords + kDeferTicketWord);
+        uint32_t last = 0;
+        if (lane == 0) {
+            if (err == 1u) seen += __hip_atomic_fetch_max(err_w, 5u, __ATOMIC_RELAXED, __HIP_MEMORY_SCOPE_AGENT);
+            if (s_would) seen += __hip_atomic_fetch_add(err_w + 1, 1u, __ATOMIC_RELAXED, __HIP_MEMORY_SCOPE_AGENT);
+            asm volatile("" : : "v"(seen) : "memory");
+            last = __hip_atomic_fetch_add(ticket, 1u, __ATOMIC_RELAXED, __HIP_MEMORY_SCOPE_AGENT) + 1u == gridDim.x ? 1u : 0u;
+        }
+        if (!__builtin_amdgcn_readfirstlane(last)) return;
+        asm volatile("" ::: "memory");
+        const uint32_t e = __hip_atomic_load(err_w, __ATOMIC_RELAXED, __HIP_MEMORY_SCOPE_AGENT);
+        const uint32_t n = __hip_atomic_load((bits & kDecKeep) ? err_w + 1 : defer_l, __ATOMIC_RELAXED, __HIP_MEMORY_SCOPE_AGENT);
+        static_assert(kDeferSlots == kWave, "one accumulator per lane");
+        __hip_atomic_store(slots + lane * kDeferSlotWords, 0ull, __ATOMIC_RELAXED, __HIP_MEMORY_SCOPE_AGENT);
+        if (lane < 4u) reinterpret_cast<uint64_t*>(status_l)[lane] = lane == 0u ? (uint64_t)e : 0ull;
+        if (lane == 0) {
+            uint64_t* const fb = reinterpret_cast<uint64_t*>((uintptr_t)s_keep[4]);
+            if (fb) __hip_atomic_store(fb, (bits & ~0xFFFFFFFFull) | n, __ATOMIC_RELAXED, __HIP_MEMORY_SCOPE_SYSTEM);
+            __hip_atomic_store(reinterpret_cast<uint64_t*>(err_w), 0ull, __ATOMIC_RELAXED, __HIP_MEMORY_SCOPE_AGENT);
+            reinterpret_cast<uint64_t*>(err_w)[1] = bits >> 32;
+            __hip_atomic_store(ticket, 0u, __ATOMIC_RELAXED, __HIP_MEMORY_SCOPE_AGENT);
+        }
+    };
     if (s_err) {
-        if (threadIdx.x == 0) atomicMax(&status[0], 5u);
+        depart();
         return;
     }
     const uint32_t* __restrict__ s32 = reinterpret_cast<const uint32_t*>(terse);
@@ -414,7 +460,9 @@
                         if (s == 0u) { d_chg += c; d_blk += n; }
                         else if (n) { d_chg = c; d_blk = n; }
                     }
-                    if (d_chg * (uint64_t)TRPX_DEFER_DEN > (uint64_t)TRPX_DEFER_NUM * d_blk && lane == 0) s_err = 3u;
+                    if (d_chg * (uint64_t)TRPX_DEFER_DEN > (uint64_t)TRPX_DEFER_NUM * d_blk && lane == 0) {
+                        if (s_keep[3] & kDecKeep) s_would = 1u; else s_err = 3u;
+                    }
 #ifdef TRPX_DEFER_STATS
                     if (lane == 0) {
                         if (d_chg * (uint64_t)TRPX_DEFER_DEN > (uint64_t)TRPX_DEFER_NUM * d_blk) atomicAdd(status + (s == 0u ? 2 : s == 3u ? 3 : 4), 1u);
@@ -585,24 +633,18 @@
 #ifdef TRPX_DEC_NO_STORE
     if (diag_acc == 0x12345678u) fout[threadIdx.x] = (T)diag_acc;
 #endif
-    if (threadIdx.x == 0 && s_err != 0u) {
-        asm volatile("" ::: "memory");
-        uint32_t* const status_l = reinterpret_cast<uint32_t*>((uintptr_t)s_keep[0]);
-        uint32_t* const defer_l = reinterpret_cast<uint32_t*>((uintptr_t)s_keep[1]);
-        if (s_err == 1u) atomicMax(&status_l[0], 5u);
-        if (s_err >= 2u) {
-            defer_l[1u + atomicAdd(&defer_l[0], 1u)] = (uint32_t)s_keep[2] | (s_err == 3u ? 0x80000000u : 0u);
-            if (s_err == 3u) atomicAdd(reinterpret_cast<unsigned long long*>(defer_l) - 2, 1ull);
-        }
-    }
+    asm volatile("" ::: "memory");
+    depart();
 }
 
 template <typename T, bool LINES>
 __global__ __launch_bounds__(kFrameThreads, sizeof(T) == 4 ? 6 : 8) void k_decode_frames(const uint8_t* __restrict__ terse, uint64_t terse_bytes,
                                                                const uint64_t* __restrict__ frame_offsets, FrameGeom g,
                                                                T* __restrict__ pixels_out, uint32_t* __restrict__ defer,
-                                                               uint32_t* __restrict__ status) {
-    decode_frame_body<T, 0, false, LINES>(terse, terse_bytes, frame_offsets, g, pixels_out, defer, status, blockIdx.x, nullptr, nullptr);
+                                                               uint32_t* __restrict__ status, uint64_t ctl_bits,
+                                                               uint64_t* __restrict__ feedback) {
+    decode_frame_body<T, 0, false, LINES>(terse, terse_bytes, frame_offsets, g, pixels_out, defer, status, blockIdx.x, nullptr, nullptr,
+                                          nullptr, ctl_bits, feedback);
 }
 
 template <typename T>
@@ -720,6 +762,14 @@
     return for_pixel_type(dtype, [&]<class T>() { return launch_decode_frames_indexed_t<T>(a, list, st); });
 }
 
+bool decode_ticket_route(const FrameGeom& g, size_t n_frames) {
+#ifdef TRPX_DEFER_STATS
+    return false;
+#else
+    return seg_single_wave(g, n_frames);
+#endif
+}
+
 template <typename T>
 static hipError_t launch_decode_frames_t(const DecodeArgs& a, hipStream_t st) {
     uint32_t* defer = a.defer && a.seg_ws ? a.defer : nullptr;
@@ -728,11 +778,21 @@
         if (!defer) return hipErrorInvalidValue;
         const hipError_t e = launch_chain_zero(a, (uint32_t)PixelTraits<T>::bits, true, st);
         if (e != hipSuccess) return e;
-    } else
+    }
+    const bool whole = !chain && !(a.parts && a.parts_per_frame > 1u);
+    const bool ticket = whole && defer && a.ctl.ticket && decode_ticket_route(a.geom, a.n_frames);
+    const bool keep = ticket && a.ctl.keep;
+    int launches = 0;
+    if (!chain && !(ticket && !a.ctl.clear)) {
         hipLaunchKernelGGL(k_zero_words<0>, dim3(1), dim3(kThreads), 0, st,
                            defer ? reinterpret_cast<uint64_t*>(defer) - kDeferSlots * kDeferSlotWords : static_cast<uint64_t*>(nullptr),
                            (uint64_t)(defer ? kDeferSlots * kDeferSlotWords + 1 : 0),
                            reinterpret_cast<uint64_t*>(a.status), (uint64_t)4);
+        ++launches;
+    }
+    const uint64_t ctl_bits = ticket ? kDecTicket | (keep ? kDecKeep : 0u) | ((uint64_t)a.ctl.seq << 32) : 0ull;
+    uint64_t* const feedback = ticket ? a.ctl.feedback : nullptr;
+    if (a.ctl.launches) *a.ctl.launches = 0;
     Profiler& prof = profiler();
     prof.begin();
     prof.mark(st);
@@ -767,16 +827,21 @@
                            static_cast<const uint32_t*>(nullptr));
     } else if ((a.geom.n_values * sizeof(T)) % 128u == 0u && (uintptr_t)a.pixels_out % 128u == 0u)
         hipLaunchKernelGGL((k_decode_frames<T, false>), dim3(a.n_frames), dim3(kFrameThreads), 0, st, a.terse, (uint64_t)a.terse_bytes,
-                           a.frame_offsets, a.geom, static_cast<T*>(a.pixels_out), defer, a.status);
+                           a.frame_offsets, a.geom, static_cast<T*>(a.pixels_out), defer, a.status, ctl_bits, feedback);
     else
         hipLaunchKernelGGL((k_decode_frames<T, true>), dim3(a.n_frames), dim3(kFrameThreads), 0, st, a.terse, (uint64_t)a.terse_bytes,
-                           a.frame_offsets, a.geom, static_cast<T*>(a.pixels_out), defer, a.status);
+                           a.frame_offsets, a.geom, static_cast<T*>(a.pixels_out), defer, a.status, ctl_bits, feedback);
+    ++launches;
     prof.mark(st);
-    if (defer) {
+    if (defer && keep)
+        prof.mark(st);
+    else if (defer) {
         const hipError_t e = launch_decode_deferred(PixelTraits<T>::dtype, a, st);
         prof.mark(st);
         if (e != hipSuccess) return e;
-    }
+        launches += a.index_given ? 1 : 2;
+    }
+    if (whole && a.ctl.launches) *a.ctl.launches = launches;
     return hipGetLastError();
 }
 
diff --git a/trpx_amd/csrc/launchers.hpp b/trpx_amd/csrc/launchers.hpp
--- a/trpx_amd/csrc/launchers.hpp
+++ b/trpx_amd/csrc/launchers.hpp
@@ -31,6 +31,17 @@
 uint32_t single_part_blocks(size_t n_frames);
 void set_single_part_rule(uint32_t many_frames, uint32_t many_blocks);
 
+struct DecodeCtl {
+    bool      ticket = false;
+    bool      keep = false;
+    bool      clear = true;
+    uint32_t  seq = 0;
+    uint64_t* feedback = nullptr;
+    int*      launches = nullptr;
+};
+
+bool decode_ticket_route(const FrameGeom& g, size_t n_frames);
+
 struct DecodeArgs {
     const uint8_t*  terse;
     size_t          terse_bytes;
@@ -49,6 +60,7 @@
     uint32_t        parts_per_frame = 1;
     void*           part_ws = nullptr;
     bool            index_given = false;
+    DecodeCtl       ctl;
     bool            chain = false;
 };
 uint32_t parts_per_frame(const FrameGeom& g, size_t n_frames);
```

After: 3.789 million (median of 6 runs). About the same (+0.8%).
